# Ryukhaan/speech-to-video-mpp

Hardware: AMD Instinct MI355X
Metric: synthesized 256×256 frames/sec/GPU (LNet+ENet path); 1/2/4/8-GPU scaling (higher is better)
Workload: dtype f32; 1 GPU; ENet(+LNet) forward, B=16 synthetic 256x256 crops + [1,80,16] mel windows -> 384x384 (models/ENet.py:82-139); crop=256, global_batch=16, batch_per_gpu=16, parallelism=frame-shard x1 (no data-path collective), graph=True, lanes=1, world_size_seen=1

## Files before the change

include/s2v.h:

```cpp
#ifndef S2V_H_
#define S2V_H_

#include <stddef.h>
#include <stdint.h>

#ifdef __cplusplus
extern "C" {
#endif

typedef void *s2v_stream_t;

enum {
    S2V_OK = 0,
    S2V_E_INVALID = -1,
    S2V_E_LAUNCH = -2,
    S2V_E_WORKSPACE = -3
};

enum {
    S2V_ACT_NONE = 0,
    S2V_ACT_RELU = 1,
    S2V_ACT_LRELU = 2,
    S2V_ACT_SIGMOID = 3,
    S2V_ACT_TANH = 4,
    S2V_ACT_GELU_TANH = 5
};

enum {
    S2V_IN_DIRECT = 0,
    S2V_IN_NEAREST_UP2 = 1,
    S2V_IN_TRANSPOSED = 2
};

enum { S2V_PAD_ZERO = 0, S2V_PAD_REFLECT = 1 };

typedef struct s2v_conv_params {
    const float *x; int n, h, w, cin, xcs;
    int in_mode; int pad_mode;
    int pre_act; float pre_alpha;
    const float *in_scale; int in_scale_ns;
    int kh, kw, sh, sw, ph, pw, dh, dw;
    const float *wt; int kpad, npad; int cout;
    int b_kn; int ldb;
    float *y; int oh, ow, ycs;
    const float *scale, *shift;
    const float *nc_scale; int nc_scale_ns;
    const float *pix_add; float pix_w;
    const float *res; int res_cs, res_h, res_w, res_oy, res_ox; int res_after_act;
    int act; float alpha;
    int batch; long long x_bs, w_bs, y_bs, res_bs;
    float *ws; size_t ws_bytes;
    int force_tile; int force_splits;
    int out_step; int out_full_h, out_full_w;
    int prec;
    const void *wt_x3;
    int grid_cap;
    float wt_scale;
    int out_pool;
    int x_split;
    unsigned long long *stamps;
    const unsigned long long *stamp_ctr;
    int stamp_slot, stamp_stride, stamp_reps;
    float x_scale;
    int *nonfinite;
    int d2s_cout;
    const float *post_mul, *post_add; int post_cs, post_c0;
    const float *dup_src, *dup_bias; float dup_a; int dup_cs, dup_off;
} s2v_conv_params;

enum { S2V_PREC_F32 = 0, S2V_PREC_BF16X3 = 1, S2V_PREC_F16X3 = 2, S2V_PREC_F16 = 3 };

int s2v_conv2d(const s2v_conv_params *p, s2v_stream_t stream);
size_t s2v_conv2d_ws_bytes(const s2v_conv_params *p);
int s2v_conv2d_plan(const s2v_conv_params *p, int *out11);
#define S2V_CONV_GROUP_MAX 4
int s2v_conv2d_group(const s2v_conv_params *ps, int n, s2v_stream_t stream);
size_t s2v_conv2d_group_ws_bytes(const s2v_conv_params *ps, int n);
int s2v_conv2d_group_plan(const s2v_conv_params *ps, int n, int *out);
enum { S2V_TUNE_HALO_MIN_BLOCKS = 0, S2V_TUNE_GLDS_TILE = 1, S2V_TUNE_SMALLK_TILE = 2, S2V_TUNE_X3_RATE_512 = 3,
       S2V_TUNE_IN_FUSED = 4, S2V_TUNE_RESIZE_UP2 = 5, S2V_TUNE_COUNT = 6 };
int s2v_tune(int key, long long value, long long *old_value);

int s2v_amax(const float *x, long long pixels, int c, int xcs, float *out, s2v_stream_t stream);

int s2v_split_weights(const float *w, int rows, int kpad, int prec, float scale, void *out, s2v_stream_t stream);
int s2v_split_weights_x3(const float *w, int rows, int kpad, void *out, s2v_stream_t stream);
int s2v_split_act(const float *x, long long pixels, int c, int xcs, int prec, float *out, int ocs,
                  s2v_stream_t stream);

int s2v_layernorm2d(const float *x, int n, int h, int w, int c, int xcs,
                    const float *weight, const float *bias, float eps, int act, float alpha, int pool,
                    const float *res, int res_cs, float *y, int ycs, void *ws, size_t ws_bytes,
                    s2v_stream_t stream);
size_t s2v_layernorm2d_ws_bytes(int n, int h, int w, int c);

int s2v_instnorm_adain(const float *x, int n, int h, int w, int c, int xcs,
                       const float *gamma, const float *beta, int gb_ns, float eps, int act, float alpha,
                       const float *res, int res_cs, float *y, int ycs, void *ws, size_t ws_bytes,
                       s2v_stream_t stream);
int s2v_instnorm_adain_pad(const float *x, int n, int h, int w, int c, int xcs, const float *gamma,
                           const float *beta, int gb_ns, float eps, int act, float alpha, const float *res, int res_cs,
                           float *y, int ycs, float *yp, int ypcs, void *ws, size_t ws_bytes, s2v_stream_t stream);
size_t s2v_instnorm_ws_bytes(int n, int h, int w, int c);

int s2v_adain_params(const float *hid, int batch, int hid_ns, int nhidden, const float *w2t,
                     const float *bias, const int *seg, int total, float *out, int out_ns,
                     s2v_stream_t stream);

int s2v_modconv_demod(const float *s, int batch, int s_ns, int cin, const float *wsq, int cout,
                      float eps, float post, float *d, int d_ns, s2v_stream_t stream);

int s2v_modconv_demod_rows(const float *s, int batch, int s_ns, const int *rows, int nrows,
                           const float *wsq, float eps, float post, float *d, int d_ns,
                           s2v_stream_t stream);

int s2v_resize(const float *x, int n, int c, int ih, int iw, long long xsn, long long xsc, long long xsy,
               long long xsx, float *y, int oh, int ow, long long ysn, long long ysc, long long ysy,
               long long ysx, float scale_h, float scale_w, int mode, s2v_stream_t stream);

int s2v_torgb_up2(const float *x, int n, int h, int w, int c, int xcs, const float *wt, int kpad, const float *s,
                  int s_ns, const float *bias, const float *skip, int skcs, float *y, int ycs, s2v_stream_t stream);

int s2v_row_pack(const float *x, int n, int h, int w, int c, int xcs, int kw, int pw, float *y, int ycs,
                 s2v_stream_t stream);

int s2v_pad_reflect(const float *x, int n, int h, int w, int c, int xcs, int pt, int pb, int pl, int pr,
                    float *y, int ycs, s2v_stream_t stream);

int s2v_row_layernorm(const float *x, int rows, int dim, int xld, const float *weight, const float *bias,
                      float eps, float *y, int yld, s2v_stream_t stream);

int s2v_attention(const float *q, const float *k, const float *v, int batch, int heads, int tokens,
                  int dim_head, int ld_q, int ld_k, int ld_v, long long bs_q, long long bs_k, long long bs_v,
                  float scale, float *o, int ld_o, long long bs_o, s2v_stream_t stream);

int s2v_flow_warp(const float *flow, int n, int fh, int fw, int flow_cs, const float *src, int c, int h,
                  int w, long long ssn, long long ssc, long long ssy, long long ssx, float *y, int ycs,
                  s2v_stream_t stream);
int s2v_flow_warp_cat(const float *flow, int n, int fh, int fw, int flow_cs, const float *src, int c, int h,
                      int w, long long ssn, long long ssc, long long ssy, long long ssx, float *y, int ycs,
                      s2v_stream_t stream);

int s2v_melspectrogram(const float *wav, long long n_samples, const float *tables, int pad_reflect,
                       float *out, long long frames, s2v_stream_t stream);

int s2v_mel_chunks(const float *mel, long long frames, const int *starts, int nchunks, int step, float *out,
                   s2v_stream_t stream);

int s2v_fused_bias_act(const float *x, const float *b, const float *ref, float *y, long long size, int c,
                       long long step_b, int act, int grad, float alpha, float scale, s2v_stream_t stream);
int s2v_upfirdn2d(const float *x, int major, int in_h, int in_w, int minor, const float *k, int kh, int kw,
                  int up_x, int up_y, int down_x, int down_y, int pad_x0, int pad_x1, int pad_y0, int pad_y1,
                  float *y, int out_h, int out_w, s2v_stream_t stream);
enum { S2V_DT_F32 = 0, S2V_DT_F16 = 1, S2V_DT_F64 = 2 };
int s2v_fused_bias_act_dt(int dtype, const void *x, const void *b, const void *ref, void *y, long long size, int c,
                          long long step_b, int act, int grad, double alpha, double scale, s2v_stream_t stream);
int s2v_upfirdn2d_dt(int dtype, const void *x, int major, int in_h, int in_w, int minor, const void *k, int kh,
                     int kw, int up_x, int up_y, int down_x, int down_y, int pad_x0, int pad_x1, int pad_y0,
                     int pad_y1, void *y, int out_h, int out_w, s2v_stream_t stream);

size_t s2v_fft_tables_floats(int h, int w);
int s2v_rfft2(const float *x, int n, int h, int w, int c, int xcs, const float *tables, float *spec, int scs,
              s2v_stream_t stream);
int s2v_irfft2(const float *spec, int n, int h, int w, int c, int scs, const float *tables, const float *res,
               int rcs, float *y, int ycs, s2v_stream_t stream);

int s2v_f16_split_check(const float *x, long long n, int *mismatch, s2v_stream_t stream);

int s2v_ffc_channels(int h);
int s2v_ffc_spec_fwd(const float *x_g, int xcs, int n, int h, const void *w1, int w1_kpad, float wt_scale, float x_scale,
                     const float *scale, const float *shift, const float *tables, float *t1, float *spec, int *flag,
                     int prec, s2v_stream_t stream);
int s2v_ffc_spec_inv(const float *spec, int n, int h, const void *wfu, int wfu_kpad, float wt_scale, float x_scale,
                     const float *scale, const float *shift, const float *tables, const float *t1, float *u, int *flag,
                     int prec, s2v_stream_t stream);
int s2v_ffc_norm(const float *y, int ycs, int n, int h, const float *u, const void *w2, int w2_kpad, float wt_scale,
                 float x_scale, const float *gamma, const float *beta, int gb_ns, float eps, int act, float alpha,
                 const float *res, int res_cs, float *out, int out_cs, float *pad, int pad_cs, int *flag, int prec,
                 s2v_stream_t stream);

int s2v_modulate_weights(const float *wt, int npad, int kpad, int K, int cin, int cout, const float *s, int s_ns,
                         const float *d, int d_ns, int batch, float *out, s2v_stream_t stream);
int s2v_modulate_weights_split(const float *wt, int npad, int kpad, int K, int cin, int cout, const float *s,
                               int s_ns, const float *d, int d_ns, int batch, int prec, float scale, void *out,
                               s2v_stream_t stream);
int s2v_modulate_weights_x3(const float *wt, int npad, int kpad, int K, int cin, int cout, const float *s, int s_ns,
                            const float *d, int d_ns, int batch, void *out, s2v_stream_t stream);

int s2v_fir2d(const float *x, int n, int ih, int iw, int c, int xcs, const float *k, int kh, int kw, int up,
              int down, int pad_y0, int pad_x0, float *y, int oh, int ow, int ycs, float gain, const float *bias,
              int act, float alpha, float post, s2v_stream_t stream);

int s2v_gaussian_noise(float *y, long long n, unsigned long long seed, unsigned long long offset,
                       s2v_stream_t stream);
int s2v_gaussian_noise_ctr(float *y, long long n, unsigned long long seed, unsigned long long offset,
                           const unsigned long long *ctr, int shift, s2v_stream_t stream);
int s2v_counter_add(unsigned long long *ctr, unsigned long long inc, s2v_stream_t stream);

int s2v_lipsync_inputs(const float *src, const float *fake, int n, int h, int w, unsigned char *ref_u8,
                       float *face6, float *gt, s2v_stream_t stream);
int s2v_to_u8(const float *x, long long n, float lo, float hi, float scale, float offset, unsigned char *y,
              s2v_stream_t stream);
int s2v_eltwise(const float *x, int xcs, const float *mul, int mcs, const float *add, int acs, const float *bias,
                long long pixels, int c, float a, int act, float alpha, float post, float *y, int ycs,
                s2v_stream_t stream);

int s2v_fill(float *y, long long n, float value, s2v_stream_t stream);


int s2v_resize_linear(const void *x, int n, int h, int w, int c, long long xrs, long long xis, void *y, int oh,
                      int ow, long long yrs, long long yis, int mode, s2v_stream_t stream);
int s2v_resize_linear_fxfy(const void *x, int n, int h, int w, int c, long long xrs, long long xis, void *y, int oh,
                           int ow, long long yrs, long long yis, int mode, double fx, double fy, s2v_stream_t stream);

size_t s2v_laplacian_blend_ws_bytes(int n, int h, int w, int c, int levels);
int s2v_laplacian_blend(const unsigned char *a, const unsigned char *b, const float *m, int n, int h, int w, int c,
                        int levels, int clip, float *out, void *ws, size_t ws_bytes, s2v_stream_t stream);

int s2v_parse_mask(const float *x, int n, int h, int w, int c, long long xbs, long long ps, long long cs,
                   const unsigned char *cmap, unsigned char *out, int *cls, s2v_stream_t stream);

int s2v_img_u8_to_m11(const unsigned char *x, long long pixels, int flip, float *y, int ycs, s2v_stream_t stream);


int s2v_sr_u8_in(const unsigned char *x, int n, int h, int w, int flip, int pad_b, int pad_r, float *y, int ycs,
                 s2v_stream_t stream);
int s2v_sr_f32_out(const float *x, int n, int h, int w, int xh, int xw, int xcs, int flip, unsigned char *y,
                   s2v_stream_t stream);


int s2v_bgr_mean_nhwc4(const void *x, int xtype, long long pixels, float *y, s2v_stream_t stream);
int s2v_maxpool2d_nhwc(const float *x, int n, int h, int w, int c, int k, int s, int p, float *y, int oh, int ow,
                       s2v_stream_t stream);
int s2v_retina_decode(const float *const *heads, const int *hs, const int *ws, int cs, int im_h, int im_w,
                      float thresh, float *cand, int *count, int max_cand, s2v_stream_t stream);
int s2v_retina_split(const float *const *heads, const int *hs, const int *ws, int cs, int im_h, int im_w, int n,
                     float *loc, float *conf, float *landms, s2v_stream_t stream);
int s2v_u8_mean_nhwc4(const unsigned char *x, int n, long long pixels, const float *mean, int flip, float *y,
                      s2v_stream_t stream);
int s2v_l2norm_nhwc(const float *x, long long pixels, int c, long long x_cs, const float *weight, float eps, float *y,
                    long long y_cs, s2v_stream_t stream);
int s2v_s3fd_decode(const float *const *heads, const int *hs, const int *ws, int cs, int n, float thresh, float *cand,
                    int *count, int max_cand, s2v_stream_t stream);
int s2v_nms(const float *cand, const int *count, int n, int max_cand, int row_stride, float iou_thresh,
            float min_score, int top_k, int keep_max, float *out, int *kept, int *status, s2v_stream_t stream);
int s2v_nms_capacity(void);
int s2v_jpeg_encode(const uint8_t *frames, int n, int h, int w, long pitch_bytes, long frame_stride_bytes, int bgr,
                    const uint8_t *header, int header_bytes, const uint16_t *qtables, uint8_t *out, long capacity,
                    int *sizes, int *status, void *ws, long ws_bytes, s2v_stream_t stream);
long s2v_jpeg_ws_bytes(int n, int h, int w);
long s2v_jpeg_worst_bytes(int h, int w);
int s2v_jpeg_decode(const uint8_t *data, long data_bytes, const int *intervals, int n_intervals,
                    const int *frame_first, int max_per_frame, int n, int h, int w, int sampling,
                    const uint16_t *qtables, const uint8_t *huff_sets, int n_sets, const int *set_index, uint8_t *out,
                    long pitch_bytes, long frame_stride_bytes, int bgr, int *status, void *ws, long ws_bytes, int split,
                    s2v_stream_t stream);
long s2v_jpeg_decode_ws_bytes(int n, int h, int w, int sampling);
int s2v_warp_affine(const void *x, int n, int h, int w, int c, long long xrs, long long xis, int dtype,
                    const double *M, void *y, int oh, int ow, long long yrs, long long yis, s2v_stream_t stream);
int s2v_face_paste(const float *mask, const unsigned char *face, int S, const double *M, float *full_mask,
                   unsigned char *full_img, int H, int W, int y0, int x0, int wh, int ww, s2v_stream_t stream);
size_t s2v_gaussian_blur_ws_bytes(int h, int w, int dtype);
int s2v_gaussian_blur(const void *x, int xtype, int h, int w, int zero_border, const void *kern, int ksize, void *y,
                      int ytype, int dtype, void *ws, size_t ws_bytes, s2v_stream_t stream);
int s2v_filter3x3_u8(const unsigned char *x, int h, int w, int c, const float *kern, unsigned char *y,
                     s2v_stream_t stream);
int s2v_u8_to_gan(const unsigned char *x, int n, int h, int w, float *y, s2v_stream_t stream);
int s2v_gan_to_u8(const float *x, int n, int h, int w, unsigned char *y, s2v_stream_t stream);
int s2v_u8_div255_f64(const unsigned char *x, long long n, double *y, s2v_stream_t stream);
int s2v_u8_div255_f64_border(const unsigned char *x, int h, int w, int border, double *y, s2v_stream_t stream);
int s2v_face_blend(const unsigned char *base, const float *full_mask, const unsigned char *full_img,
                   const double *mask_sharp, unsigned char *out, long long pixels, s2v_stream_t stream);


int s2v_warp_affine_border(const void *x, int n, int h, int w, int c, long long xrs, long long xis, int dtype,
                           const double *M, void *y, int oh, int ow, long long yrs, long long yis,
                           const double *border, s2v_stream_t stream);
int s2v_tensor2img_u8(const float *x, int n, int h, int w, unsigned char *y, s2v_stream_t stream);
int s2v_restore_mask(const double *M, int S, int H, int W, int y0, int x0, int wh, int ww, float *erosion,
                     double *area, s2v_stream_t stream);
int s2v_restore_parts(void);
int s2v_erode_rect_f32(const float *x, int h, int w, int k, float *y, float *ws, s2v_stream_t stream);
int s2v_restore_paste(const unsigned char *face, int S, const double *M, const float *soft, const float *erosion,
                      int y0, int x0, int wh, int ww, const void *base, int base_f32, void *out, int out_f32, int H,
                      int W, s2v_stream_t stream);


int s2v_pil_resize_crop(const unsigned char *x, int n, int h0, int w0, long long xis, const int *params, int filter,
                        float *y, int oh, int ow, int ycs, s2v_stream_t stream);


int s2v_pil_transform_quad(const unsigned char *x, int n, int h, int w, int c, long long xrs, long long xis,
                           const double *table, unsigned char *y, int oh, int ow, long long yrs, long long yis,
                           s2v_stream_t stream);
int s2v_pil_perspective_paste(const unsigned char *crop, int n, int sh, int sw, int cc, long long crs,
                              long long cis, const double *coeffs, const unsigned char *target, int h, int w,
                              int tc, long long trs, long long tis, unsigned char *y, int yc, long long yrs,
                              long long yis, s2v_stream_t stream);

int s2v_spatial_mean_nhwc(const float *x, int n, int hw, int c, float *y, s2v_stream_t stream);


int s2v_bn_act_nhwc(const float *x, long long pixels, int c, long long x_cs, int x_off, const float *scale,
                    const float *shift, float *y, long long y_cs, int y_off, s2v_stream_t stream);
int s2v_fan_merge(const float *a, long long a_cs, const float *b, long long b_cs, int b_half, int n, int h, int w,
                  int c, float *s, long long s_cs, float *sa, long long sa_cs, const float *scale_a,
                  const float *shift_a, float *p, long long p_cs, float *pa, long long pa_cs, const float *scale_b,
                  const float *shift_b, s2v_stream_t stream);
int s2v_fan_crop(const unsigned char *frames, int n, int h, int w, const int *table, const int *host_table, int faces,
                 float *y, s2v_stream_t stream);
int s2v_fan_peaks(const float *hm, int n, int h, int w, int c, long long cs, float *preds, float *vals,
                  s2v_stream_t stream);


int s2v_gani_input(const unsigned char *x, int n, int h, int w, long long xrs, long long xis, const float *aus,
                   float *y, int oh, int ow, s2v_stream_t stream);
int s2v_gani_blend(const float *head, long long head_cs, const float *in, long long in_cs, int n, int h, int w,
                   float *color_mask, float *aus_mask, float *fake_img, s2v_stream_t stream);
int s2v_gani_compose(const float *pred, const unsigned char *orig, long long ors, long long ois, const float *fake,
                     int fh, int fw, int n, int ph, int pw, void *y, int out_u8, s2v_stream_t stream);

const char *s2v_last_error(void);
int s2v_device_cus(void);
const char *s2v_version(void);

#ifdef __cplusplus
}
#endif
#endif
```

speech-to-video-mpp_amd/_lib.py:

```python
from __future__ import annotations

import ctypes
import os
import threading

LIB_PATH = os.path.join(os.path.dirname(os.path.abspath(__file__)), "libs2v.so")

ACT_NONE, ACT_RELU, ACT_LRELU, ACT_SIGMOID, ACT_TANH, ACT_GELU_TANH = range(6)
IN_DIRECT, IN_NEAREST_UP2, IN_TRANSPOSED = range(3)
PAD_ZERO, PAD_REFLECT = range(2)
PREC_F32, PREC_BF16X3, PREC_F16X3, PREC_F16 = range(4)

_c_int, _c_float, _c_ll, _c_size, _vp = ctypes.c_int, ctypes.c_float, ctypes.c_longlong, ctypes.c_size_t, ctypes.c_void_p


class ConvParams(ctypes.Structure):
    _fields_ = [
        ("x", _vp), ("n", _c_int), ("h", _c_int), ("w", _c_int), ("cin", _c_int), ("xcs", _c_int),
        ("in_mode", _c_int), ("pad_mode", _c_int), ("pre_act", _c_int), ("pre_alpha", _c_float),
        ("in_scale", _vp), ("in_scale_ns", _c_int),
        ("kh", _c_int), ("kw", _c_int), ("sh", _c_int), ("sw", _c_int), ("ph", _c_int), ("pw", _c_int),
        ("dh", _c_int), ("dw", _c_int),
        ("wt", _vp), ("kpad", _c_int), ("npad", _c_int), ("cout", _c_int), ("b_kn", _c_int), ("ldb", _c_int),
        ("y", _vp), ("oh", _c_int), ("ow", _c_int), ("ycs", _c_int),
        ("scale", _vp), ("shift", _vp), ("nc_scale", _vp), ("nc_scale_ns", _c_int),
        ("pix_add", _vp), ("pix_w", _c_float),
        ("res", _vp), ("res_cs", _c_int), ("res_h", _c_int), ("res_w", _c_int), ("res_oy", _c_int),
        ("res_ox", _c_int), ("res_after_act", _c_int),
        ("act", _c_int), ("alpha", _c_float),
        ("batch", _c_int), ("x_bs", _c_ll), ("w_bs", _c_ll), ("y_bs", _c_ll), ("res_bs", _c_ll),
        ("ws", _vp), ("ws_bytes", _c_size),
        ("force_tile", _c_int), ("force_splits", _c_int),
        ("out_step", _c_int), ("out_full_h", _c_int), ("out_full_w", _c_int),
        ("prec", _c_int), ("wt_x3", _vp),
        ("grid_cap", _c_int),
        ("wt_scale", _c_float),
        ("out_pool", _c_int),
        ("x_split", _c_int),
        ("stamps", _vp), ("stamp_ctr", _vp), ("stamp_slot", _c_int), ("stamp_stride", _c_int),
        ("stamp_reps", _c_int),
        ("x_scale", _c_float), ("nonfinite", _vp),
        ("d2s_cout", _c_int),
        ("post_mul", _vp), ("post_add", _vp), ("post_cs", _c_int), ("post_c0", _c_int),
        ("dup_src", _vp), ("dup_bias", _vp), ("dup_a", _c_float), ("dup_cs", _c_int), ("dup_off", _c_int),
    ]


_SIGS = {
    "s2v_conv2d": (_c_int, [ctypes.POINTER(ConvParams), _vp]),
    "s2v_conv2d_ws_bytes": (_c_size, [ctypes.POINTER(ConvParams)]),
    "s2v_conv2d_plan": (_c_int, [ctypes.POINTER(ConvParams), ctypes.POINTER(_c_int)]),
    "s2v_conv2d_group": (_c_int, [ctypes.POINTER(ConvParams), _c_int, _vp]),
    "s2v_conv2d_group_ws_bytes": (_c_size, [ctypes.POINTER(ConvParams), _c_int]),
    "s2v_conv2d_group_plan": (_c_int, [ctypes.POINTER(ConvParams), _c_int, ctypes.POINTER(_c_int)]),
    "s2v_tune": (_c_int, [_c_int, _c_ll, ctypes.POINTER(_c_ll)]),
    "s2v_layernorm2d": (_c_int, [_vp, _c_int, _c_int, _c_int, _c_int, _c_int, _vp, _vp, _c_float, _c_int, _c_float,
                                 _c_int, _vp, _c_int, _vp, _c_int, _vp, _c_size, _vp]),
    "s2v_layernorm2d_ws_bytes": (_c_size, [_c_int, _c_int, _c_int, _c_int]),
    "s2v_instnorm_adain": (_c_int, [_vp, _c_int, _c_int, _c_int, _c_int, _c_int, _vp, _vp, _c_int, _c_float, _c_int,
                                    _c_float, _vp, _c_int, _vp, _c_int, _vp, _c_size, _vp]),
    "s2v_instnorm_adain_pad": (_c_int, [_vp, _c_int, _c_int, _c_int, _c_int, _c_int, _vp, _vp, _c_int, _c_float,
                                        _c_int, _c_float, _vp, _c_int, _vp, _c_int, _vp, _c_int, _vp, _c_size, _vp]),
    "s2v_instnorm_ws_bytes": (_c_size, [_c_int, _c_int, _c_int, _c_int]),
    "s2v_adain_params": (_c_int, [_vp, _c_int, _c_int, _c_int, _vp, _vp, _vp, _c_int, _vp, _c_int, _vp]),
    "s2v_modconv_demod": (_c_int, [_vp, _c_int, _c_int, _c_int, _vp, _c_int, _c_float, _c_float, _vp, _c_int, _vp]),
    "s2v_modconv_demod_rows": (_c_int, [_vp, _c_int, _c_int, _vp, _c_int, _vp, _c_float, _c_float, _vp, _c_int,
                                        _vp]),
    "s2v_torgb_up2": (_c_int, [_vp, _c_int, _c_int, _c_int, _c_int, _c_int, _vp, _c_int, _vp, _c_int, _vp, _vp,
                               _c_int, _vp, _c_int, _vp]),
    "s2v_resize": (_c_int, [_vp, _c_int, _c_int, _c_int, _c_int, _c_ll, _c_ll, _c_ll, _c_ll, _vp, _c_int, _c_int,
                            _c_ll, _c_ll, _c_ll, _c_ll, _c_float, _c_float, _c_int, _vp]),
    "s2v_row_pack": (_c_int, [_vp, _c_int, _c_int, _c_int, _c_int, _c_int, _c_int, _c_int, _vp, _c_int, _vp]),
    "s2v_pad_reflect": (_c_int, [_vp, _c_int, _c_int, _c_int, _c_int, _c_int, _c_int, _c_int, _c_int, _c_int, _vp,
                                 _c_int, _vp]),
    "s2v_row_layernorm": (_c_int, [_vp, _c_int, _c_int, _c_int, _vp, _vp, _c_float, _vp, _c_int, _vp]),
    "s2v_attention": (_c_int, [_vp, _vp, _vp, _c_int, _c_int, _c_int, _c_int, _c_int, _c_int, _c_int, _c_ll, _c_ll,
                               _c_ll, _c_float, _vp, _c_int, _c_ll, _vp]),
    "s2v_flow_warp": (_c_int, [_vp, _c_int, _c_int, _c_int, _c_int, _vp, _c_int, _c_int, _c_int, _c_ll, _c_ll,
                               _c_ll, _c_ll, _vp, _c_int, _vp]),
    "s2v_flow_warp_cat": (_c_int, [_vp, _c_int, _c_int, _c_int, _c_int, _vp, _c_int, _c_int, _c_int, _c_ll, _c_ll,
                                   _c_ll, _c_ll, _vp, _c_int, _vp]),
    "s2v_melspectrogram": (_c_int, [_vp, _c_ll, _vp, _c_int, _vp, _c_ll, _vp]),
    "s2v_mel_chunks": (_c_int, [_vp, _c_ll, _vp, _c_int, _c_int, _vp, _vp]),
    "s2v_fused_bias_act": (_c_int, [_vp, _vp, _vp, _vp, _c_ll, _c_int, _c_ll, _c_int, _c_int, _c_float, _c_float,
                                    _vp]),
    "s2v_upfirdn2d": (_c_int, [_vp, _c_int, _c_int, _c_int, _c_int, _vp, _c_int, _c_int, _c_int, _c_int, _c_int,
                               _c_int, _c_int, _c_int, _c_int, _c_int, _vp, _c_int, _c_int, _vp]),
    "s2v_fused_bias_act_dt": (_c_int, [_c_int, _vp, _vp, _vp, _vp, _c_ll, _c_int, _c_ll, _c_int, _c_int,
                                       ctypes.c_double, ctypes.c_double, _vp]),
    "s2v_upfirdn2d_dt": (_c_int, [_c_int, _vp, _c_int, _c_int, _c_int, _c_int, _vp, _c_int, _c_int, _c_int, _c_int,
                                  _c_int, _c_int, _c_int, _c_int, _c_int, _c_int, _vp, _c_int, _c_int, _vp]),
    "s2v_fir2d": (_c_int, [_vp, _c_int, _c_int, _c_int, _c_int, _c_int, _vp, _c_int, _c_int, _c_int, _c_int, _c_int,
                           _c_int, _vp, _c_int, _c_int, _c_int, _c_float, _vp, _c_int, _c_float, _c_float, _vp]),
    "s2v_fft_tables_floats": (_c_size, [_c_int, _c_int]),
    "s2v_rfft2": (_c_int, [_vp, _c_int, _c_int, _c_int, _c_int, _c_int, _vp, _vp, _c_int, _vp]),
    "s2v_irfft2": (_c_int, [_vp, _c_int, _c_int, _c_int, _c_int, _c_int, _vp, _vp, _c_int, _vp, _c_int, _vp]),
    "s2v_f16_split_check": (_c_int, [_vp, _c_ll, _vp, _vp]),
    "s2v_ffc_channels": (_c_int, [_c_int]),
    "s2v_ffc_spec_fwd": (_c_int, [_vp, _c_int, _c_int, _c_int, _vp, _c_int, _c_float, _c_float, _vp, _vp, _vp, _vp, _vp,
                                  _vp, _c_int, _vp]),
    "s2v_ffc_spec_inv": (_c_int, [_vp, _c_int, _c_int, _vp, _c_int, _c_float, _c_float, _vp, _vp, _vp, _vp, _vp, _vp,
                                  _c_int, _vp]),
    "s2v_ffc_norm": (_c_int, [_vp, _c_int, _c_int, _c_int, _vp, _vp, _c_int, _c_float, _c_float, _vp, _vp, _c_int,
                              _c_float, _c_int, _c_float, _vp, _c_int, _vp, _c_int, _vp, _c_int, _vp, _c_int, _vp]),
    "s2v_split_weights": (_c_int, [_vp, _c_int, _c_int, _c_int, _c_float, _vp, _vp]),
    "s2v_split_act": (_c_int, [_vp, _c_ll, _c_int, _c_int, _c_int, _vp, _c_int, _vp]),
    "s2v_amax": (_c_int, [_vp, _c_ll, _c_int, _c_int, _vp, _vp]),
    "s2v_split_weights_x3": (_c_int, [_vp, _c_int, _c_int, _vp, _vp]),
    "s2v_modulate_weights_split": (_c_int, [_vp, _c_int, _c_int, _c_int, _c_int, _c_int, _vp, _c_int, _vp, _c_int,
                                            _c_int, _c_int, _c_float, _vp, _vp]),
    "s2v_modulate_weights_x3": (_c_int, [_vp, _c_int, _c_int, _c_int, _c_int, _c_int, _vp, _c_int, _vp, _c_int,
                                         _c_int, _vp, _vp]),
    "s2v_modulate_weights": (_c_int, [_vp, _c_int, _c_int, _c_int, _c_int, _c_int, _vp, _c_int, _vp, _c_int, _c_int,
                                      _vp, _vp]),
    "s2v_gaussian_noise": (_c_int, [_vp, _c_ll, ctypes.c_uint64, ctypes.c_uint64, _vp]),
    "s2v_gaussian_noise_ctr": (_c_int, [_vp, _c_ll, ctypes.c_uint64, ctypes.c_uint64, _vp, _c_int, _vp]),
    "s2v_counter_add": (_c_int, [_vp, ctypes.c_uint64, _vp]),
    "s2v_lipsync_inputs": (_c_int, [_vp, _vp, _c_int, _c_int, _c_int, _vp, _vp, _vp, _vp]),
    "s2v_to_u8": (_c_int, [_vp, _c_ll, _c_float, _c_float, _c_float, _c_float, _vp, _vp]),
    "s2v_eltwise": (_c_int, [_vp, _c_int, _vp, _c_int, _vp, _c_int, _vp, _c_ll, _c_int, _c_float, _c_int, _c_float,
                             _c_float, _vp, _c_int, _vp]),
    "s2v_fill": (_c_int, [_vp, _c_ll, _c_float, _vp]),
    "s2v_resize_linear": (_c_int, [_vp, _c_int, _c_int, _c_int, _c_int, _c_ll, _c_ll, _vp, _c_int, _c_int, _c_ll,
                                   _c_ll, _c_int, _vp]),
    "s2v_resize_linear_fxfy": (_c_int, [_vp, _c_int, _c_int, _c_int, _c_int, _c_ll, _c_ll, _vp, _c_int, _c_int, _c_ll,
                                        _c_ll, _c_int, ctypes.c_double, ctypes.c_double, _vp]),
    "s2v_laplacian_blend_ws_bytes": (_c_size, [_c_int, _c_int, _c_int, _c_int, _c_int]),
    "s2v_laplacian_blend": (_c_int, [_vp, _vp, _vp, _c_int, _c_int, _c_int, _c_int, _c_int, _c_int, _vp, _vp, _c_size,
                                     _vp]),
    "s2v_parse_mask": (_c_int, [_vp, _c_int, _c_int, _c_int, _c_int, _c_ll, _c_ll, _c_ll, _vp, _vp, _vp, _vp]),
    "s2v_img_u8_to_m11": (_c_int, [_vp, _c_ll, _c_int, _vp, _c_int, _vp]),
    "s2v_sr_u8_in": (_c_int, [_vp, _c_int, _c_int, _c_int, _c_int, _c_int, _c_int, _vp, _c_int, _vp]),
    "s2v_sr_f32_out": (_c_int, [_vp, _c_int, _c_int, _c_int, _c_int, _c_int, _c_int, _c_int, _vp, _vp]),
    "s2v_bgr_mean_nhwc4": (_c_int, [_vp, _c_int, _c_ll, _vp, _vp]),
    "s2v_maxpool2d_nhwc": (_c_int, [_vp] + [_c_int] * 7 + [_vp, _c_int, _c_int, _vp]),
    "s2v_retina_decode": (_c_int, [_vp, _vp, _vp, _c_int, _c_int, _c_int, _c_float, _vp, _vp, _c_int, _vp]),
    "s2v_retina_split": (_c_int, [_vp, _vp, _vp, _c_int, _c_int, _c_int, _c_int, _vp, _vp, _vp, _vp]),
    "s2v_u8_mean_nhwc4": (_c_int, [_vp, _c_int, _c_ll, _vp, _c_int, _vp, _vp]),
    "s2v_l2norm_nhwc": (_c_int, [_vp, _c_ll, _c_int, _c_ll, _vp, _c_float, _vp, _c_ll, _vp]),
    "s2v_s3fd_decode": (_c_int, [_vp, _vp, _vp, _c_int, _c_int, _c_float, _vp, _vp, _c_int, _vp]),
    "s2v_nms": (_c_int, [_vp, _vp, _c_int, _c_int, _c_int, _c_float, _c_float, _c_int, _c_int, _vp, _vp, _vp, _vp]),
    "s2v_nms_capacity": (_c_int, []),
    "s2v_jpeg_encode": (_c_int, [_vp, _c_int, _c_int, _c_int, ctypes.c_long, ctypes.c_long, _c_int, _vp, _c_int, _vp,
                                 _vp, ctypes.c_long, _vp, _vp, _vp, ctypes.c_long, _vp]),
    "s2v_jpeg_ws_bytes": (ctypes.c_long, [_c_int, _c_int, _c_int]),
    "s2v_jpeg_worst_bytes": (ctypes.c_long, [_c_int, _c_int]),
    "s2v_jpeg_decode": (_c_int, [_vp, ctypes.c_long, _vp, _c_int, _vp, _c_int, _c_int, _c_int, _c_int, _c_int, _vp, _vp,
                                 _c_int, _vp, _vp, ctypes.c_long, ctypes.c_long, _c_int, _vp, _vp, ctypes.c_long,
                                 _c_int, _vp]),
    "s2v_jpeg_decode_ws_bytes": (ctypes.c_long, [_c_int, _c_int, _c_int, _c_int]),
    "s2v_bn_act_nhwc": (_c_int, [_vp, _c_ll, _c_int, _c_ll, _c_int, _vp, _vp, _vp, _c_ll, _c_int, _vp]),
    "s2v_fan_merge": (_c_int, [_vp, _c_ll, _vp, _c_ll, _c_int, _c_int, _c_int, _c_int, _c_int, _vp, _c_ll, _vp, _c_ll,
                               _vp, _vp, _vp, _c_ll, _vp, _c_ll, _vp, _vp, _vp]),
    "s2v_fan_crop": (_c_int, [_vp, _c_int, _c_int, _c_int, _vp, _vp, _c_int, _vp, _vp]),
    "s2v_fan_peaks": (_c_int, [_vp, _c_int, _c_int, _c_int, _c_int, _c_ll, _vp, _vp, _vp]),
    "s2v_warp_affine": (_c_int, [_vp, _c_int, _c_int, _c_int, _c_int, _c_ll, _c_ll, _c_int, _vp, _vp, _c_int, _c_int,
                                 _c_ll, _c_ll, _vp]),
    "s2v_face_paste": (_c_int, [_vp, _vp, _c_int, _vp, _vp, _vp] + [_c_int] * 6 + [_vp]),
    "s2v_gaussian_blur_ws_bytes": (_c_size, [_c_int, _c_int, _c_int]),
    "s2v_gaussian_blur": (_c_int, [_vp, _c_int, _c_int, _c_int, _c_int, _vp, _c_int, _vp, _c_int, _c_int, _vp, _c_size,
                                   _vp]),
    "s2v_filter3x3_u8": (_c_int, [_vp, _c_int, _c_int, _c_int, _vp, _vp, _vp]),
    "s2v_u8_to_gan": (_c_int, [_vp, _c_int, _c_int, _c_int, _vp, _vp]),
    "s2v_gan_to_u8": (_c_int, [_vp, _c_int, _c_int, _c_int, _vp, _vp]),
    "s2v_u8_div255_f64": (_c_int, [_vp, _c_ll, _vp, _vp]),
    "s2v_u8_div255_f64_border": (_c_int, [_vp, _c_int, _c_int, _c_int, _vp, _vp]),
    "s2v_face_blend": (_c_int, [_vp, _vp, _vp, _vp, _vp, _c_ll, _vp]),
    "s2v_warp_affine_border": (_c_int, [_vp, _c_int, _c_int, _c_int, _c_int, _c_ll, _c_ll, _c_int, _vp, _vp, _c_int,
                                        _c_int, _c_ll, _c_ll, _vp, _vp]),
    "s2v_tensor2img_u8": (_c_int, [_vp, _c_int, _c_int, _c_int, _vp, _vp]),
    "s2v_restore_mask": (_c_int, [_vp] + [_c_int] * 7 + [_vp, _vp, _vp]),
    "s2v_restore_parts": (_c_int, []),
    "s2v_erode_rect_f32": (_c_int, [_vp, _c_int, _c_int, _c_int, _vp, _vp, _vp]),
    "s2v_restore_paste": (_c_int, [_vp, _c_int, _vp, _vp, _vp] + [_c_int] * 4 + [_vp, _c_int, _vp, _c_int, _c_int,
                                                                             _c_int, _vp]),
    "s2v_pil_resize_crop": (_c_int, [_vp, _c_int, _c_int, _c_int, _c_ll, _vp, _c_int, _vp, _c_int, _c_int, _c_int,
                                     _vp]),
    "s2v_pil_transform_quad": (_c_int, [_vp, _c_int, _c_int, _c_int, _c_int, _c_ll, _c_ll, _vp, _vp, _c_int, _c_int,
                                        _c_ll, _c_ll, _vp]),
    "s2v_pil_perspective_paste": (_c_int, [_vp, _c_int, _c_int, _c_int, _c_int, _c_ll, _c_ll, _vp, _vp, _c_int,
                                           _c_int, _c_int, _c_ll, _c_ll, _vp, _c_int, _c_ll, _c_ll, _vp]),
    "s2v_spatial_mean_nhwc": (_c_int, [_vp, _c_int, _c_int, _c_int, _vp, _vp]),
    "s2v_gani_input": (_c_int, [_vp, _c_int, _c_int, _c_int, _c_ll, _c_ll, _vp, _vp, _c_int, _c_int, _vp]),
    "s2v_gani_blend": (_c_int, [_vp, _c_ll, _vp, _c_ll, _c_int, _c_int, _c_int, _vp, _vp, _vp, _vp]),
    "s2v_gani_compose": (_c_int, [_vp, _vp, _c_ll, _c_ll, _vp, _c_int, _c_int, _c_int, _c_int, _c_int, _vp, _c_int,
                                  _vp]),
    "s2v_last_error": (ctypes.c_char_p, []),
    "s2v_device_cus": (_c_int, []),
    "s2v_version": (ctypes.c_char_p, []),
}

EXPORTS = tuple(_SIGS)

_lock = threading.Lock()
_lib = None


class S2VError(RuntimeError):
    pass


def load():
    global _lib
    if _lib is not None:
        return _lib
    with _lock:
        if _lib is None:
            if not os.path.exists(LIB_PATH):
                raise S2VError(f"{LIB_PATH} is missing: build it with `make -C {os.path.dirname(LIB_PATH)}/csrc` "
                               "(or __graft_entry__.build()); the HIP path has no CPU fallback")
            lib = ctypes.CDLL(LIB_PATH)
            for name, (res, args) in _SIGS.items():
                fn = getattr(lib, name)
                fn.restype = res
                fn.argtypes = args
            _lib = lib
    return _lib


def check(rc: int, what: str):
    if rc != 0:
        msg = load().s2v_last_error().decode(errors="replace")
        raise S2VError(f"{what} failed ({rc}): {msg}")
```

speech-to-video-mpp_amd/csrc/conv_plan.cpp:

```cpp
#include "conv_plan.hpp"

#include <cmath>
#include <cstdint>
#include <cstdlib>
#include <vector>

namespace s2v {

static const struct { const char *env; long long def; } kKnobs[S2V_TUNE_COUNT] = {
    {"S2V_HALO_MIN_BLOCKS", 0}, {"S2V_GLDS_TILE", -1}, {"S2V_SMALLK_TILE", 1}, {"S2V_X3_RATE_512", 0},
    {"S2V_IN_FUSED", 576},
    {"S2V_RESIZE_UP2", 1}};
static_assert(S2V_TUNE_HALO_MIN_BLOCKS == 0 && S2V_TUNE_GLDS_TILE == 1 && S2V_TUNE_SMALLK_TILE == 2 &&
              S2V_TUNE_X3_RATE_512 == 3 && S2V_TUNE_IN_FUSED == 4 && S2V_TUNE_RESIZE_UP2 == 5, "kKnobs order");
static long long g_tune[S2V_TUNE_COUNT];
static bool g_tune_init = false;
long long tune_get(int key) {
    for (int i = 0; i < S2V_TUNE_COUNT && !g_tune_init; ++i) {
        const char *e = getenv(kKnobs[i].env);
        g_tune[i] = e ? atoll(e) : kKnobs[i].def;
    }
    g_tune_init = true;
    return g_tune[key];
}

long long tune_set(int key, long long value) {
    const long long prev = tune_get(key);
    g_tune[key] = value;
    return prev;
}

static bool head_x3_on() {
    static const int on = [] { const char *e = getenv("S2V_HEAD_X3"); return e ? atoi(e) : 1; }();
    return on != 0;
}
static bool k4_on() {
    static const int on = [] { const char *e = getenv("S2V_K4"); return e ? atoi(e) : 1; }();
    return on != 0;
}
static const std::vector<int> &group_tiles() {
    static const std::vector<int> cands = [] {
        std::vector<int> v;
        const char *e = getenv("S2V_GROUP_TILES");
        if (e && *e) {
            for (const char *q = e; *q;) {
                const int t = atoi(q);
                if (t == 0 || t == 1 || t == 3 || t == 4 || t == 6) v.push_back(t);
                while (*q && *q != ',') ++q;
                if (*q == ',') ++q;
            }
        }
        if (v.empty()) v = {4, 3, 1};
        return v;
    }();
    return cands;
}

static int plan_cus() { return device_cus() > 0 ? device_cus() : 256; }

static const TileCfg kTiles[] = {
    {128, 128, 2, 4, 1, 2}, {128, 64, 2, 4, 1, 2}, {64, 128, 2, 4, 1, 2}, {64, 64, 2, 4, 1, 2}, {256, 32, 4, 4, 1, 2},
    {128, 32, 4, 4, 1, 2}};
constexpr int kNumTiles = sizeof(kTiles) / sizeof(kTiles[0]);
struct X3Cfg {
    TileCfg t;
    float tflops;
    int bpc;
    int kind = 0;
};
static const X3Cfg kX3Tiles[] = {
    {{256, 256, 2, 8, 1, 1}, 400.f, 1}, {{128, 128, 2, 8, 1, 1}, 330.f, 2}, {{64, 128, 2, 8, 1, 1}, 260.f, 3},
    {{128, 64, 2, 4, 1, 1}, 290.f, 3},  {{64, 64, 2, 4, 1, 1}, 265.f, 4},   {{128, 32, 4, 4, 1, 1}, 235.f, 4},
    {{256, 128, 4, 8, 1, 1}, 335.f, 1}, {{256, 64, 8, 8, 1, 1}, 300.f, 2},  {{512, 128, 4, 8, 1, 1}, 360.f, 1},
    {{512, 64, 8, 8, 1, 1}, 335.f, 1},  {{256, 64, 4, 4, 1, 1}, 350.f, 2},  {{256, 32, 4, 4, 1, 1}, 0.f, 2},
    {{64, 64, 2, 4, 4, 1}, 0.f, 1},     {{128, 64, 2, 4, 2, 1}, 0.f, 1},   {{128, 32, 4, 4, 2, 1}, 0.f, 1},
    {{256, 64, 4, 4, 1, 1}, 0.f, 2, 1},
    {{256, 64, 4, 4, 1, 1}, 0.f, 2, 2},
    {{256, 64, 4, 4, 1, 1}, 0.f, 2, 3},
    {{512, 64, 8, 8, 1, 1}, 0.f, 1, 4},
    {{256, 128, 4, 8, 1, 1}, 0.f, 1, 5}};
constexpr int kNumX3 = sizeof(kX3Tiles) / sizeof(kX3Tiles[0]);

struct GldsCfg {
    int bm, bn, wm, nst;
};
static const GldsCfg kGlds[] = {{256, 256, 2, 2}, {256, 128, 4, 3}, {512, 128, 4, 2}};

static int batch_of(const s2v_conv_params *p) { return p->batch > 0 ? p->batch : 1; }

static long long tile_blocks(const Plan &pl, const TileCfg &t) {
    return (long long)cdiv(pl.M, t.bm) * cdiv(pl.cout, t.bn) * pl.batch;
}

int epi_vec4(const s2v_conv_params *p) {
    return p->cout % 4 == 0 && p->ycs % 4 == 0 && ((uintptr_t)p->y % 16) == 0 && p->y_bs % 4 == 0 &&
           (!p->res || (p->res_cs % 4 == 0 && ((uintptr_t)p->res % 16) == 0 && p->res_bs % 4 == 0)) &&
           (!p->scale || ((uintptr_t)p->scale % 16) == 0) && (!p->shift || ((uintptr_t)p->shift % 16) == 0) &&
           (!p->post_mul || (p->post_cs % 4 == 0 && p->post_c0 % 4 == 0 && ((uintptr_t)p->post_mul % 16) == 0 &&
                             ((uintptr_t)p->post_add % 16) == 0)) &&
           (!p->dup_src || (p->dup_cs % 4 == 0 && p->dup_off % 4 == 0 && ((uintptr_t)p->dup_src % 16) == 0 &&
                            (!p->dup_bias || ((uintptr_t)p->dup_bias % 16) == 0)));
}

static bool vec4_input(const s2v_conv_params *p) {
    return (p->cin % 4 == 0) && (p->xcs % 4 == 0) && (((uintptr_t)p->x % 16) == 0) && (p->x_bs % 4 == 0) &&
           (!p->in_scale || (p->in_scale_ns % 4 == 0 && ((uintptr_t)p->in_scale % 16) == 0));
}

static bool use_direct(const s2v_conv_params *p) { return p->cout <= 4 && !p->b_kn; }

static bool plain_head(const s2v_conv_params *p) {
    return p->cout <= 4 && p->kh == p->kw && p->in_mode == S2V_IN_DIRECT && p->sh == 1 && p->sw == 1 && p->dh == 1 &&
           p->dw == 1 && !p->in_scale && !p->pre_act && !p->w_bs && batch_of(p) == 1 && !p->b_kn && p->out_step <= 1 &&
           p->ph < p->kh && p->pw < p->kw && p->xcs % 4 == 0 && ((uintptr_t)p->x % 16) == 0 &&
           !(p->pad_mode == S2V_PAD_REFLECT && (p->ph >= p->h || p->pw >= p->w));
}

static int halo_ks(const s2v_conv_params *p) {
    if (!plain_head(p) || (p->kh != 3 && p->kh != 5 && p->kh != 7) || p->cin % 4) return 0;
    const long long blocks = (long long)p->n * cdiv(p->ow, 128) * cdiv(p->oh, 8);
    if (blocks < tune_get(S2V_TUNE_HALO_MIN_BLOCKS)) return 0;
    return p->kh;
}

static int halo_splits(const s2v_conv_params *p, int &per) {
    const long long blocks = (long long)p->n * cdiv(p->ow, 128) * cdiv(p->oh, 8);
    const int cus = plan_cus();
    const int quads = p->cin / 4;
    int s = blocks >= 3LL * cus ? 1 : (int)((3LL * cus + blocks - 1) / blocks);
    if (s > quads / 2) s = quads / 2;
    if (s < 1) s = 1;
    per = 4 * ((quads + s - 1) / s);
    return (p->cin + per - 1) / per;
}

static bool head_x3_ok(const s2v_conv_params *p) {
    if (!head_x3_on() || p->prec == S2V_PREC_F32 || p->x_split || p->force_tile || !p->wt_x3 || ((uintptr_t)p->wt_x3 % 16))
        return false;
    return plain_head(p) && (p->kh == 7 || p->kh == 5) && (p->cin == 32 || p->cin % 64 == 0) && p->cin <= 512 &&
           !p->out_pool && !p->d2s_cout;
}
static int head_rows(const s2v_conv_params *p) {
    const long long strips = cdiv(p->ow, 32 - p->kw + 1);
    int th = 16;
    const long long groups = p->cin > 64 ? p->cin / 64 : 1;
    while (th > 4 && (long long)p->n * strips * groups * cdiv(p->oh, th) < 2LL * device_cus()) th /= 2;
    return th;
}

static bool cpar_lw(int co, int K, long long w_bs, int batch, int M, int tpp) {
    return (size_t)co * K * sizeof(float) <= 16 * 1024 && (w_bs == 0 || batch == 1 || M % (256 / tpp) == 0);
}

static int cpar_lanes(int cin) { return cin >= 128 ? 8 : cin >= 64 ? 4 : cin >= 32 ? 2 : 4; }

static bool k4_ok(const s2v_conv_params *p) {
    if (!k4_on() || p->cin != 4 || p->kh != p->kw || (p->kh != 1 && p->kh != 3) || p->force_tile || p->b_kn || p->x_split)
        return false;
    if (p->in_mode != S2V_IN_DIRECT || p->pad_mode != S2V_PAD_ZERO || p->sh != 1 || p->sw != 1 || p->dh != 1 ||
        p->dw != 1 || p->ph != p->kh / 2 || p->pw != p->kw / 2)
        return false;
    if (p->cout % 32 || p->cout > 256 || p->in_scale || p->pre_act != S2V_ACT_NONE || p->nc_scale || p->res ||
        p->post_mul || p->dup_src || p->out_pool || p->out_step > 1 || p->d2s_cout > 0)
        return false;
    if (!p->wt || p->kpad < p->kh * p->kw * 4 || p->xcs % 4 || ((uintptr_t)p->x % 16) || p->x_bs % 4) return false;
    return (long long)p->n * p->oh * p->ow < (1LL << 31);
}

static bool smallk_cfg(const s2v_conv_params *p, int M, int K, int &tppx, int &qpt) {
    if (p->b_kn || p->force_tile || p->out_pool || p->cout < 8 || (p->cout & 3) || K > 64 || !vec4_input(p)) return false;
    if (p->prec != S2V_PREC_F32 && p->kh * p->kw > 1) return false;
    if (p->prec != S2V_PREC_F32 && K >= 32) return false;
    const int quads = p->cout / 4;
    if (quads & (quads - 1)) return false;
    tppx = quads < 64 ? quads : 64;
    qpt = quads / tppx;
    if (qpt > 2 || (size_t)K * p->cout * sizeof(float) > 64 * 1024) return false;
    return p->w_bs == 0 || batch_of(p) == 1 || M % (256 / tppx) == 0;
}

static int smallk_iters(const s2v_conv_params *p, int M, int tppx) {
    const bool per_entry = p->w_bs != 0 && batch_of(p) > 1;
    int it = 16;
    while (it > 1 && per_entry && M % (it * (256 / tppx)) != 0) it /= 2;
    return it;
}

static bool is_smallk(const s2v_conv_params *p) {
    const long long m = (long long)p->n * p->oh * p->ow, k = (long long)p->kh * p->kw * p->cin;
    int tppx, qpt;
    return m < (1LL << 31) && k <= 64 && smallk_cfg(p, (int)m, (int)k, tppx, qpt);
}
static bool tiled_x3(const s2v_conv_params *p) {
    return p->prec != S2V_PREC_F32 && !(use_direct(p) && !p->force_tile) && !is_smallk(p) && !k4_ok(p);
}

static int a_mode(const s2v_conv_params *p) {
    const bool vec = (p->cin % 4 == 0) && (p->xcs % 4 == 0) && (((uintptr_t)p->x % 16) == 0) && (p->x_bs % 4 == 0);
    if (!vec) return 2;
    const bool simple_pre = (p->pre_act == S2V_ACT_NONE || p->pre_act == S2V_ACT_RELU || p->pre_act == S2V_ACT_LRELU) &&
                            (!p->in_scale || (p->in_scale_ns % 4 == 0 && ((uintptr_t)p->in_scale % 16) == 0));
    if (p->cin % 32 == 0 && p->in_mode != S2V_IN_TRANSPOSED && simple_pre && !p->b_kn)
        return (p->pad_mode == S2V_PAD_ZERO && p->in_mode == S2V_IN_DIRECT) ? 0 : 3;
    if (p->cin % 32 == 0 && p->in_mode == S2V_IN_DIRECT && p->pad_mode == S2V_PAD_ZERO && simple_pre) return 0;
    return 1;
}

static long long x_extent_bytes(const s2v_conv_params *p) {
    return ((long long)p->n * p->h * p->w - 1) * p->xcs * 4 + (long long)p->cin * 4;
}
static long long w_extent_bytes(const s2v_conv_params *p) { return (long long)p->npad * p->kpad * 4; }

static bool x3_partial_1x1(const s2v_conv_params *p) {
    return p->kh == 1 && p->kw == 1 && p->cin % 8 == 0 && p->cin % 32 != 0 && p->in_mode == S2V_IN_DIRECT &&
           p->pad_mode == S2V_PAD_ZERO && !p->b_kn && !p->x_split && a_mode(p) == 1 && p->pre_act == S2V_ACT_NONE &&
           !p->in_scale;
}

static int x3_amode(const s2v_conv_params *p, const TileCfg &t) {
    const int am = x3_partial_1x1(p) ? 0 : a_mode(p);
    if (am != 0 || p->b_kn || p->kh * p->kw > 32 || t.bm % (16 * t.nw) != 0) return a_mode(p);
    if (x_extent_bytes(p) >= (1LL << 31) || w_extent_bytes(p) >= (1LL << 31)) return a_mode(p);
    return 4;
}

static bool direct_a_ok(const s2v_conv_params *p) {
    return tiled_x3(p) && !p->b_kn && !p->x_split && a_mode(p) == 0 && p->cin % 32 == 0 && !p->out_pool &&
           x_extent_bytes(p) < (1LL << 31) && w_extent_bytes(p) < (1LL << 31) && (long long)cdiv(p->cout, 64) * 64 <= p->npad;
}
static bool nar_ok(const s2v_conv_params *p) {
    return direct_a_ok(p) && p->kh * p->kw <= 32 && (!p->in_scale || (p->oh * p->ow) % 256 == 0);
}
static bool halo_ok(const s2v_conv_params *p) {
    return direct_a_ok(p) && p->kh == 3 && p->kw == 3 && p->sh == 1 && p->sw == 1 && p->dh == 1 && p->dw == 1 &&
           p->ph == 1 && p->pw == 1;
}

static double halo_fill(const s2v_conv_params *p, int th) {
    return (double)p->oh * p->ow / ((double)cdiv(p->oh, th) * th * cdiv(p->ow, 64) * 64);
}

static bool x3_kind_ok(const s2v_conv_params *p, int kind) {
    if (kind == 4) return halo_ok(p) && p->oh % 8 == 0;
    if (kind == 5) return halo_ok(p) && (long long)cdiv(p->cout, 128) * 128 <= p->npad;
    return kind == 0 || (kind == 3 ? halo_ok(p) : nar_ok(p));
}

static int persist_blocks(const s2v_conv_params *p, const Plan &pl) {
    if (p->grid_cap <= 0 || p->b_kn || pl.tile != 0 || pl.amode != 4 || p->post_mul || p->dup_src) return 0;
    const long long cap = p->grid_cap & ~7LL;
    return cap > 0 && tile_blocks(pl, pl.t) * pl.splits > cap ? (int)cap : 0;
}

static int fill_splits(const s2v_conv_params *p, const Plan &pl, long long blocks, long long below) {
    if (p->force_splits > 0) return p->force_splits;
    const int s = blocks < below ? (int)((2LL * plan_cus() + blocks - 1) / blocks) : 1;
    return s > pl.ktiles / 8 ? pl.ktiles / 8 : s;
}

static void finish_plan(Plan &pl, int splits) {
    if (pl.kslab > 1) {
        const int groups = pl.ktiles / pl.kslab;
        if (splits > groups) splits = groups;
        if (splits < 1) splits = 1;
        pl.tps = (groups + splits - 1) / splits * pl.kslab;
        pl.splits = (pl.ktiles + pl.tps - 1) / pl.tps;
        return;
    }
    if (splits > pl.ktiles) splits = pl.ktiles;
    if (splits < 1) splits = 1;
    pl.tps = (pl.ktiles + splits - 1) / splits;
    pl.splits = (pl.ktiles + pl.tps - 1) / pl.tps;
}

static void finish_x3(const s2v_conv_params *p, Plan &pl, int tile, int splits) {
    const X3Cfg &c = kX3Tiles[tile];
    pl.tile = tile;
    pl.t = c.t;
    pl.route = c.kind >= 3 ? Route::X3Halo : c.kind >= 1 ? Route::X3Nar : Route::X3Tile;
    if (c.kind >= 3) {
        pl.kslab = 9;
        pl.th = c.kind == 4 ? 8 : 4;
        pl.wn = c.kind == 5 ? 2 : 1;
    }
    finish_plan(pl, splits);
    pl.amode = c.kind >= 3 ? 8 : c.kind >= 1 ? 5 + c.kind : x3_amode(p, c.t);
    if (c.kind >= 1 || pl.amode == 4) {
        pl.x_bytes = (unsigned)x_extent_bytes(p);
        pl.w_bytes = (unsigned)w_extent_bytes(p);
    }
    if (pl.route == Route::X3Tile) pl.persist = persist_blocks(p, pl);
}

static void make_plan_x3(const s2v_conv_params *p, Plan &pl) {
    const int M = pl.M, batch = pl.batch;
    const int cus = plan_cus();
    if (p->force_tile > 0) {
        const int tile = p->force_tile - 1;
        return finish_x3(p, pl, tile, fill_splits(p, pl, tile_blocks(pl, kX3Tiles[tile].t), 2LL * cus));
    }
    if (halo_ok(p) && p->cout > 32 && p->cout <= 128 && halo_fill(p, 4) >= 0.85) {
        const long long blocks = (long long)p->n * cdiv(p->oh, 4) * cdiv(p->ow, 64) * cdiv(p->cout, 64) * batch;
        const int kind = p->cout > 64 && x3_kind_ok(p, 5) ? 5 : 3;
        const bool big_n128 = p->cout > 64 && (long long)p->n * p->oh * p->ow * batch >= (1LL << 20);
        if (blocks >= 2LL * cus && !big_n128) {
            for (int i = 0; i < kNumX3; ++i)
                if (kX3Tiles[i].kind == kind) return finish_x3(p, pl, i, 1);
        }
    }
    if (pl.ktiles <= 4 && !p->b_kn && tune_get(S2V_TUNE_SMALLK_TILE)) {
        int t = p->cout > 128 ? 0 : (p->cout > 64 ? 1 : 4);
        const TileCfg &c = kX3Tiles[t].t;
        if ((long long)cdiv(p->cout, c.bn) * c.bn <= p->npad && tile_blocks(pl, c) >= 4LL * cus) return finish_x3(p, pl, t, 1);
    }
    double best = 1e30;
    int bt = 8, bs = 1;
    const int am = a_mode(p);
    for (int i = 0; i < kNumX3; ++i) {
        const X3Cfg &c = kX3Tiles[i];
        if (c.tflops <= 0.f) continue;
        if (!x3_kind_ok(p, c.kind)) continue;
        if (p->b_kn && c.t.nw != 4) continue;
        if (c.t.bm >= 256 && c.t.bn >= 128 && am != 0 && am != 3) continue;
        if (c.t.bm >= 256 && c.t.bn <= 64 && am != 0) continue;
        if (!p->b_kn && (long long)cdiv(p->cout, c.t.bn) * c.t.bn > p->npad) continue;
        const long long tiles = tile_blocks(pl, c.t);
        const double slots = (double)cus * c.bpc;
        for (int s = 1; s <= 16; s *= 2) {
            if (s > 1 && (p->force_splits > 0 || s > pl.ktiles / 4)) break;
            if (p->force_splits > 0) s = p->force_splits;
            const int tps = (pl.ktiles + s - 1) / s;
            const long long r512 = (c.t.bm == 512) ? tune_get(S2V_TUNE_X3_RATE_512) : 0;
            const double rate = r512 > 0 ? (double)r512 : c.tflops;
            const double t_block = 2.0 * c.t.bm * c.t.bn * 32.0 * tps / (rate * 1e12 / slots);
            double t = std::ceil((double)(tiles * s) / slots) * t_block;
            if (s > 1) t += 4e-6 + (double)batch * M * p->cout * 4.0 * (s + 1) / 4e12;
            if (t < best * 0.97) {
                best = t;
                bt = i;
                bs = s;
            }
            if (p->force_splits > 0) break;
        }
    }
    finish_x3(p, pl, bt, bs);
}

static int glds_cfg(const s2v_conv_params *p) {
    const int forced = (int)tune_get(S2V_TUNE_GLDS_TILE);
    if (forced >= 0 && forced < (int)(sizeof(kGlds) / sizeof(kGlds[0]))) {
        const GldsCfg &c = kGlds[forced];
        if ((long long)cdiv(p->cout, c.bn) * c.bn <= p->npad) return forced;
    }
    if (p->cout > 128 && (long long)cdiv(p->cout, 256) * 256 <= p->npad) return 0;
    const long long m = (long long)p->n * p->oh * p->ow * batch_of(p);
    return m >= 512LL * 1024 ? 2 : 1;
}

static void make_plan_glds(const s2v_conv_params *p, Plan &pl) {
    pl.route = Route::Glds;
    pl.tile = glds_cfg(p);
    const GldsCfg &c = kGlds[pl.tile];
    pl.t = TileCfg{c.bm, c.bn, c.wm, 8, c.nst, 0};
    pl.amode = 5;
    finish_plan(pl, fill_splits(p, pl, tile_blocks(pl, pl.t), plan_cus()));
}

static void make_plan_igemm(const s2v_conv_params *p, Plan &pl) {
    const long long target = 2LL * plan_cus();
    int cands[kNumTiles];
    int nc = 0;
    if (p->force_tile > 0) {
        cands[nc++] = p->force_tile - 1;
    } else if (p->cout <= 32) {
        cands[nc++] = 5;
    } else if (p->cout <= 64) {
        cands[nc++] = 1; cands[nc++] = 3;
    } else {
        cands[nc++] = 0; cands[nc++] = 1; cands[nc++] = 2; cands[nc++] = 3;
    }
    pl.tile = cands[nc - 1];
    for (int i = 0; i < nc; ++i)
        if (tile_blocks(pl, kTiles[cands[i]]) >= target) {
            pl.tile = cands[i];
            break;
        }
    pl.route = Route::Igemm;
    pl.t = kTiles[pl.tile];
    pl.amode = a_mode(p);
    finish_plan(pl, fill_splits(p, pl, tile_blocks(pl, pl.t), target));
}

static Plan new_plan(const s2v_conv_params *p, int M, int K) {
    Plan pl{};
    pl.M = M; pl.K = K; pl.batch = batch_of(p);
    pl.cout = p->cout; pl.prec = p->prec; pl.bkn = p->b_kn != 0;
    pl.kslab = 1; pl.ktiles = (K + 31) / 32; pl.splits = 1; pl.tps = pl.ktiles;
    return pl;
}

static Plan make_plan(const s2v_conv_params *p_in, int M, int K) {
    s2v_conv_params q = *p_in;
    if (q.prec == S2V_PREC_F16) q.prec = S2V_PREC_F16X3;
    if (q.out_pool) q.force_splits = 1;
    const s2v_conv_params *p = &q;
    Plan pl = new_plan(p, M, K);
    int tppx, qpt;
    if (p->x_split) {
        make_plan_glds(p, pl);
    } else if (head_x3_ok(p)) {
        pl.route = Route::HeadX3;
        pl.splits = p->cin > 64 ? p->cin / 64 : 1;
        pl.fsize = p->kh;
        pl.ncs = p->cin == 32 ? 1 : 2;
        pl.rows = head_rows(p);
    } else if (use_direct(p) && !p->force_tile) {
        if ((pl.fsize = halo_ks(p)) != 0) {
            pl.route = Route::HaloSmall;
            pl.splits = halo_splits(p, pl.tps);
        } else if (vec4_input(p)) {
            pl.route = Route::SmallCpar;
            pl.lanes = cpar_lanes(p->cin);
            pl.lds_w = cpar_lw(p->cout, K, p->w_bs, pl.batch, M, pl.lanes);
        } else {
            pl.route = Route::DirectSmall;
        }
    } else if (k4_ok(p)) {
        pl.route = Route::K4;
        pl.kt = p->kh * p->kw;
    } else if (smallk_cfg(p, M, K, tppx, qpt)) {
        pl.kt = p->cin == 4 && p->kh == p->kw && (p->kh == 1 || p->kh == 3) ? p->kh * p->kw : 0;
        pl.route = pl.kt ? Route::SmallK4 : Route::SmallK;
        pl.tppx = tppx;
        pl.qpt = qpt;
        pl.iters = smallk_iters(p, M, tppx);
    } else if (tiled_x3(p)) {
        make_plan_x3(p, pl);
    } else {
        make_plan_igemm(p, pl);
    }
    if (pl.splits > 1) pl.ws_bytes = (size_t)pl.batch * pl.splits * (size_t)M * p->cout * sizeof(float);
    if (p_in->prec == S2V_PREC_F16 && (pl.route == Route::X3Tile || pl.route == Route::X3Halo)) pl.prec = S2V_PREC_F16;
    return pl;
}

static bool pow2_or_zero(float v) {
    int e;
    return v == 0.f || (v > 0.f && std::frexp(v, &e) == 0.5f);
}

static int validate(const s2v_conv_params *p, int &M, int &K) {
    S2V_REQUIRE(p && p->x && p->y, "conv2d: null pointer");
    S2V_REQUIRE(pow2_or_zero(p->x_scale), "conv2d: x_scale must be 0 or a positive power of two, got %g", p->x_scale);
    S2V_REQUIRE(!p->x_split || p->x_scale == 0.f || p->x_scale == 1.f,
                "conv2d: split-layout inputs carry no x_scale (split them already scaled)");
    S2V_REQUIRE(!p->stamps || (p->stamp_ctr && p->stamp_reps > 0 && p->stamp_slot >= 0 &&
                               p->stamp_slot < p->stamp_stride),
                "conv2d: launch stamps need stamp_ctr, stamp_reps > 0 and 0 <= stamp_slot < stamp_stride");
    S2V_REQUIRE(p->prec == S2V_PREC_F32 || p->prec == S2V_PREC_BF16X3 || p->prec == S2V_PREC_F16X3 ||
                    p->prec == S2V_PREC_F16,
                "conv2d: bad prec %d", p->prec);
    S2V_REQUIRE(pow2_or_zero(p->wt_scale), "conv2d: wt_scale must be 0 or a positive power of two, got %g", p->wt_scale);
    const bool x3 = tiled_x3(p);
// ... 200 lines not shown
```

speech-to-video-mpp_amd/csrc/torch_launch.cpp:

```cpp
#include <ATen/ATen.h>
#include <ATen/hip/HIPContext.h>
#include <c10/core/DeviceGuard.h>
#include <torch/library.h>

#include <vector>

#include "../../include/s2v.h"

namespace {

using at::Tensor;
using OptT = c10::optional<Tensor>;

void *stream() { return (void *)at::hip::getCurrentHIPStream().stream(); }

void check(int rc, const char *what) { TORCH_CHECK(rc == 0, what, " failed (", rc, "): ", s2v_last_error()); }

bool has(const OptT &t) { return t && t->defined(); }

void same_dev(const Tensor &t, const at::Device &dev, const char *what) {
    TORCH_CHECK(t.is_cuda(), what, ": expected a HIP device tensor (the s2v ops have no CPU kernel)");
    TORCH_CHECK(t.device() == dev, what, ": on ", t.device(), ", the op's inputs are on ", dev);
}

// ... 354 lines not shown
    float wscale = 1.f;
    if (x3) {
        wscale = ((prec == S2V_PREC_F16X3 || prec == S2V_PREC_F16) && has(d)) ? 2048.f : 1.f;
        p.wt = nullptr; p.wt_x3 = wbuf.data_ptr(); p.wt_scale = wscale;
    }
    set_stamps(p, stamps, stamp_ctr, stamp_pos, dev);
    set_range(p, x_scale, nonfinite, dev);
    const size_t need = s2v_conv2d_ws_bytes(&p);
    const Ws w = workspace(ws, dev);
    if (dry || w.bytes < need) return plan_list(p, (int64_t)need);
    p.ws = (float *)w.p; p.ws_bytes = w.bytes;
    auto out = plan_list(p, 0);
    const float *dp = has(d) ? d->data_ptr<float>() : nullptr;
    TORCH_CHECK(premod == 0.0 || (x3 ? premod == (double)wscale : premod < 0.0),
                "modconv: the pre-modulated weights (premod ", premod, ") are not the layout this conv reads (",
                x3 ? "split, pre-scale " : "fp32", x3 ? wscale : 0.f, ")");
    if (premod == 0.0 && x3)
        check(s2v_modulate_weights_split(wt.data_ptr<float>(), npad, kpad, K, p.cin, (int)cout, s.data_ptr<float>(),
                                         s_ns, dp, d_ns, B, split_layout(prec), wscale, wbuf.data_ptr(), stream()),
              "s2v_modulate_weights_split");
    else if (premod == 0.0)
        check(s2v_modulate_weights(wt.data_ptr<float>(), npad, kpad, K, p.cin, (int)cout, s.data_ptr<float>(), s_ns, dp,
                                   d_ns, B, wbuf.data_ptr<float>(), stream()),
              "s2v_modulate_weights");
    check(s2v_conv2d(&p, stream()), "s2v_conv2d");
    return out;
}

void modulate_weights_(const Tensor &wt, const Tensor &s, const OptT &d, const Tensor &wbuf, int64_t cout, int64_t cin,
                       int64_t taps, int64_t prec, double wscale) {
    const c10::DeviceGuard guard(wt.device());
    const at::Device dev = wt.device();
    f32(wt, dev, "modulate wt");
    TORCH_CHECK(wt.dim() == 2 && wt.is_contiguous() && wt.size(0) >= cout, "modulate wt: packed [npad, kpad]");
    const int npad = (int)wt.size(0), kpad = (int)wt.size(1), K = (int)(taps * cin);
    TORCH_CHECK(kpad >= K && cin > 0 && cout > 0, "modulate: kpad < taps * cin");
    f32(wbuf, dev, "modulate wbuf");
    TORCH_CHECK(wbuf.dim() == 3 && wbuf.is_contiguous() && wbuf.size(1) == npad && wbuf.size(2) == kpad,
                "modulate wbuf: [B, npad, kpad]");
    const int B = (int)wbuf.size(0);
    const int s_ns = (int)rows_view(s, dev, B, cin, "modulate s");
    int d_ns = 0;
    if (has(d)) d_ns = (int)rows_view(*d, dev, B, cout, "modulate d");
    const float *dp = has(d) ? d->data_ptr<float>() : nullptr;
    if (prec != S2V_PREC_F32)
        check(s2v_modulate_weights_split(wt.data_ptr<float>(), npad, kpad, K, (int)cin, (int)cout, s.data_ptr<float>(),
                                         s_ns, dp, d_ns, B, (int)prec, (float)wscale, wbuf.data_ptr(), stream()),
              "s2v_modulate_weights_split");
    else
        check(s2v_modulate_weights(wt.data_ptr<float>(), npad, kpad, K, (int)cin, (int)cout, s.data_ptr<float>(), s_ns,
                                   dp, d_ns, B, wbuf.data_ptr<float>(), stream()),
              "s2v_modulate_weights");
}

std::vector<int64_t> gemm_kn_(const Tensor &a, const Tensor &b, const Tensor &out, int64_t batch, int64_t a_bs,
                              int64_t b_bs, int64_t out_bs, const OptT &res, int64_t res_bs, int64_t act, double alpha,
                              int64_t prec, const OptT &ws, int64_t force_tile, int64_t force_splits, bool dry) {
    const c10::DeviceGuard guard(a.device());
    const at::Device dev = a.device();
    f32(a, dev, "gemm a"); f32(b, dev, "gemm b"); f32(out, dev, "gemm out");
    TORCH_CHECK(a.is_contiguous() && b.is_contiguous() && out.is_contiguous(), "gemm: contiguous operands");
    const int64_t M = a.size(-2), K = a.size(-1), N = b.size(-1);
    TORCH_CHECK(b.size(-2) == K && out.size(-2) == M && out.size(-1) == N, "gemm: [M, K] @ [K, N] -> [M, N]");
    TORCH_CHECK(batch >= 1 && (batch - 1) * a_bs + M * K <= a.numel() && (batch - 1) * b_bs + K * N <= b.numel() &&
                    (batch - 1) * out_bs + M * N <= out.numel(),
                "gemm: batch strides leave the operands");
    s2v_conv_params p{};
    p.x = a.data_ptr<float>(); p.n = 1; p.h = 1; p.w = (int)M; p.cin = (int)K; p.xcs = (int)K;
    p.kh = p.kw = p.sh = p.sw = p.dh = p.dw = 1;
    p.wt = b.data_ptr<float>(); p.cout = (int)N; p.b_kn = 1; p.ldb = (int)N;
    p.prec = (int)prec;
    p.y = out.data_ptr<float>(); p.oh = 1; p.ow = (int)M; p.ycs = (int)N;
    if (has(res)) {
        f32(*res, dev, "gemm res");
        TORCH_CHECK(res->is_contiguous() && (batch - 1) * res_bs + M * N <= res->numel(), "gemm res");
        p.res = res->data_ptr<float>(); p.res_cs = (int)N; p.res_h = 1; p.res_w = (int)M; p.res_bs = res_bs;
    }
    p.act = (int)act; p.alpha = (float)alpha;
    p.batch = (int)batch; p.x_bs = a_bs; p.w_bs = b_bs; p.y_bs = out_bs;
    p.force_tile = (int)force_tile; p.force_splits = (int)force_splits;
    const size_t need = s2v_conv2d_ws_bytes(&p);
    const Ws w = workspace(ws, dev);
    if (dry || w.bytes < need) return plan_list(p, (int64_t)need);
    p.ws = (float *)w.p; p.ws_bytes = w.bytes;
    auto o = plan_list(p, 0);
    check(s2v_conv2d(&p, stream()), "s2v_conv2d(gemm)");
    return o;
}

void amax_(const Tensor &x, const Tensor &out) {
    const c10::DeviceGuard guard(x.device());
    const NV xv = nhwc(x, x.device(), "amax x");
    f32(out, x.device(), "amax out");
    TORCH_CHECK(out.numel() >= 1 && out.is_contiguous(), "amax out: float32 [1]");
    check(s2v_fill(out.data_ptr<float>(), 1, 0.f, stream()), "s2v_fill");
    check(s2v_amax(xv.p, (long long)xv.n * xv.h * xv.w, xv.c, xv.cs, out.data_ptr<float>(), stream()), "s2v_amax");
}

void split_weights_(const Tensor &w, const Tensor &out, int64_t prec, double scale) {
    const c10::DeviceGuard guard(w.device());
    f32(w, w.device(), "split_weights w");
    f32(out, w.device(), "split_weights out");
    TORCH_CHECK(w.dim() == 2 && w.is_contiguous() && out.sizes() == w.sizes() && out.is_contiguous() &&
                    w.size(1) % 32 == 0,
                "split_weights: packed [rows, kpad], kpad % 32 == 0, out of the same shape");
    check(s2v_split_weights(w.data_ptr<float>(), (int)w.size(0), (int)w.size(1), (int)prec, (float)scale,
                            out.data_ptr(), stream()),
          "s2v_split_weights");
}

void split_act_(const Tensor &x, const Tensor &out, int64_t prec) {
    const c10::DeviceGuard guard(x.device());
    const NV xv = nhwc(x, x.device(), "split_act x"), ov = nhwc(out, x.device(), "split_act out");
    TORCH_CHECK(xv.n == ov.n && xv.h == ov.h && xv.w == ov.w && xv.c == ov.c, "split_act: out must match x");
    check(s2v_split_act(xv.p, (long long)xv.n * xv.h * xv.w, xv.c, xv.cs, (int)prec, ov.p, ov.cs, stream()),
          "s2v_split_act");
}

int64_t layernorm2d_(const Tensor &x, const Tensor &weight, const Tensor &bias, double eps, int64_t act,
                     double alpha, bool pool, const OptT &res, const Tensor &y, const OptT &ws) {
    const c10::DeviceGuard guard(x.device());
    const at::Device dev = x.device();
    const NV xv = nhwc(x, dev, "layernorm2d x"), yv = nhwc(y, dev, "layernorm2d y");
    const int f = pool ? 2 : 1;
    TORCH_CHECK(yv.n == xv.n && yv.h * f == xv.h && yv.w * f == xv.w && yv.c == xv.c, "layernorm2d: y shape");
    const float *wp = vec(weight, dev, xv.c, "layernorm2d weight"), *bp = vec(bias, dev, xv.c, "layernorm2d bias");
    const float *rp = nullptr;
    int rcs = 0;
    if (has(res)) {
        const NV rv = nhwc(*res, dev, "layernorm2d res");
        TORCH_CHECK(rv.n == yv.n && rv.h == yv.h && rv.w == yv.w && rv.c == yv.c, "layernorm2d: res shape");
        rp = rv.p; rcs = rv.cs;
    }
    const size_t need = s2v_layernorm2d_ws_bytes(xv.n, xv.h, xv.w, xv.c);
    const Ws w = workspace(ws, dev);
    if (w.bytes < need) return (int64_t)need;
    check(s2v_layernorm2d(xv.p, xv.n, xv.h, xv.w, xv.c, xv.cs, wp, bp, (float)eps, (int)act, (float)alpha, pool, rp,
                          rcs, yv.p, yv.cs, w.p, w.bytes, stream()),
          "s2v_layernorm2d");
    return 0;
}

int64_t instnorm_(const Tensor &x, const OptT &gamma, const OptT &beta, double eps, int64_t act, double alpha,
                  const OptT &res, const Tensor &y, const OptT &pad_out, const OptT &ws) {
    const c10::DeviceGuard guard(x.device());
    const at::Device dev = x.device();
    const NV xv = nhwc(x, dev, "instnorm x"), yv = nhwc(y, dev, "instnorm y");
    TORCH_CHECK(yv.n == xv.n && yv.h == xv.h && yv.w == xv.w && yv.c == xv.c, "instnorm: y shape");
    TORCH_CHECK(has(gamma) == has(beta), "instnorm: gamma and beta together");
    const float *gp = nullptr, *bp = nullptr;
    int ns = 0;
    if (has(gamma)) {
        ns = (int)rows_view(*gamma, dev, xv.n, xv.c, "instnorm gamma");
        TORCH_CHECK(rows_view(*beta, dev, xv.n, xv.c, "instnorm beta") == ns, "instnorm: gamma / beta row strides");
        gp = gamma->data_ptr<float>(); bp = beta->data_ptr<float>();
    }
    const float *rp = nullptr;
    int rcs = 0;
    if (has(res)) {
        const NV rv = nhwc(*res, dev, "instnorm res");
        TORCH_CHECK(rv.n == xv.n && rv.h == xv.h && rv.w == xv.w && rv.c == xv.c, "instnorm: res shape");
        rp = rv.p; rcs = rv.cs;
    }
    const size_t need = s2v_instnorm_ws_bytes(xv.n, xv.h, xv.w, xv.c);
    const Ws w = workspace(ws, dev);
    if (w.bytes < need) return (int64_t)need;
    if (has(pad_out)) {
        const NV pv = nhwc(*pad_out, dev, "instnorm pad_out");
        TORCH_CHECK(pv.n == xv.n && pv.h == xv.h + 2 && pv.w == xv.w + 2 && pv.c == xv.c,
                    "instnorm pad_out: [N, H + 2, W + 2, C]");
        check(s2v_instnorm_adain_pad(xv.p, xv.n, xv.h, xv.w, xv.c, xv.cs, gp, bp, ns, (float)eps, (int)act,
                                     (float)alpha, rp, rcs, yv.p, yv.cs, pv.p, pv.cs, w.p, w.bytes, stream()),
              "s2v_instnorm_adain_pad");
    } else {
        check(s2v_instnorm_adain(xv.p, xv.n, xv.h, xv.w, xv.c, xv.cs, gp, bp, ns, (float)eps, (int)act, (float)alpha, rp,
                                 rcs, yv.p, yv.cs, w.p, w.bytes, stream()),
              "s2v_instnorm_adain");
    }
    return 0;
}

void adain_params_(const Tensor &hid, int64_t nhidden, const Tensor &w2t, const Tensor &bias, const Tensor &seg,
                   const Tensor &out) {
    const c10::DeviceGuard guard(hid.device());
    const at::Device dev = hid.device();
    const int64_t batch = out.size(0), total = out.size(1);
    const int64_t hns = rows_view(hid, dev, batch, 1, "adain hid");
    const int64_t ons = rows_view(out, dev, batch, total, "adain out");
    f32(w2t, dev, "adain w2t");
    TORCH_CHECK(w2t.is_contiguous() && w2t.dim() == 2 && w2t.size(0) == nhidden && w2t.size(1) == total,
                "adain w2t: [nhidden, total]");
    vec(bias, dev, total, "adain bias");
    same_dev(seg, dev, "adain seg");
    TORCH_CHECK(seg.scalar_type() == at::kInt && seg.is_contiguous() && seg.numel() >= total, "adain seg: int32 [total]");
    check(s2v_adain_params(hid.data_ptr<float>(), (int)batch, (int)hns, (int)nhidden, w2t.data_ptr<float>(),
                           bias.data_ptr<float>(), seg.data_ptr<int>(), (int)total, out.data_ptr<float>(), (int)ons,
                           stream()),
          "s2v_adain_params");
}

void modconv_demod_(const Tensor &s, const Tensor &wsq, const Tensor &d, double eps, double post) {
    const c10::DeviceGuard guard(s.device());
    const at::Device dev = s.device();
    const int64_t batch = d.size(0), cout = wsq.size(0), cin = wsq.size(1);
    const int64_t sns = rows_view(s, dev, batch, cin, "demod s"), dns = rows_view(d, dev, batch, cout, "demod d");
    vec(wsq, dev, cout * cin, "demod wsq");
    check(s2v_modconv_demod(s.data_ptr<float>(), (int)batch, (int)sns, (int)cin, wsq.data_ptr<float>(), (int)cout,
                            (float)eps, (float)post, d.data_ptr<float>(), (int)dns, stream()),
          "s2v_modconv_demod");
}

void modconv_demod_rows_(const Tensor &s, const Tensor &rows, const Tensor &wsq, const Tensor &d, double eps,
                         double post, int64_t s_reach) {
    const c10::DeviceGuard guard(s.device());
    const at::Device dev = s.device();
    const int64_t batch = d.size(0), nrows = rows.size(0);
    same_dev(rows, dev, "demod rows");
    TORCH_CHECK(rows.scalar_type() == at::kInt && rows.is_contiguous() && rows.dim() == 2 && rows.size(1) == 4,
                "demod rows: int32 [nrows, 4]");
    const int64_t sns = rows_view(s, dev, batch, std::max<int64_t>(s_reach, 2), "demod s");
    vec(wsq, dev, wsq.numel(), "demod wsq");
    const int64_t dns = rows_view(d, dev, batch, nrows, "demod d");
    check(s2v_modconv_demod_rows(s.data_ptr<float>(), (int)batch, (int)sns, rows.data_ptr<int>(), (int)nrows,
                                 wsq.data_ptr<float>(), (float)eps, (float)post, d.data_ptr<float>(), (int)dns,
                                 stream()),
          "s2v_modconv_demod_rows");
}

void row_layernorm_(const Tensor &x, const Tensor &weight, const Tensor &bias, double eps, const Tensor &y) {
    const c10::DeviceGuard guard(x.device());
    const at::Device dev = x.device();
    const int64_t rows = x.size(0), dim = x.size(1);
    const int64_t xld = rows_view(x, dev, rows, dim, "row_layernorm x");
    const int64_t yld = rows_view(y, dev, rows, dim, "row_layernorm y");
    check(s2v_row_layernorm(x.data_ptr<float>(), (int)rows, (int)dim, (int)xld, vec(weight, dev, dim, "ln weight"),
                            vec(bias, dev, dim, "ln bias"), (float)eps, y.data_ptr<float>(), (int)yld, stream()),
          "s2v_row_layernorm");
}

void attention_(const Tensor &q, const Tensor &k, const Tensor &v, const Tensor &out, int64_t batch, int64_t heads,
                int64_t tokens, int64_t dim_head, double scale) {
    const c10::DeviceGuard guard(q.device());
    const at::Device dev = q.device();
    const int64_t rows = batch * tokens, cols = heads * dim_head;
    const int64_t lq = rows_view(q, dev, rows, cols, "attention q"), lk = rows_view(k, dev, rows, cols, "attention k");
    const int64_t lv = rows_view(v, dev, rows, cols, "attention v"), lo = rows_view(out, dev, rows, cols, "attention out");
    check(s2v_attention(q.data_ptr<float>(), k.data_ptr<float>(), v.data_ptr<float>(), (int)batch, (int)heads,
                        (int)tokens, (int)dim_head, (int)lq, (int)lk, (int)lv, tokens * lq, tokens * lk, tokens * lv,
                        (float)scale, out.data_ptr<float>(), (int)lo, tokens * lo, stream()),
          "s2v_attention");
}

const float *strided(const Tensor &base, int64_t off, at::IntArrayRef size, at::IntArrayRef st, const at::Device &dev,
                     const char *what) {
    f32(base, dev, what);
    TORCH_CHECK(size.size() == 4 && st.size() == 4, what, ": 4 sizes and 4 strides");
    int64_t lo = off, hi = off;
    for (int i = 0; i < 4; ++i) {
        TORCH_CHECK(size[i] > 0, what, ": empty view");
        const int64_t span = (size[i] - 1) * st[i];
        if (span < 0) lo += span; else hi += span;
    }
    const int64_t avail = base.storage().nbytes() / 4 - base.storage_offset();
    TORCH_CHECK(lo >= 0 && hi < avail, what, ": view [", lo, ", ", hi, "] leaves its tensor (", avail, " elements)");
    return base.data_ptr<float>() + off;
}

void resize_(const Tensor &x, int64_t x_off, at::IntArrayRef x_size, at::IntArrayRef x_stride, const Tensor &y,
             int64_t y_off, at::IntArrayRef y_size, at::IntArrayRef y_stride, double scale_h, double scale_w,
             int64_t mode) {
    const c10::DeviceGuard guard(x.device());
    const at::Device dev = x.device();
    const float *xp = strided(x, x_off, x_size, x_stride, dev, "resize x");
    float *yp = const_cast<float *>(strided(y, y_off, y_size, y_stride, dev, "resize y"));
    TORCH_CHECK(x_size[0] == y_size[0] && x_size[1] == y_size[1], "resize: n / c of x and y differ");
    check(s2v_resize(xp, (int)x_size[0], (int)x_size[1], (int)x_size[2], (int)x_size[3], x_stride[0], x_stride[1],
                     x_stride[2], x_stride[3], yp, (int)y_size[2], (int)y_size[3], y_stride[0], y_stride[1],
                     y_stride[2], y_stride[3], (float)scale_h, (float)scale_w, (int)mode, stream()),
          "s2v_resize");
}

void row_pack_(const Tensor &x, const Tensor &y, int64_t kw, int64_t pw) {
    const c10::DeviceGuard guard(x.device());
    const at::Device dev = x.device();
    const NV xv = nhwc(x, dev, "row_pack x"), yv = nhwc(y, dev, "row_pack y");
    TORCH_CHECK(yv.n == xv.n && yv.h == xv.h && yv.w == xv.w && yv.c == yv.cs && yv.c >= kw * xv.c,
                "row_pack: y must be a dense [n, h, w, >= kw * c] tensor");
    check(s2v_row_pack(xv.p, xv.n, xv.h, xv.w, xv.c, xv.cs, (int)kw, (int)pw, yv.p, yv.cs, stream()), "s2v_row_pack");
}

void pad_reflect_(const Tensor &x, const Tensor &y, at::IntArrayRef pads) {
    const c10::DeviceGuard guard(x.device());
    const at::Device dev = x.device();
    TORCH_CHECK(pads.size() == 4, "pad_reflect: pads (top, bottom, left, right)");
    const NV xv = nhwc(x, dev, "pad_reflect x"), yv = nhwc(y, dev, "pad_reflect y");
    TORCH_CHECK(yv.n == xv.n && yv.c == xv.c && yv.h == xv.h + pads[0] + pads[1] && yv.w == xv.w + pads[2] + pads[3],
                "pad_reflect: y shape");
    check(s2v_pad_reflect(xv.p, xv.n, xv.h, xv.w, xv.c, xv.cs, (int)pads[0], (int)pads[1], (int)pads[2], (int)pads[3],
                          yv.p, yv.cs, stream()),
          "s2v_pad_reflect");
}

void torgb_up2_(const Tensor &x, const Tensor &wt, const Tensor &s, const OptT &bias, const Tensor &skip,
                const Tensor &y) {
    const c10::DeviceGuard guard(x.device());
    const at::Device dev = x.device();
    const NV xv = nhwc(x, dev, "torgb x"), kv = nhwc(skip, dev, "torgb skip"), yv = nhwc(y, dev, "torgb y");
    f32(wt, dev, "torgb wt");
    TORCH_CHECK(wt.dim() == 2 && wt.is_contiguous() && wt.size(0) >= 3 && wt.size(1) >= xv.c,
                "torgb wt: packed 1x1 rows [>= 3, kpad >= C]");
    const int s_ns = (int)rows_view(s, dev, xv.n, xv.c, "torgb s");
    const float *bp = vec(bias, dev, 3, "torgb bias");
    TORCH_CHECK(kv.n == xv.n && yv.n == xv.n && yv.h == xv.h && yv.w == xv.w && 2 * kv.h == xv.h && 2 * kv.w == xv.w &&
                    kv.c == 4 && yv.c == 4,
                "torgb: skip [N, H/2, W/2, 4] and y [N, H, W, 4] views expected");
    check(s2v_torgb_up2(xv.p, xv.n, xv.h, xv.w, xv.c, xv.cs, wt.data_ptr<float>(), (int)wt.size(1), s.data_ptr<float>(),
                        s_ns, bp, kv.p, kv.cs, yv.p, yv.cs, stream()),
          "s2v_torgb_up2");
}

void flow_warp_(const Tensor &flow, const Tensor &src, const Tensor &y) {
    const c10::DeviceGuard guard(flow.device());
    const at::Device dev = flow.device();
    const NV fv = nhwc(flow, dev, "flow_warp flow"), yv = nhwc(y, dev, "flow_warp y");
    f32(src, dev, "flow_warp src");
    TORCH_CHECK(src.dim() == 4 && src.size(0) == fv.n && fv.c >= 2, "flow_warp: src [N, C, H, W], flow >= 2 channels");
    TORCH_CHECK(yv.n == fv.n && yv.h == src.size(2) && yv.w == src.size(3) && yv.c == src.size(1), "flow_warp: y shape");
    check(s2v_flow_warp(fv.p, fv.n, fv.h, fv.w, fv.cs, src.data_ptr<float>(), (int)src.size(1), (int)src.size(2),
                        (int)src.size(3), src.stride(0), src.stride(1), src.stride(2), src.stride(3), yv.p, yv.cs,
                        stream()),
          "s2v_flow_warp");
}

void flow_warp_cat_(const Tensor &flow, const Tensor &src, const Tensor &y) {
    const c10::DeviceGuard guard(flow.device());
    const at::Device dev = flow.device();
    const NV fv = nhwc(flow, dev, "flow_warp_cat flow"), yv = nhwc(y, dev, "flow_warp_cat y");
    f32(src, dev, "flow_warp_cat src");
    TORCH_CHECK(src.dim() == 4 && src.size(0) == fv.n && fv.c >= 2, "flow_warp_cat: src [N, C, H, W], flow >= 2 channels");
    TORCH_CHECK(yv.n == fv.n && yv.h == src.size(2) && yv.w == src.size(3) && yv.c == 2 * src.size(1),
                "flow_warp_cat: y [N, H, W, 2C]");
    check(s2v_flow_warp_cat(fv.p, fv.n, fv.h, fv.w, fv.cs, src.data_ptr<float>(), (int)src.size(1), (int)src.size(2),
                            (int)src.size(3), src.stride(0), src.stride(1), src.stride(2), src.stride(3), yv.p, yv.cs,
                            stream()),
          "s2v_flow_warp_cat");
}

void fill_value_(const Tensor &y, double value) {
    const c10::DeviceGuard guard(y.device());
    f32(y, y.device(), "fill y");
    TORCH_CHECK(y.is_contiguous(), "fill: contiguous y");
    check(s2v_fill(y.data_ptr<float>(), y.numel(), (float)value, stream()), "s2v_fill");
}

void gaussian_noise_(const Tensor &y, int64_t seed, int64_t offset, const OptT &ctr, int64_t shift) {
    const c10::DeviceGuard guard(y.device());
    f32(y, y.device(), "noise y");
    TORCH_CHECK(y.is_contiguous(), "noise: contiguous y");
    if (has(ctr)) {
        same_dev(*ctr, y.device(), "noise ctr");
        TORCH_CHECK(ctr->scalar_type() == at::kLong && ctr->numel() >= 1, "noise ctr: int64 [1]");
        check(s2v_gaussian_noise_ctr(y.data_ptr<float>(), y.numel(), (unsigned long long)seed,
                                     (unsigned long long)offset, (const unsigned long long *)ctr->data_ptr(), (int)shift,
                                     stream()),
              "s2v_gaussian_noise_ctr");
    } else {
        check(s2v_gaussian_noise(y.data_ptr<float>(), y.numel(), (unsigned long long)seed, (unsigned long long)offset,
                                 stream()),
              "s2v_gaussian_noise");
    }
}

void counter_add_(const Tensor &ctr, int64_t inc) {
    const c10::DeviceGuard guard(ctr.device());
    same_dev(ctr, ctr.device(), "counter");
    TORCH_CHECK(ctr.scalar_type() == at::kLong && ctr.numel() >= 1, "counter: int64 [1]");
    check(s2v_counter_add((unsigned long long *)ctr.data_ptr(), (unsigned long long)inc, stream()), "s2v_counter_add");
}

void rfft2_(const Tensor &x, const Tensor &tables, const Tensor &spec) {
    const c10::DeviceGuard guard(x.device());
    const at::Device dev = x.device();
    const NV xv = nhwc(x, dev, "rfft2 x");
    vec(tables, dev, (int64_t)s2v_fft_tables_floats(xv.h, xv.w), "rfft2 tables");
    f32(spec, dev, "rfft2 spec");
    TORCH_CHECK(spec.dim() == 3 && spec.is_contiguous() && spec.size(0) == xv.n &&
                    spec.size(1) == (int64_t)xv.h * (xv.w / 2 + 1) && spec.size(2) >= 2 * xv.c,
                "rfft2 spec: [N, h * (w/2 + 1), >= 2C]");
    check(s2v_rfft2(xv.p, xv.n, xv.h, xv.w, xv.c, xv.cs, tables.data_ptr<float>(), spec.data_ptr<float>(),
                    (int)spec.size(2), stream()),
          "s2v_rfft2");
}

const void *split_rows(const Tensor &w, const at::Device &dev, int64_t rows, int64_t k, const char *what) {
    f32(w, dev, what);
    TORCH_CHECK(w.dim() == 2 && w.is_contiguous() && w.size(0) >= rows && w.size(1) >= k && w.size(1) % 32 == 0, what,
                ": split packed weights [npad >= ", rows, ", kpad >= ", k, "] expected, got ", w.sizes());
    return w.data_ptr();
}

int *range_flag(const OptT &flag, const at::Device &dev) {
    if (!has(flag)) return nullptr;
    same_dev(*flag, dev, "ffc flag");
    TORCH_CHECK(flag->scalar_type() == at::kInt && flag->numel() >= 1, "ffc flag: int32 [1]");
    return flag->data_ptr<int>();
}

void ffc_spec_fwd_(const Tensor &xg, const Tensor &w1, double wt_scale, double x_scale, const OptT &scale,
                   const OptT &shift, const Tensor &tables, const Tensor &t1, const Tensor &spec, const OptT &flag,
                   int64_t prec) {
    const c10::DeviceGuard guard(xg.device());
    const at::Device dev = xg.device();
    const NV xv = nhwc(xg, dev, "ffc x_g");
    const int c = s2v_ffc_channels(xv.h), cg = c - c / 4, cc = cg / 2;
    TORCH_CHECK(c > 0 && xv.w == xv.h && xv.c == cg, "ffc_spec_fwd: x_g [N, h, h, 3C/4] with h in {12, 24, 48}");
    const NV tv = nhwc(t1, dev, "ffc t1");
    TORCH_CHECK(tv.n == xv.n && tv.h == xv.h && tv.w == xv.w && tv.c == cc && tv.cs == cc, "ffc t1: dense [N, h, h, cc]");
    f32(spec, dev, "ffc spec");
    TORCH_CHECK(spec.dim() == 3 && spec.is_contiguous() && spec.size(0) == xv.n &&
                    spec.size(1) == (int64_t)xv.h * (xv.h / 2 + 1) && spec.size(2) == 2 * cc,
                "ffc spec: dense [N, F, 2cc]");
    vec(tables, dev, (int64_t)s2v_fft_tables_floats(xv.h, xv.h), "ffc tables");
    check(s2v_ffc_spec_fwd(xv.p, xv.cs, xv.n, xv.h, split_rows(w1, dev, cc, cg, "ffc w1"), (int)w1.size(1),
                           (float)wt_scale, (float)x_scale, vec(scale, dev, cc, "ffc scale1"), vec(shift, dev, cc, "ffc shift1"),
                           tables.data_ptr<float>(), tv.p, spec.data_ptr<float>(), range_flag(flag, dev), (int)prec,
                           stream()),
          "s2v_ffc_spec_fwd");
}

void ffc_spec_inv_(const Tensor &spec, const Tensor &wfu, double wt_scale, double x_scale, const OptT &scale,
                   const OptT &shift, const Tensor &tables, const Tensor &t1, const Tensor &u, const OptT &flag,
                   int64_t prec) {
    const c10::DeviceGuard guard(spec.device());
    const at::Device dev = spec.device();
    const NV tv = nhwc(t1, dev, "ffc t1"), uv = nhwc(u, dev, "ffc u");
    const int c = s2v_ffc_channels(tv.h), cg = c - c / 4, cc = cg / 2;
    TORCH_CHECK(c > 0 && tv.w == tv.h && tv.c == cc && tv.cs == cc, "ffc t1: dense [N, h, h, cc]");
    TORCH_CHECK(uv.n == tv.n && uv.h == tv.h && uv.w == tv.w && uv.c == cc && uv.cs == cc, "ffc u: dense [N, h, h, cc]");
    f32(spec, dev, "ffc spec");
    TORCH_CHECK(spec.dim() == 3 && spec.is_contiguous() && spec.size(0) == tv.n &&
                    spec.size(1) == (int64_t)tv.h * (tv.h / 2 + 1) && spec.size(2) == 2 * cc,
                "ffc spec: dense [N, F, 2cc]");
    vec(tables, dev, (int64_t)s2v_fft_tables_floats(tv.h, tv.h), "ffc tables");
    check(s2v_ffc_spec_inv(spec.data_ptr<float>(), tv.n, tv.h, split_rows(wfu, dev, 2 * cc, cg, "ffc wfu"),
                           (int)wfu.size(1), (float)wt_scale, (float)x_scale, vec(scale, dev, 2 * cc, "ffc scale_fu"),
                           vec(shift, dev, 2 * cc, "ffc shift_fu"), tables.data_ptr<float>(), tv.p, uv.p,
                           range_flag(flag, dev), (int)prec, stream()),
          "s2v_ffc_spec_inv");
}

void ffc_norm_(const Tensor &y, const Tensor &u, const Tensor &w2, double wt_scale, double x_scale, const OptT &gamma,
               const OptT &beta, double eps, int64_t act, double alpha, const OptT &res, const Tensor &out,
               const OptT &pad_out, const OptT &flag, int64_t prec) {
    const c10::DeviceGuard guard(y.device());
    const at::Device dev = y.device();
    const NV yv = nhwc(y, dev, "ffc_norm y"), uv = nhwc(u, dev, "ffc_norm u"), ov = nhwc(out, dev, "ffc_norm out");
    const int c = s2v_ffc_channels(yv.h), cg = c - c / 4, cc = cg / 2;
    TORCH_CHECK(c > 0 && yv.w == yv.h && yv.c == c, "ffc_norm: y [N, h, h, C] with h in {12, 24, 48}");
    TORCH_CHECK(uv.n == yv.n && uv.h == yv.h && uv.w == yv.w && uv.c == cc && uv.cs == cc, "ffc_norm u: dense [N, h, h, cc]");
    TORCH_CHECK(ov.n == yv.n && ov.h == yv.h && ov.w == yv.w && ov.c == c, "ffc_norm: out shape");
    TORCH_CHECK(has(gamma) == has(beta), "ffc_norm: gamma and beta together");
    const float *gp = nullptr, *bp = nullptr;
    int ns = 0;
    if (has(gamma)) {
        ns = (int)rows_view(*gamma, dev, yv.n, c, "ffc_norm gamma");
        TORCH_CHECK(rows_view(*beta, dev, yv.n, c, "ffc_norm beta") == ns, "ffc_norm: gamma / beta row strides");
        gp = gamma->data_ptr<float>(); bp = beta->data_ptr<float>();
    }
    const float *rp = nullptr;
    int rcs = 0;
    if (has(res)) {
        const NV rv = nhwc(*res, dev, "ffc_norm res");
        TORCH_CHECK(rv.n == yv.n && rv.h == yv.h && rv.w == yv.w && rv.c == c, "ffc_norm: res shape");
        rp = rv.p; rcs = rv.cs;
    }
    float *pp = nullptr;
    int pcs = 0;
    if (has(pad_out)) {
        const NV pv = nhwc(*pad_out, dev, "ffc_norm pad_out");
        TORCH_CHECK(pv.n == yv.n && pv.h == yv.h + 2 && pv.w == yv.w + 2 && pv.c == c, "ffc_norm pad_out: [N, h+2, h+2, C]");
        pp = pv.p; pcs = pv.cs;
    }
    check(s2v_ffc_norm(yv.p, yv.cs, yv.n, yv.h, uv.p, split_rows(w2, dev, cg, cc, "ffc w2"), (int)w2.size(1),
                       (float)wt_scale, (float)x_scale, gp, bp, ns, (float)eps, (int)act, (float)alpha, rp, rcs, ov.p,
                       ov.cs, pp, pcs, range_flag(flag, dev), (int)prec, stream()),
          "s2v_ffc_norm");
}

void irfft2_(const Tensor &spec, const Tensor &tables, const OptT &res, const Tensor &y) {
    const c10::DeviceGuard guard(spec.device());
    const at::Device dev = spec.device();
    const NV yv = nhwc(y, dev, "irfft2 y");
    vec(tables, dev, (int64_t)s2v_fft_tables_floats(yv.h, yv.w), "irfft2 tables");
    f32(spec, dev, "irfft2 spec");
    TORCH_CHECK(spec.dim() == 3 && spec.is_contiguous() && spec.size(0) == yv.n &&
                    spec.size(1) == (int64_t)yv.h * (yv.w / 2 + 1) && spec.size(2) >= 2 * yv.c,
                "irfft2 spec: [N, h * (w/2 + 1), >= 2C]");
    const float *rp = nullptr;
    int rcs = 0;
    if (has(res)) {
        const NV rv = nhwc(*res, dev, "irfft2 res");
        TORCH_CHECK(rv.n == yv.n && rv.h == yv.h && rv.w == yv.w && rv.c == yv.c, "irfft2: res shape");
        rp = rv.p; rcs = rv.cs;
    }
    check(s2v_irfft2(spec.data_ptr<float>(), yv.n, yv.h, yv.w, yv.c, (int)spec.size(2), tables.data_ptr<float>(), rp,
                     rcs, yv.p, yv.cs, stream()),
          "s2v_irfft2");
}

void eltwise_(const Tensor &x, const OptT &mul, const OptT &add, const OptT &bias, double a, int64_t act,
              double alpha, double post, const Tensor &y) {
    const c10::DeviceGuard guard(x.device());
    const at::Device dev = x.device();
    const NV xv = nhwc(x, dev, "eltwise x"), yv = nhwc(y, dev, "eltwise y");
    TORCH_CHECK(yv.n == xv.n && yv.h == xv.h && yv.w == xv.w && yv.c == xv.c, "eltwise: y shape");
    const float *mp = nullptr, *ap = nullptr;
    int mcs = 0, acs = 0;
    if (has(mul)) {
        const NV v = nhwc(*mul, dev, "eltwise mul");
        TORCH_CHECK(v.n == xv.n && v.h == xv.h && v.w == xv.w && v.c == xv.c, "eltwise: mul shape");
        mp = v.p; mcs = v.cs;
    }
    if (has(add)) {
        const NV v = nhwc(*add, dev, "eltwise add");
        TORCH_CHECK(v.n == xv.n && v.h == xv.h && v.w == xv.w && v.c == xv.c, "eltwise: add shape");
        ap = v.p; acs = v.cs;
    }
    check(s2v_eltwise(xv.p, xv.cs, mp, mcs, ap, acs, vec(bias, dev, xv.c, "eltwise bias"),
                      (long long)xv.n * xv.h * xv.w, xv.c, (float)a, (int)act, (float)alpha, (float)post, yv.p, yv.cs,
                      stream()),
          "s2v_eltwise");
}

void fir2d_(const Tensor &x, const Tensor &kernel, const Tensor &y, int64_t up, int64_t down, int64_t pad_y0,
            int64_t pad_x0, double gain, const OptT &bias, int64_t act, double alpha, double post) {
    const c10::DeviceGuard guard(x.device());
    const at::Device dev = x.device();
    const NV xv = nhwc(x, dev, "fir2d x"), yv = nhwc(y, dev, "fir2d y");
    TORCH_CHECK(xv.n == yv.n && xv.c == yv.c, "fir2d: batch / channel mismatch");
    f32(kernel, dev, "fir2d kernel");
    TORCH_CHECK(kernel.dim() == 2 && kernel.is_contiguous(), "fir2d kernel: [kh, kw]");
    check(s2v_fir2d(xv.p, xv.n, xv.h, xv.w, xv.c, xv.cs, kernel.data_ptr<float>(), (int)kernel.size(0),
                    (int)kernel.size(1), (int)up, (int)down, (int)pad_y0, (int)pad_x0, yv.p, yv.h, yv.w, yv.cs,
                    (float)gain, vec(bias, dev, xv.c, "fir2d bias"), (int)act, (float)alpha, (float)post, stream()),
          "s2v_fir2d");
}

void lipsync_inputs_(const Tensor &src, const OptT &fake, const Tensor &ref_u8, const Tensor &face6,
                     const Tensor &gt) {
    const c10::DeviceGuard guard(src.device());
    const at::Device dev = src.device();
    f32(src, dev, "lipsync src"); f32(face6, dev, "lipsync face6");
    f32(gt, dev, "lipsync gt");
    same_dev(ref_u8, dev, "lipsync ref_u8");
    TORCH_CHECK(src.dim() == 4 && src.size(1) == 3 && src.is_contiguous(), "lipsync: src [N, 3, H, W] contiguous");
    const int64_t n = src.size(0), h = src.size(2), w = src.size(3);
    if (has(fake)) {
        f32(*fake, dev, "lipsync fake");
        TORCH_CHECK(fake->is_contiguous() && fake->sizes() == src.sizes(), "lipsync: fake like src");
    }
    TORCH_CHECK(ref_u8.scalar_type() == at::kByte && ref_u8.is_contiguous() && ref_u8.sizes() == src.sizes(),
                "lipsync: ref_u8 uint8 like src");
    TORCH_CHECK(face6.is_contiguous() && face6.dim() == 4 && face6.size(0) == n && face6.size(1) == 6 &&
                    face6.size(2) == h && face6.size(3) == w,
                "lipsync: face6 [N, 6, H, W]");
    TORCH_CHECK(gt.is_contiguous() && gt.sizes() == src.sizes(), "lipsync: gt like src");
    check(s2v_lipsync_inputs(src.data_ptr<float>(), has(fake) ? fake->data_ptr<float>() : nullptr, (int)n, (int)h, (int)w,
                             ref_u8.data_ptr<uint8_t>(), face6.data_ptr<float>(), gt.data_ptr<float>(), stream()),
          "s2v_lipsync_inputs");
}

void to_u8_(const Tensor &x, const Tensor &y, double lo, double hi, double scale, double offset) {
    const c10::DeviceGuard guard(x.device());
    f32(x, x.device(), "to_u8 x");
    same_dev(y, x.device(), "to_u8 y");
    TORCH_CHECK(x.is_contiguous() && y.is_contiguous() && y.scalar_type() == at::kByte && y.numel() == x.numel(),
                "to_u8: contiguous x and uint8 y of the same size");
    check(s2v_to_u8(x.data_ptr<float>(), x.numel(), (float)lo, (float)hi, (float)scale, (float)offset,
                    y.data_ptr<uint8_t>(), stream()),
          "s2v_to_u8");
}

void mel_chunks_(const Tensor &mel, const Tensor &starts, int64_t step, const Tensor &out) {
    const c10::DeviceGuard guard(mel.device());
    const at::Device dev = mel.device();
    f32(mel, dev, "mel_chunks mel");
    f32(out, dev, "mel_chunks out");
    same_dev(starts, dev, "mel_chunks starts");
    TORCH_CHECK(mel.dim() == 2 && mel.size(0) == 80 && mel.is_contiguous(), "mel_chunks: mel [80, frames]");
    TORCH_CHECK(starts.scalar_type() == at::kInt && starts.is_contiguous(), "mel_chunks: int32 starts");
    const int64_t nch = starts.numel();
    TORCH_CHECK(out.is_contiguous() && out.numel() == nch * 80 * step, "mel_chunks: out [n, 80, step]");
    check(s2v_mel_chunks(mel.data_ptr<float>(), mel.size(1), starts.data_ptr<int>(), (int)nch, (int)step,
                         out.data_ptr<float>(), stream()),
          "s2v_mel_chunks");
}

void melspectrogram_(const Tensor &wav, const Tensor &tables, bool pad_reflect, const Tensor &out) {
    const c10::DeviceGuard guard(wav.device());
    const at::Device dev = wav.device();
    f32(wav, dev, "mel wav");
    f32(out, dev, "mel out");
    TORCH_CHECK(wav.dim() == 1 && wav.is_contiguous(), "mel: wav [S]");
    const int64_t frames = 1 + wav.size(0) / 200;
    TORCH_CHECK(out.is_contiguous() && out.dim() == 2 && out.size(0) == 80 && out.size(1) == frames,
                "mel: out [80, 1 + S / 200]");
    vec(tables, dev, 80 * 401 + 3 * 800, "mel tables");
    check(s2v_melspectrogram(wav.data_ptr<float>(), wav.size(0), tables.data_ptr<float>(), pad_reflect,
                             out.data_ptr<float>(), frames, stream()),
          "s2v_melspectrogram");
}

}

TORCH_LIBRARY_FRAGMENT(s2v, m) {
    m.def("conv2d_(Tensor x, Tensor(a!) y, Tensor wt, Tensor? wt_split, float wt_scale, int cout, int[2] kernel, "
          "int[2] stride, int[2] padding, int[2] dilation, int in_mode, int pad_mode, int prec, Tensor? scale, "
          "Tensor? shift, Tensor? in_scale, Tensor? nc_scale, int pre_act, float pre_alpha, Tensor? pix_add, "
          "float pix_w, Tensor? res, int[2] res_offset, bool res_after_act, int act, float alpha, int out_step, "
          "bool out_pool, bool x_split, Tensor? ws, int grid_cap, int force_tile, int force_splits, "
          "Tensor(s!)? stamps, Tensor? stamp_ctr, int[3] stamp_pos, float x_scale, Tensor(f!)? nonfinite, "
          "bool dry, Tensor? post_mul=None, Tensor? post_add=None, int post_c0=0, Tensor? dup_src=None, "
          "Tensor? dup_bias=None, float dup_a=0., int dup_off=0) -> int[]");
    m.def("modulated_conv2d_(Tensor x, Tensor(a!) y, Tensor wt, Tensor s, Tensor? d, Tensor(b!) wbuf, int cout, "
          "int[2] kernel, int[2] padding, int in_mode, int prec, bool x_split, Tensor? scale, Tensor? shift, "
          "Tensor? pix_add, "
          "float pix_w, Tensor? res, "
          "bool res_after_act, int act, float alpha, Tensor? ws, int force_splits, Tensor(s!)? stamps, Tensor? stamp_ctr, "
          "int[3] stamp_pos, float x_scale, Tensor(f!)? nonfinite, bool dry, int d2s=0, int force_tile=0, "
          "float premod=0.) -> int[]");
    m.def("modulate_weights_(Tensor wt, Tensor s, Tensor? d, Tensor(a!) wbuf, int cout, int cin, int taps, int prec, "
          "float wscale) -> ()");
    m.def("amax_(Tensor x, Tensor(a!) out) -> ()");
    m.def("group_begin_() -> ()", &group_begin_);
    m.def("group_abort_() -> ()", &group_abort_);
    m.def("group_end_(Tensor? ws, bool dry) -> int[]", &group_end_);
    m.def("gemm_kn_(Tensor a, Tensor b, Tensor(a!) out, int batch, int a_bs, int b_bs, int out_bs, Tensor? res, "
          "int res_bs, int act, float alpha, int prec, Tensor? ws, int force_tile, int force_splits, bool dry) -> int[]");
    m.def("split_weights_(Tensor w, Tensor(a!) out, int prec, float scale) -> ()");
    m.def("split_act_(Tensor x, Tensor(a!) out, int prec) -> ()");
    m.def("layernorm2d_(Tensor x, Tensor weight, Tensor bias, float eps, int act, float alpha, bool pool, "
          "Tensor? res, Tensor(a!) y, Tensor? ws) -> int");
    m.def("instnorm_(Tensor x, Tensor? gamma, Tensor? beta, float eps, int act, float alpha, Tensor? res, "
          "Tensor(a!) y, Tensor(b!)? pad_out, Tensor? ws) -> int");
    m.def("adain_params_(Tensor hid, int nhidden, Tensor w2t, Tensor bias, Tensor seg, Tensor(a!) out) -> ()");
    m.def("modconv_demod_(Tensor s, Tensor wsq, Tensor(a!) d, float eps, float post) -> ()");
    m.def("modconv_demod_rows_(Tensor s, Tensor rows, Tensor wsq, Tensor(a!) d, float eps, float post, "
          "int s_reach) -> ()");
    m.def("row_layernorm_(Tensor x, Tensor weight, Tensor bias, float eps, Tensor(a!) y) -> ()");
    m.def("attention_(Tensor q, Tensor k, Tensor v, Tensor(a!) out, int batch, int heads, int tokens, int dim_head, "
          "float scale) -> ()");
    m.def("resize_(Tensor x, int x_off, int[4] x_size, int[4] x_stride, Tensor(a!) y, int y_off, int[4] y_size, "
          "int[4] y_stride, float scale_h, float scale_w, int mode) -> ()");
    m.def("pad_reflect_(Tensor x, Tensor(a!) y, int[4] pads) -> ()");
    m.def("row_pack_(Tensor x, Tensor(a!) y, int kw, int pw) -> ()");
    m.def("torgb_up2_(Tensor x, Tensor wt, Tensor s, Tensor? bias, Tensor skip, Tensor(a!) y) -> ()");
    m.def("flow_warp_(Tensor flow, Tensor src, Tensor(a!) y) -> ()");
    m.def("flow_warp_cat_(Tensor flow, Tensor src, Tensor(a!) y) -> ()");
    m.def("fill_value_(Tensor(a!) y, float value) -> ()");
    m.def("gaussian_noise_(Tensor(a!) y, int seed, int offset, Tensor? ctr, int shift) -> ()");
    m.def("counter_add_(Tensor(a!) ctr, int inc) -> ()");
    m.def("rfft2_(Tensor x, Tensor tables, Tensor(a!) spec) -> ()");
    m.def("irfft2_(Tensor spec, Tensor tables, Tensor? res, Tensor(a!) y) -> ()");
    m.def("ffc_spec_fwd_(Tensor x_g, Tensor w1, float wt_scale, float x_scale, Tensor? scale, Tensor? shift, "
          "Tensor tables, Tensor(a!) t1, Tensor(b!) spec, Tensor? flag, int prec) -> ()");
    m.def("ffc_spec_inv_(Tensor spec, Tensor wfu, float wt_scale, float x_scale, Tensor? scale, Tensor? shift, "
          "Tensor tables, Tensor t1, Tensor(a!) u, Tensor? flag, int prec) -> ()");
    m.def("ffc_norm_(Tensor(c!) y, Tensor u, Tensor w2, float wt_scale, float x_scale, Tensor? gamma, Tensor? beta, "
          "float eps, int act, float alpha, Tensor? res, Tensor(a!) out, Tensor(b!)? pad_out, Tensor? flag, int prec) -> ()");
    m.def("eltwise_(Tensor x, Tensor? mul, Tensor? add, Tensor? bias, float a, int act, float alpha, float post, "
          "Tensor(a!) y) -> ()");
    m.def("fir2d_(Tensor x, Tensor kernel, Tensor(a!) y, int up, int down, int pad_y0, int pad_x0, float gain, "
          "Tensor? bias, int act, float alpha, float post) -> ()");
    m.def("lipsync_inputs_(Tensor src, Tensor? fake, Tensor(a!) ref_u8, Tensor(b!) face6, Tensor(c!) gt) -> ()");
    m.def("to_u8_(Tensor x, Tensor(a!) y, float lo, float hi, float scale, float offset) -> ()");
    m.def("mel_chunks_(Tensor mel, Tensor starts, int step, Tensor(a!) out) -> ()");
    m.def("melspectrogram_(Tensor wav, Tensor tables, bool pad_reflect, Tensor(a!) out) -> ()");
}

TORCH_LIBRARY_IMPL(s2v, CUDA, m) {
    m.impl("conv2d_", &conv2d_);
    m.impl("modulated_conv2d_", &modulated_conv2d_);
    m.impl("modulate_weights_", &modulate_weights_);
    m.impl("gemm_kn_", &gemm_kn_);
    m.impl("split_weights_", &split_weights_);
    m.impl("amax_", &amax_);
    m.impl("split_act_", &split_act_);
    m.impl("layernorm2d_", &layernorm2d_);
    m.impl("instnorm_", &instnorm_);
    m.impl("adain_params_", &adain_params_);
    m.impl("modconv_demod_", &modconv_demod_);
    m.impl("modconv_demod_rows_", &modconv_demod_rows_);
    m.impl("row_layernorm_", &row_layernorm_);
    m.impl("attention_", &attention_);
    m.impl("resize_", &resize_);
    m.impl("pad_reflect_", &pad_reflect_);
    m.impl("row_pack_", &row_pack_);
    m.impl("torgb_up2_", &torgb_up2_);
    m.impl("flow_warp_", &flow_warp_);
    m.impl("flow_warp_cat_", &flow_warp_cat_);
    m.impl("fill_value_", &fill_value_);
    m.impl("gaussian_noise_", &gaussian_noise_);
    m.impl("counter_add_", &counter_add_);
    m.impl("rfft2_", &rfft2_);
    m.impl("irfft2_", &irfft2_);
    m.impl("ffc_spec_fwd_", &ffc_spec_fwd_);
    m.impl("ffc_spec_inv_", &ffc_spec_inv_);
    m.impl("ffc_norm_", &ffc_norm_);
    m.impl("eltwise_", &eltwise_);
    m.impl("fir2d_", &fir2d_);
    m.impl("lipsync_inputs_", &lipsync_inputs_);
    m.impl("to_u8_", &to_u8_);
    m.impl("mel_chunks_", &mel_chunks_);
    m.impl("melspectrogram_", &melspectrogram_);
}
```

speech-to-video-mpp_amd/csrc/torgb.hip:

```cpp
#include "common.hpp"

namespace s2v {

__device__ __forceinline__ void up2_index(int dst, int in, int &i0, int &i1, float &l0, float &l1) {
    float src = 0.5f * ((float)dst + 0.5f) - 0.5f;
    if (src < 0.f) src = 0.f;
    i0 = (int)src;
    i1 = i0 + ((i0 < in - 1) ? 1 : 0);
    l1 = src - (float)i0;
    l0 = 1.f - l1;
}

template <int TPP, int PPT>
__global__ __launch_bounds__(256) void torgb_up2_kernel(const float *__restrict__ x, int C, int H, int W, int xcs,
                                                        const float *__restrict__ wt, int kpad,
                                                        const float *__restrict__ s, int s_ns,
                                                        const float *__restrict__ bias,
                                                        const float *__restrict__ skip, int skcs,
                                                        float *__restrict__ y, int ycs) {
    extern __shared__ __attribute__((aligned(16))) float wm[];
    constexpr int SLOTS = 256 / TPP, PB = SLOTS * PPT;
    const int hw = H * W;
    const unsigned blk = xcd_block(blockIdx.x, gridDim.x);
    const long long q0 = (long long)blk * PB;
    const int b = (int)(q0 / hw);
    for (int e = threadIdx.x; e < 3 * C; e += 256) {
        const int o = e / C, c = e - o * C;
        wm[e] = wt[(long long)o * kpad + c] * s[(long long)b * s_ns + c];
    }
    __syncthreads();
    const int sub = threadIdx.x % TPP, slot = threadIdx.x / TPP;
    const float *xb = x + (long long)b * hw * xcs;
    const int p0 = (int)(q0 - (long long)b * hw) + slot;
    float acc[PPT][3];
#pragma unroll
    for (int i = 0; i < PPT; ++i) acc[i][0] = acc[i][1] = acc[i][2] = 0.f;
    for (int c = sub * 4; c < C; c += 4 * TPP) {
        const float4 w0 = *(const float4 *)&wm[c], w1 = *(const float4 *)&wm[C + c], w2 = *(const float4 *)&wm[2 * C + c];
        float4 v[PPT];
#pragma unroll
        for (int i = 0; i < PPT; ++i) v[i] = *(const float4 *)(xb + (long long)(p0 + i * SLOTS) * xcs + c);
#pragma unroll
        for (int i = 0; i < PPT; ++i) {
            acc[i][0] = fmaf(v[i].x, w0.x, fmaf(v[i].y, w0.y, fmaf(v[i].z, w0.z, fmaf(v[i].w, w0.w, acc[i][0]))));
            acc[i][1] = fmaf(v[i].x, w1.x, fmaf(v[i].y, w1.y, fmaf(v[i].z, w1.z, fmaf(v[i].w, w1.w, acc[i][1]))));
            acc[i][2] = fmaf(v[i].x, w2.x, fmaf(v[i].y, w2.y, fmaf(v[i].z, w2.z, fmaf(v[i].w, w2.w, acc[i][2]))));
        }
    }
#pragma unroll
    for (int i = 0; i < PPT; ++i)
#pragma unroll
        for (int o = 0; o < 3; ++o)
#pragma unroll
            for (int off = TPP / 2; off > 0; off >>= 1) acc[i][o] += __shfl_xor(acc[i][o], off, 64);
#pragma unroll
    for (int i = 0; i < PPT; ++i) {
        if (sub != i % TPP) continue;
        const int p = p0 + i * SLOTS;
        const int oy = p / W, ox = p - (p / W) * W;
        const int sh = H / 2, sw = W / 2;
        int y0, y1, x0, x1;
        float ly0, ly1, lx0, lx1;
        up2_index(oy, sh, y0, y1, ly0, ly1);
        up2_index(ox, sw, x0, x1, lx0, lx1);
        const float *sb = skip + (long long)b * sh * sw * skcs;
        const float4 ta = *(const float4 *)(sb + ((long long)y0 * sw + x0) * skcs);
        const float4 tb = *(const float4 *)(sb + ((long long)y0 * sw + x1) * skcs);
        const float4 tc = *(const float4 *)(sb + ((long long)y1 * sw + x0) * skcs);
        const float4 td = *(const float4 *)(sb + ((long long)y1 * sw + x1) * skcs);
        float4 u;
        u.x = ly0 * (lx0 * ta.x + lx1 * tb.x) + ly1 * (lx0 * tc.x + lx1 * td.x);
        u.y = ly0 * (lx0 * ta.y + lx1 * tb.y) + ly1 * (lx0 * tc.y + lx1 * td.y);
        u.z = ly0 * (lx0 * ta.z + lx1 * tb.z) + ly1 * (lx0 * tc.z + lx1 * td.z);
        u.w = ly0 * (lx0 * ta.w + lx1 * tb.w) + ly1 * (lx0 * tc.w + lx1 * td.w);
        float4 r;
        r.x = (acc[i][0] + (bias ? bias[0] : 0.f)) + u.x;
        r.y = (acc[i][1] + (bias ? bias[1] : 0.f)) + u.y;
        r.z = (acc[i][2] + (bias ? bias[2] : 0.f)) + u.z;
        r.w = u.w;
        *(float4 *)(y + ((long long)b * hw + p) * ycs) = r;
    }
}

template <int PPT>
static void launch_torgb(unsigned grid, size_t smem, const float *x, int c, int h, int w, int xcs, const float *wt,
                         int kpad, const float *s, int s_ns, const float *bias, const float *skip, int skcs, float *y,
                         int ycs, hipStream_t st) {
    torgb_up2_kernel<8, PPT><<<grid, 256, smem, st>>>(x, c, h, w, xcs, wt, kpad, s, s_ns, bias, skip, skcs, y, ycs);
}

}

using namespace s2v;

extern "C" int s2v_torgb_up2(const float *x, int n, int h, int w, int c, int xcs, const float *wt, int kpad,
                             const float *s, int s_ns, const float *bias, const float *skip, int skcs, float *y,
                             int ycs, s2v_stream_t stream) {
    S2V_REQUIRE(x && wt && s && skip && y && n > 0 && h > 1 && w > 1 && c > 0, "torgb_up2: bad args");
    S2V_REQUIRE(h % 2 == 0 && w % 2 == 0, "torgb_up2: output %dx%d must be twice the skip size", h, w);
    S2V_REQUIRE(c % 32 == 0 && xcs % 4 == 0 && xcs >= c && kpad >= c && s_ns >= c && skcs % 4 == 0 && skcs >= 4 &&
                    ycs % 4 == 0 && ycs >= 4,
                "torgb_up2: C %% 32 == 0, 4-channel skip / output, float4 pitches required");
    S2V_REQUIRE(((uintptr_t)x % 16) == 0 && ((uintptr_t)skip % 16) == 0 && ((uintptr_t)y % 16) == 0,
                "torgb_up2: 16-byte aligned x / skip / y");
    const long long hw = (long long)h * w, total = (long long)n * hw;
    int ppt = 16 / (c / 32);
    if (ppt < 1) ppt = 1;
    if (ppt > 4) ppt = 4;
    while (ppt > 1 && hw % (32LL * ppt) != 0) ppt >>= 1;
    S2V_REQUIRE(hw % (32LL * ppt) == 0, "torgb_up2: h * w must be a multiple of 32 (blocks stay in one sample)");
    const unsigned grid = (unsigned)(total / (32LL * ppt));
    const size_t smem = (size_t)3 * c * sizeof(float);
    hipStream_t st = (hipStream_t)stream;
    switch (ppt) {
        case 4: launch_torgb<4>(grid, smem, x, c, h, w, xcs, wt, kpad, s, s_ns, bias, skip, skcs, y, ycs, st); break;
        case 2: launch_torgb<2>(grid, smem, x, c, h, w, xcs, wt, kpad, s, s_ns, bias, skip, skcs, y, ycs, st); break;
        default: launch_torgb<1>(grid, smem, x, c, h, w, xcs, wt, kpad, s, s_ns, bias, skip, skcs, y, ycs, st); break;
    }
    return check_launch("torgb_up2");
}
```

speech-to-video-mpp_amd/engine/enet.py:

```python
from __future__ import annotations

import math
import os

import torch

from .. import ops
from ..ops import NHWC, ConvW
from .lnet import LNetEngine

LRELU = 0.2
OVERLAP = os.environ.get("S2V_ENET_OVERLAP", "1") == "1"
FUSED_TORGB = os.environ.get("S2V_ENET_FUSED_TORGB", "1") == "1"
POLY_UP = os.environ.get("S2V_ENET_POLY_UP", "1") == "1"
POLY_UP4 = os.environ.get("S2V_ENET_POLY_UP4", "0") == "1"
STYLE_GRID = os.environ.get("S2V_ENET_STYLE_GRID", "half")
ROWPACK0 = os.environ.get("S2V_ENET_ROWPACK0", "0") == "1"
FORK_AT = int(os.environ.get("S2V_ENET_FORK_AT", "0"))
PAUSE = tuple(int(v) for v in os.environ.get("S2V_ENET_PAUSE", "").split(":")) if os.environ.get("S2V_ENET_PAUSE") else None
PREMOD = os.environ.get("S2V_ENET_PREMOD", "1") == "1"
STACK_STRIPS = os.environ.get("S2V_ENET_STACK_STRIPS", "1") == "1"
RESUME_GRID = os.environ.get("S2V_ENET_RESUME_GRID", "")


def style_grid(device) -> int:
    if STYLE_GRID == "half":
        return ops.half_chip_blocks(device)
    return int(STYLE_GRID)

_FOLD = (((0.75, 0.25, 0.0), (0.25, 0.75, 0.75), (0.0, 0.0, 0.25)),
         ((0.25, 0.0, 0.0), (0.75, 0.75, 0.25), (0.0, 0.25, 0.75)))


def fold_up2_conv3(w: torch.Tensor) -> torch.Tensor:
    f = torch.tensor(_FOLD, dtype=torch.float64)
    wd = w.double()
    return torch.cat([torch.einsum("ap,bq,oipq->oiab", f[ry], f[rx], wd) for ry in (0, 1) for rx in (0, 1)]).float()


class StyleLayer:

    def __init__(self, sd, p, device, demodulate, upsample, is_rgb):
        m = p + "modulated_conv."
        w = sd[m + "weight"].float()[0]
        self.k = w.shape[-1]
        if w.shape[1] == 3:
            w = ops.pad_cin(w, 4)
        self.cin, self.cout = w.shape[1], w.shape[0]
        self.demodulate, self.upsample, self.is_rgb = demodulate, upsample, is_rgb
        bias = sd[p + "bias"].float().reshape(-1)
        self.conv = ConvW(w, bias, device, padding=self.k // 2)
        self.wsq = w.pow(2).sum((2, 3)).contiguous().to(device)
        self.mod_w = sd[m + "modulation.weight"].float()
        self.mod_b = sd[m + "modulation.bias"].float()
        if self.mod_w.shape[0] < self.cin:
            self.mod_w = torch.cat([self.mod_w, torch.zeros(self.cin - self.mod_w.shape[0], self.mod_w.shape[1])])
            self.mod_b = torch.cat([self.mod_b, torch.zeros(self.cin - self.mod_b.shape[0])])
        self.noise_w = None if is_rgb else float(sd[p + "weight"].float().reshape(-1)[0])
        self.device = device
        self.conv4 = self.wsq4 = None
        if upsample and self.k == 3 and (self.cin % 32 == 0 or (POLY_UP4 and self.cin == 4)):
            self.conv4 = ConvW(fold_up2_conv3(w), bias.repeat(4), device, padding=1)
            self.wsq4 = self.wsq.repeat(4, 1).contiguous()
        self.rp = None
        if ROWPACK0 and self.conv4 is None and not is_rgb and self.k == 3 and self.cin * self.k <= 32:
            self.conv.make_rowpack(device)
            self.rp = self.conv.rowpack.cin
            self.conv.rowpack.shift = self.conv.shift


class ENetEngine:
    def __init__(self, sd, device):
        dev = torch.device(device)
        self.device = dev
        self.lnet = LNetEngine(sd, dev, prefix="low_res.")
        self.first = ConvW(ops.pad_cin(sd["conv_body_first.weight"].float(), 4), sd["conv_body_first.bias"], dev)
        self.down = []
        for i in range(6):
            p = f"conv_body_down.{i}."
            sw = sd[p + "skip.weight"].float()
            skip2 = (sw / 4.0).expand(-1, -1, 2, 2).contiguous()
            self.down.append((ConvW(sd[p + "conv1.weight"], sd[p + "conv1.bias"], dev, padding=1),
                              ConvW(sd[p + "conv2.weight"], sd[p + "conv2.bias"], dev, padding=1),
                              ConvW(skip2, None, dev, stride=2)))
        self.final_conv = ConvW(sd["final_conv.weight"], sd["final_conv.bias"], dev, padding=1)
        wl = sd["final_linear.weight"].float()
        c4 = sd["final_conv.weight"].shape[0]
        wl = wl.reshape(wl.shape[0], c4, 4, 4).permute(0, 2, 3, 1).reshape(wl.shape[0], -1)
        self.final_linear = ConvW(wl, sd["final_linear.bias"], dev)
        self.layers = []
        for i in range(2):
            self.layers.append(StyleLayer(sd, f"style_convs.{2 * i}.", dev, True, True, False))
            self.layers.append(StyleLayer(sd, f"style_convs.{2 * i + 1}.", dev, True, False, False))
            self.layers.append(StyleLayer(sd, f"to_rgbs.{i}.", dev, False, False, True))
        offs, o, ws, bs = [], 0, [], []
        for l in self.layers:
            offs.append(o)
            mw, mb = l.mod_w, l.mod_b
            if l.rp is not None:
                z = l.rp - l.k * l.cin
                mw = torch.cat([mw] * l.k + [torch.zeros(z, mw.shape[1])])
                mb = torch.cat([mb] * l.k + [torch.zeros(z)])
            pad = (-mw.shape[0]) % 4
            ws += [mw, torch.zeros(pad, l.mod_w.shape[1])]
            bs += [mb, torch.zeros(pad)]
            o += mw.shape[0] + pad
        self.mod = ConvW(torch.cat(ws, 0), torch.cat(bs, 0), dev)
        self.mod_offs = offs
        self._demod = {}
        self.noise_seed = 0x5EED
        self.last_noises = [None] * 4

    def _side(self, ctx):
        side = ctx.streams(("enet", id(self)), 1)
        return None if side is None else side[0]

    def _demod_table(self, poly):
        if poly not in self._demod:
            ls = [(self.mod_offs[j], self.layers[j].wsq4 if poly and self.layers[j].conv4 is not None
                   else self.layers[j].wsq) for j in (0, 1, 3, 4)]
            t = ops.DemodRows(ls, self.device)
            t.width = [w.shape[0] for _, w in ls]
            self._demod[poly] = t
        return self._demod[poly]

    def _demods(self, ctx, s2):
        t = self._demod_table(POLY_UP)
        dall = ops.empty((s2.shape[0], t.nrows), self.device)
        ops.modconv_demod_rows(ctx, s2, t, dall, eps=1e-8, post=math.sqrt(2.0))
        return t, dall

    def _premodulate(self, ctx, s2, dtab, dall, b) -> dict:
        wb = {}
        for st in range(2):
            for li in range(2):
                L, idx = self.layers[3 * st + li], 2 * st + li
                off = self.mod_offs[3 * st + li]
                r0, wd = dtab.r0[idx], dtab.width[idx]
                sv = s2[:, off: off + L.cin]
                if L.cin <= 4:
                    continue
                if POLY_UP and L.conv4 is not None:
                    d4 = dall[:, r0: r0 + wd]
                    wb[idx] = {"conv4": ops.modulate_weights(ctx, L.conv4, sv, d4, b),
                               "conv": ops.modulate_weights(ctx, L.conv, sv, d4[:, : L.cout], b)}
                elif L.rp is None:
                    wb[idx] = {"conv": ops.modulate_weights(ctx, L.conv, sv, dall[:, r0: r0 + L.cout], b)}
        return wb

    def _poly_styleconv(self, ctx, L, cur: NHWC, s, d4, idx, noises, ctr, wb=None):
        dev, b = self.device, cur.n
        h2, w2 = 2 * cur.h, 2 * cur.w
        d = d4[:, : L.cout]
        noise = None
        if L.noise_w:
            if noises is not None and noises[idx] is not None:
                noise = noises[idx].reshape(b, h2, w2).contiguous()
            else:
                noise = torch.empty((b, h2, w2), device=dev)
                ops.gaussian_noise(ctx, noise, self.noise_seed, idx << 36, ctr=ctr, shift=40)
                self.last_noises[idx] = noise
        y = NHWC.empty(b, h2, w2, L.cout, dev)
        kw = dict(act=ops.ACT_LRELU, alpha=LRELU, pix_w=L.noise_w or 0.0)
        wb = wb or {}
        ops.modulated_conv2d(ctx, cur, L.conv4, y, s, d4, pix_add=noise, d2s=True, premod=wb.get("conv4"), **kw)
        c = cur.c
        if STACK_STRIPS:
            for axis, n_src, n_out in ((1, cur.h, h2), (2, cur.w, w2)):
                xs = NHWC(torch.cat([cur.t.narrow(axis, 0, 2), cur.t.narrow(axis, n_src - 2, 2)], axis))
                up = NHWC.empty(b, 2 * xs.h, 2 * xs.w, c, dev)
                ops.resize_nhwc(ctx, xs, up, scale_factor=2)
                ys = NHWC.empty(b, up.h, up.w, L.cout, dev)
                nz = None if noise is None else torch.cat([noise.narrow(axis, 0, 4), noise.narrow(axis, n_out - 4, 4)],
                                                          axis)
                ops.modulated_conv2d(ctx, up, L.conv, ys, s, d, pix_add=nz, premod=wb.get("conv"), **kw)
                y.t.narrow(axis, 0, 2).copy_(ys.t.narrow(axis, 0, 2))
                y.t.narrow(axis, n_out - 2, 2).copy_(ys.t.narrow(axis, 6, 2))
            return y
        strips = ((cur.t[:, 0:2], lambda t: t[:, 0:4], lambda t: t[:, 0:2], lambda t: t[:, 0:2]),
                  (cur.t[:, cur.h - 2:], lambda t: t[:, h2 - 4:], lambda t: t[:, 2:4], lambda t: t[:, h2 - 2:]),
                  (cur.t[:, :, 0:2], lambda t: t[:, :, 0:4], lambda t: t[:, :, 0:2], lambda t: t[:, :, 0:2]),
                  (cur.t[:, :, cur.w - 2:], lambda t: t[:, :, w2 - 4:], lambda t: t[:, :, 2:4],
                   lambda t: t[:, :, w2 - 2:]))
        for xs_t, nsel, ssel, ysel in strips:
            xs = NHWC(xs_t.contiguous())
            up = NHWC.empty(b, 2 * xs.h, 2 * xs.w, c, dev)
            ops.resize_nhwc(ctx, xs, up, scale_factor=2)
            ys = NHWC.empty(b, up.h, up.w, L.cout, dev)
            nz = None if noise is None else nsel(noise).contiguous()
            ops.modulated_conv2d(ctx, up, L.conv, ys, s, d, pix_add=nz, premod=wb.get("conv"), **kw)
            ysel(y.t).copy_(ssel(ys.t))
        return y

    def style_code(self, ctx, ref: torch.Tensor):
        st = self.style_begin(ctx, ref)
        self.style_down(ctx, st, len(self.down))
        return self.style_end(ctx, st)

    def style_begin(self, ctx, ref: torch.Tensor) -> dict:
        dev, b = self.device, ref.shape[0]
        x = NHWC.empty(b, 256, 256, 4, dev)
        ops.fill(ctx, x.t)
        ops.nchw_to_nhwc(ctx, ref, x.slice(0, 3))
        f = NHWC.empty(b, 256, 256, self.first.cout, dev)
        ops.conv2d(ctx, x, self.first, f, act=ops.ACT_LRELU, alpha=LRELU)
        return {"f": f, "i": 0}

    def style_down(self, ctx, st: dict, upto: int):
        f, b, dev = st["f"], st["f"].n, self.device
        while st["i"] < min(upto, len(self.down)):
            c1, c2, sk = self.down[st["i"]]
            h, w = f.h, f.w
            td = NHWC.empty(b, h // 2, w // 2, c1.cout, dev)
            ops.conv2d(ctx, f, c1, td, act=ops.ACT_LRELU, alpha=LRELU, pool=True)
            out = NHWC.empty(b, h // 2, w // 2, c2.cout, dev)
            ops.conv2d(ctx, f, sk, out)
            ops.conv2d(ctx, td, c2, out, act=ops.ACT_LRELU, alpha=LRELU, res=out, res_after=True)
            f = out
            st["i"] += 1
        st["f"] = f

    def style_end(self, ctx, st: dict):
        f, b, dev = st["f"], st["f"].n, self.device
        g = NHWC.empty(b, f.h, f.w, self.final_conv.cout, dev)
        ops.conv2d(ctx, f, self.final_conv, g, act=ops.ACT_LRELU, alpha=LRELU)
        style = NHWC.empty(b, 1, 1, self.final_linear.cout, dev)
        ops.conv2d(ctx, NHWC(g.t.view(b, 1, 1, -1)), self.final_linear, style)
        return style

    def forward(self, ctx, audio, face, gt, out: torch.Tensor, low: torch.Tensor, noises=None, aux=None):
        dev = self.device
        b = audio.shape[0]
        svec = NHWC.empty(b, 1, 1, self.mod.cout, dev)
        side = self._side(ctx) if OVERLAP else None
        enc = {}

        def finish(sctx):
            enc["style"] = self.style_end(sctx, enc.pop("st"))
            ops.conv2d(sctx, enc["style"], self.mod, svec)
            enc["d"] = self._demods(sctx, svec.t.view(b, -1))
            if PREMOD:
                enc["wb"] = self._premodulate(sctx, svec.t.view(b, -1), enc["d"][0], enc["d"][1], b)

        def fork():
            sst, sctx = side
            sst.wait_stream(torch.cuda.current_stream(dev))
            with ops.x3_grid_cap(sctx, style_grid(dev)), ops.side_stream(sst, ctx.keep):
                enc["st"] = self.style_begin(sctx, face[:, 3:])
                self.style_down(sctx, enc["st"], PAUSE[0] if PAUSE else len(self.down))
                if not PAUSE:
                    finish(sctx)

        def resume():
            sst, sctx = side
            sst.wait_stream(torch.cuda.current_stream(dev))
            grid = int(RESUME_GRID) if RESUME_GRID else style_grid(dev)
            with ops.x3_grid_cap(sctx, grid), ops.side_stream(sst, ctx.keep):
                self.style_down(sctx, enc["st"], len(self.down))
                finish(sctx)

        on_level = None
        if side is not None:
            if FORK_AT:
                on_level = lambda h: fork() if h == FORK_AT and not enc else None
            else:
                fork()
                if PAUSE and PAUSE[1]:
                    on_level = lambda h: resume() if h == PAUSE[1] and "st" in enc else None
        else:
            enc["style"] = self.style_code(ctx, face[:, 3:])
            ops.conv2d(ctx, enc["style"], self.mod, svec)
            enc["d"] = self._demods(ctx, svec.t.view(b, -1))
        x6 = NHWC.empty(b, 96, 96, 6, dev)
        ops.nchw_to_nhwc(ctx, face[:, :3], x6.slice(0, 3))
        ops.nchw_to_nhwc(ctx, gt, x6.slice(3, 3))
        lo = NHWC.empty(b, 96, 96, 4, dev)
        self.lnet.forward(ctx, audio, x6, lo, pad_rgb=True, on_level=on_level)
        if side is not None and not enc:
            fork()
        if side is not None and "st" in enc:
            resume()
        ops.nhwc_to_nchw(ctx, lo.slice(0, 3), low)
        if side is not None:
            torch.cuda.current_stream(dev).wait_stream(side[0])
        style, (dtab, dall) = enc["style"], enc["d"]
        s2 = svec.t.view(b, -1)
        if aux is not None:
            aux["style"] = style.t.view(b, -1)
        cur = NHWC.empty(b, 100, 100, 4, dev)
        ops.pad_reflect(ctx, lo, cur, (2, 2, 2, 2))
        skip = cur
        ctr = None
        self.last_noises = [None] * 4
        if noises is None and any(L.noise_w for L in self.layers):
            ctr = ctx.noise(id(self)).bump(ctx)
        for st in range(2):
            for li in range(2):
                L = self.layers[3 * st + li]
                off = self.mod_offs[3 * st + li]
                r0, wd = dtab.r0[2 * st + li], dtab.width[2 * st + li]
                if POLY_UP and L.conv4 is not None:
                    cur = self._poly_styleconv(ctx, L, cur, s2[:, off: off + L.cin], dall[:, r0: r0 + wd],
                                               2 * st + li, noises, ctr, wb=enc.get("wb", {}).get(2 * st + li))
                    continue
                x = cur
                if L.upsample:
                    x = NHWC.empty(b, 2 * cur.h, 2 * cur.w, cur.c, dev)
                    ops.resize_nhwc(ctx, cur, x, scale_factor=2)
                conv, cin = L.conv, L.cin
                if L.rp is not None:
                    xp = NHWC.empty(b, x.h, x.w, L.rp, dev)
                    ops.row_pack(ctx, x, xp, L.k, L.k // 2)
                    x, conv, cin = xp, L.conv.rowpack, L.rp
                d = dall[:, r0: r0 + L.cout]
                y = NHWC.empty(b, x.h, x.w, L.cout, dev)
                noise = None
                if L.noise_w:
                    if noises is not None and noises[2 * st + li] is not None:
                        noise = noises[2 * st + li].contiguous()
                    else:
                        noise = torch.empty((b, x.h, x.w), device=dev)
                        ops.gaussian_noise(ctx, noise, self.noise_seed, (2 * st + li) << 36, ctr=ctr, shift=40)
                        self.last_noises[2 * st + li] = noise
                pm = enc.get("wb", {}).get(2 * st + li, {}).get("conv") if L.rp is None else None
                ops.modulated_conv2d(ctx, x, conv, y, s2[:, off: off + cin], d, act=ops.ACT_LRELU, alpha=LRELU,
                                     pix_add=noise, pix_w=L.noise_w or 0.0, premod=pm)
                cur = y
            R = self.layers[3 * st + 2]
            off = self.mod_offs[3 * st + 2]
            rgb = NHWC.empty(b, cur.h, cur.w, 4, dev)
            if FUSED_TORGB and R.cin % 32 == 0 and (cur.h * cur.w) % 32 == 0:
                ops.torgb_up2(ctx, cur, R.conv, s2[:, off: off + R.cin], skip, rgb)
            else:
                ops.resize_nhwc(ctx, skip, rgb, scale_factor=2)
                ops.modulated_conv2d(ctx, cur, R.conv, rgb.slice(0, 3), s2[:, off: off + R.cin], res=rgb.slice(0, 3))
            skip = rgb
        ops.nhwc_to_nchw(ctx, skip.slice(0, 3), out, crop=(8, 8))
        return out, low
```

speech-to-video-mpp_amd/ops.py:

```python
from __future__ import annotations

import contextlib
import ctypes
import math
import os
import threading
import weakref

import torch

from . import _lib, torch_ops
from ._lib import (ACT_GELU_TANH, ACT_LRELU, ACT_NONE, ACT_RELU, ACT_SIGMOID, ACT_TANH,
                   IN_DIRECT, IN_NEAREST_UP2, IN_TRANSPOSED, PAD_REFLECT, PAD_ZERO, PREC_BF16X3, PREC_F16, PREC_F16X3, PREC_F32,
                   check)

F32 = 4

_PRECISIONS = {"f16x3": PREC_F16X3, "bf16x3": PREC_BF16X3, "f32": PREC_F32, "f16": PREC_F16}
SPLIT_PRECISIONS = ("f16x3", "bf16x3")
PRECISION = os.environ.get("S2V_PRECISION", "f16x3")
if PRECISION not in _PRECISIONS:
    raise ValueError(f"S2V_PRECISION must be one of {sorted(_PRECISIONS)}, got {PRECISION!r}")


# ... 347 lines not shown
            for rx in range(2):
                sub = torch.einsum("ap,bq,oipq->oiab", f[ry], f[rx], w).float()
                cw = ConvW(sub, None, device, padding=(1 - ry, 1 - rx))
                cw.scale, cw.shift = self.scale, self.shift
                plans.append(((ry, rx), cw, (ry, rx)))
        self.poly = plans
        return self

    def make_rowpack(self, device):
        assert self.in_mode == IN_DIRECT and (self.sh, self.sw, self.dh, self.dw) == (1, 1, 1, 1)
        assert self.pad_mode == PAD_ZERO and self.cin * self.kw <= 64 and 2 * self.pw + 1 == self.kw
        w = self.wt[: self.cout, : self.K].cpu().reshape(self.cout, self.kh, self.kw, self.cin)
        cp = (self.kw * self.cin + 31) // 32 * 32
        wp = torch.zeros(self.cout, cp, self.kh, 1)
        wp[:, : self.kw * self.cin, :, 0] = w.permute(0, 2, 3, 1).reshape(self.cout, self.kw * self.cin, self.kh)
        cw = ConvW(wp, None, device, padding=(self.ph, 0))
        cw.scale, cw.shift = self.scale, self.shift
        self.rowpack = cw
        return self

    rowpack = None

    def out_hw(self, h, w):
        if self.in_mode == IN_TRANSPOSED:
            return ((h - 1) * self.sh - 2 * self.ph + self.dh * (self.kh - 1) + self.oph + 1,
                    (w - 1) * self.sw - 2 * self.pw + self.dw * (self.kw - 1) + self.opw + 1)
        if self.in_mode == IN_NEAREST_UP2:
            h, w = 2 * h, 2 * w
        return ((h + 2 * self.ph - self.dh * (self.kh - 1) - 1) // self.sh + 1,
                (w + 2 * self.pw - self.dw * (self.kw - 1) - 1) // self.sw + 1)


def _ptr(t):
    return None if t is None else t.data_ptr()


def conv2d(ctx: Ctx, x: NHWC, cw: ConvW, y: NHWC, *, act=ACT_NONE, alpha=0.0, res: NHWC | None = None,
           res_after=False, res_offset=(0, 0), nc_scale=None, in_scale=None, pre_act=ACT_NONE, pre_alpha=0.0,
           pix_add=None, pix_w=0.0, scale=None, shift=None, force_tile=0, force_splits=0, pool=False, post=None,
           dup=None):
    assert (post is None and dup is None) or (cw.rowpack is None and getattr(cw, "poly", None) is None), \
        "conv: post / dup epilogues on plain (not row-packed, not polyphase) convs only"
    if cw.rowpack is not None:
        assert x.c == cw.cin, f"conv: input has {x.c} channels, weights expect {cw.cin}"
        assert in_scale is None, "row-packed conv: no input scale"
        xp = NHWC.empty(x.n, x.h, x.w, cw.rowpack.cin, x.t.device)
        row_pack(ctx, x, xp, cw.kw, cw.pw)
        return conv2d(ctx, xp, cw.rowpack, y, act=act, alpha=alpha, res=res, res_after=res_after, res_offset=res_offset,
                      nc_scale=nc_scale, in_scale=None, pre_act=pre_act, pre_alpha=pre_alpha, pix_add=pix_add,
                      pix_w=pix_w, scale=scale, shift=shift, force_tile=force_tile, force_splits=force_splits, pool=pool)
    if getattr(cw, "poly", None) is not None:
        assert pix_add is None, "polyphase transposed conv: no pix_add epilogue"
        assert res is None or (res.t.data_ptr() == y.t.data_ptr() and res.coff == y.coff and not res_after), \
            "polyphase transposed conv: only an in-place residual (res is the output view)"
        oh, ow = cw.out_hw(x.h, x.w)
        assert (y.n, y.h, y.w, y.c) == (x.n, oh, ow, cw.cout), "conv_transpose: output view mismatch"
        grouped = cw.in_mode == IN_NEAREST_UP2 and x.n * x.h * x.w <= UP2_GROUP_PIXELS and not force_tile
        with conv_group(ctx, enabled=grouped):
            for (ry, rx), sub, _ in cw.poly:
                if (oh - ry + 1) // 2 <= 0 or (ow - rx + 1) // 2 <= 0:
                    continue
                yc = y.t[:, ry::2, rx::2, y.coff: y.coff + y.c]
                _conv(ctx, x, sub, yc, 2, act, alpha, yc if res is not None else None, False, (0, 0), nc_scale,
                      in_scale, pre_act, pre_alpha, None, 0.0, scale, shift, force_tile, force_splits)
        return y
    oh, ow = cw.out_hw(x.h, x.w)
    assert x.c == cw.cin, f"conv: input has {x.c} channels, weights expect {cw.cin}"
    f = 2 if pool else 1
    assert (y.n, y.h * f, y.w * f, y.c) == (x.n, oh, ow, cw.cout), \
        f"conv: output view {(y.n, y.h, y.w, y.c)} != {(x.n, oh // f, ow // f, cw.cout)}"
    extra = {}
    if post is not None:
        pm, pa, c0 = post
        assert (pm.n, pm.h, pm.w, pm.c) == (y.n, y.h, y.w, cw.cout - c0) and (pa.n, pa.h, pa.w, pa.c) == (pm.n, pm.h,
                                                                                                         pm.w, pm.c)
        extra.update(post_mul=pm.v, post_add=pa.v, post_c0=int(c0))
    if dup is not None:
        ds, db, da, off = dup
        assert (ds.n, ds.h, ds.w, ds.c) == (y.n, y.h, y.w, cw.cout)
        assert y.coff == 0 and off >= cw.cout and off + cw.cout <= y.cs, "dup: second output inside y's pixel pitch"
        extra.update(dup_src=ds.v, dup_bias=db, dup_a=float(da), dup_off=int(off))
    _conv(ctx, x, cw, y.v, 1, act, alpha, None if res is None else res.v, res_after, res_offset, nc_scale, in_scale,
          pre_act, pre_alpha, pix_add, pix_w, scale, shift, force_tile, force_splits, pool=pool, extra=extra)
    return y


def _conv_flops(x, cw, yv, pool):
    oh, ow = (yv.shape[1], yv.shape[2])
    if pool:
        oh, ow = 2 * oh, 2 * ow
    pix = x.n * x.h * x.w if cw.in_mode == IN_TRANSPOSED else x.n * oh * ow
    return 2.0 * pix * cw.kh * cw.kw * cw.cin * cw.cout


def conv_key(x, cw, yv, out_step, pool, prec) -> str:
    return (f"x{x.n}x{x.h}x{x.w}x{x.c}c{x.cs}|k{cw.kh}x{cw.kw}s{cw.sh}x{cw.sw}p{cw.ph}x{cw.pw}d{cw.dh}x{cw.dw}"
            f"m{cw.in_mode}{cw.pad_mode}|y{yv.shape[1]}x{yv.shape[2]}x{cw.cout}c{yv.stride(2)}|o{out_step}{int(pool)}"
            f"|p{prec}")


def _conv(ctx, x, cw, yv, out_step, act, alpha, resv, res_after, res_offset, nc_scale, in_scale, pre_act, pre_alpha,
          pix_add, pix_w, scale, shift, force_tile, force_splits, pool=False, extra=None):
    prec = prec_code()
    x_split = int(getattr(x, "split", 0))
    if x_split and x_split != layout_code(prec):
        raise _lib.S2VError(f"conv: the input holds the split layout of precision code {x_split}, but the conv runs "
                            f"in {PRECISION!r} (code {prec}); split it again with split_act after set_precision")
    wsplit = cw.wt_x3(ctx, prec) if prec != PREC_F32 else None
    wscale = cw.split_scale(prec)
    xscale, flag = _range(ctx, cw, x, prec, in_scale)
    cap = int(getattr(ctx, "grid_cap", 0))
    sc = cw.scale if scale is None else scale
    sh = cw.shift if shift is None else shift
    key = None
    if (PERFDB or TUNE is not None) and prec != PREC_F32 and not (force_tile or force_splits or x_split or cap or
                                                                   _grouping()):
        key = conv_key(x, cw, yv, out_step, pool, layout_code(prec))
        if TUNE is None and perfdb_applies(x.t.device):
            force_tile, force_splits = PERFDB.get(key, (0, 0))

    def launch(ws, dry=False, st=_NOSTAMP, ft=None, fs=None):
        return S2V.conv2d_(x.v, yv, cw.wt, wsplit, wscale, cw.cout, [cw.kh, cw.kw], [cw.sh, cw.sw], [cw.ph, cw.pw],
                           [cw.dh, cw.dw], cw.in_mode, cw.pad_mode, prec, sc, sh, in_scale, nc_scale, pre_act, pre_alpha,
                           pix_add, pix_w, resv, list(res_offset), res_after, act, alpha, out_step, pool, x_split != 0,
                           ws, cap, force_tile if ft is None else ft, force_splits if fs is None else fs, st[0], st[1],
                           st[2], xscale, flag, dry, **(extra or {}))
    if TUNE is not None and key is not None:
        TUNE(ctx, key, lambda ft, fs: _with_ws(ctx, lambda ws: launch(ws, False, _NOSTAMP, ft, fs)[0]),
             lambda ft, fs: launch(ctx.ws.tensor(), True, _NOSTAMP, ft, fs)[1:], yv, resv)
    _run_conv(ctx, launch, x, cw, yv, pool, in_scale, nc_scale, pix_add, resv)


@contextlib.contextmanager
def conv_group(ctx: Ctx, enabled: bool = True):
    if not enabled or CONV_HOOK is not None:
        yield
        return
    S2V.group_begin_()
    _TLS.grouping = True
    try:
        yield
    except BaseException:
        S2V.group_abort_()
        raise
    finally:
        _TLS.grouping = False
    global LAST_GROUP
    res = []

    def end(ws):
        r = S2V.group_end_(ws, False)
        res[:] = r
        return r[0]
    try:
        _with_ws(ctx, end)
    except BaseException:
        S2V.group_abort_()
        raise
    LAST_GROUP = res[1] if len(res) > 1 else 0


def check_all_ranges(what="s2v"):
    for c in list(Ctx.ALL):
        c.check_range(what)


def guard_active() -> bool:
    return RANGE_GUARD and PRECISION in ("f16x3", "f16")


class _Calibration:
    SLOTS = 4096

    def __init__(self, device):
        self.device = device
        self.bufs = [torch.zeros(self.SLOTS, device=device)]
        self.n = 0
        self.items = []

    def slot(self):
        if self.n == len(self.bufs) * self.SLOTS:
            self.bufs.append(torch.zeros(self.SLOTS, device=self.device))
        i = self.n
        self.n += 1
        return i, self.bufs[i // self.SLOTS][i % self.SLOTS: i % self.SLOTS + 1]


def _root(ctx):
    while getattr(ctx, "parent", None) is not None:
        ctx = ctx.parent
    return ctx


def _amax_into(t: torch.Tensor, out: torch.Tensor):
    if t.dim() == 2:
        n, c = t.shape
        t = t.as_strided((1, 1, n, c), (n * t.stride(0), n * t.stride(0), t.stride(0), 1))
    S2V.amax_(t, out)


CALIB_PASSES = 4


def begin_calibration(ctx):
    _root(ctx).calib = _Calibration(ctx.device)


def end_forward(ctx, calibrating: bool) -> str:
    root = _root(ctx)
    cal = getattr(root, "calib", None) if calibrating else None
    root.calib = None
    flag = root._flag
    vals = [b.cpu() for b in cal.bufs] if cal is not None else []
    bad = bool(int(flag.item())) if flag is not None else False
    if flag is not None and bad:
        flag.zero_()
    scaled = False
    if cal is not None:
        per = {}
        for cw, prec, xs, ss in cal.items:
            m = float(vals[xs // _Calibration.SLOTS][xs % _Calibration.SLOTS])
            if ss >= 0:
                m *= float(vals[ss // _Calibration.SLOTS][ss % _Calibration.SLOTS])
            key = (id(cw), prec)
            per[key] = (cw, prec, max(per[key][2], m) if key in per else m)
        recal = False
        for cw, prec, m in per.values():
            if not math.isfinite(m):
                recal = True
                continue
            sc = x_scale_for(m)
            cw.__dict__.setdefault("_xscale", {})[prec] = sc
            cw.x_amax = m
            scaled = scaled or sc != 1.0
        if recal:
            return "recalibrate"
    if scaled:
        return "scaled"
    return "overflow" if bad else ""


def _range(ctx, cw, x, prec, in_scale=None):
    if layout_code(prec) != PREC_F16X3 or not RANGE_GUARD or int(getattr(x, "split", 0)):
        return 1.0, None
    scales = cw.__dict__.setdefault("_xscale", {})
    s = scales.get(prec)
    if s is None:
        if x.t.is_cuda and torch.cuda.is_current_stream_capturing():
            raise _lib.S2VError("activation ranges must be calibrated by an eager run before graph capture")
        cal = getattr(_root(ctx), "calib", None)
        if cal is not None:
            xs, out = cal.slot()
            _amax_into(x.v, out)
            ss = -1
            if in_scale is not None:
                ss, out2 = cal.slot()
                _amax_into(in_scale, out2)
            cal.items.append((cw, prec, xs, ss))
            return 1.0, ctx.range_flag()
        m = torch.zeros(2, device=x.t.device)
        _amax_into(x.v, m[0:1])
        if in_scale is not None:
            _amax_into(in_scale, m[1:2])
        mv = m.cpu()
        amax = float(mv[0]) * (float(mv[1]) if in_scale is not None else 1.0)
        s = x_scale_for(amax)
        scales[prec] = s
        cw.x_amax = amax
    return s, ctx.range_flag()


def _run_conv(ctx, launch, x, cw, yv, pool, in_scale=None, nc_scale=None, pix_add=None, resv=None):
    st = _NOSTAMP

    def go():
        _with_ws(ctx, lambda ws: launch(ws, False, st)[0])
    if CONV_HOOK is None and STAMP is None:
        go()
        return
    plan = launch(ctx.ws.tensor(), True)[1:]
    oh, ow = yv.shape[1] * (2 if pool else 1), yv.shape[2] * (2 if pool else 1)
    info = ConvLaunch(plan, n=x.n, h=x.h, w=x.w, cin=x.c, oh=oh, ow=ow, cout=cw.cout, kh=cw.kh, kw=cw.kw,
                      in_scale=in_scale is not None, nc_scale=nc_scale is not None, pix_add=pix_add is not None,
                      res=resv is not None, res_is_y=resv is not None and resv.data_ptr() == yv.data_ptr())
    flops = _conv_flops(x, cw, yv, pool)
    if STAMP is not None and not _grouping():
        st = STAMP(info, flops) or _NOSTAMP
    if CONV_HOOK is None:
        go()
    else:
        CONV_HOOK(ctx, info, flops, go)


def modulate_weights(ctx: Ctx, cw: ConvW, s: torch.Tensor, d: torch.Tensor | None, batch: int):
    prec = prec_code()
    wbuf = empty((batch, cw.npad, cw.kpad), cw.wt.device)
    wscale = 2048.0 if (layout_code(prec) == PREC_F16X3 and d is not None) else 1.0
    S2V.modulate_weights_(cw.wt, s, d, wbuf, cw.cout, cw.cin, cw.kh * cw.kw, layout_code(prec), wscale)
    return wbuf, (wscale if prec != PREC_F32 else -1.0)


def modulated_conv2d(ctx: Ctx, x: NHWC, cw: ConvW, y: NHWC, s: torch.Tensor, d: torch.Tensor | None = None, *,
                     act=ACT_NONE, alpha=0.0, res: NHWC | None = None, res_after=False, pix_add=None, pix_w=0.0,
                     shift=None, force_splits=0, d2s=False, premod=None):
    oh, ow = cw.out_hw(x.h, x.w)
    assert cw.in_mode != IN_TRANSPOSED and cw.poly is None and (cw.sh, cw.sw, cw.dh, cw.dw) == (1, 1, 1, 1), \
        "modulated_conv2d: direct stride-1 convs only"
    if d2s:
        assert x.c == cw.cin and cw.cout % 4 == 0 and res is None and (y.n, y.h, y.w, y.c) == (x.n, 2 * oh, 2 * ow,
                                                                                             cw.cout // 4)
    else:
        assert x.c == cw.cin and (y.n, y.h, y.w, y.c) == (x.n, oh, ow, cw.cout)
    if premod is not None:
        wbuf, pm = premod
        assert tuple(wbuf.shape) == (x.n, cw.npad, cw.kpad), "modulated_conv2d: premod weights of another shape"
    else:
        wbuf, pm = torch.empty((x.n, cw.npad, cw.kpad), device=cw.wt.device), 0.0
    yv, resv = y.v, None if res is None else res.v
    prec = prec_code()
    x_split = int(getattr(x, "split", 0))
    if x_split and x_split != layout_code(prec):
        raise _lib.S2VError(f"modulated conv: the input holds the split layout of precision code {x_split}, but the "
                            f"conv runs in {PRECISION!r} (code {prec})")
    sh = cw.shift if shift is None else shift
    xscale, flag = _range(ctx, cw, x, prec)
    key, force_tile = None, 0
    if (PERFDB or TUNE is not None) and prec != PREC_F32 and not (force_splits or x_split):
        key = conv_key(x, cw, yv, 1, False, layout_code(prec)) + f"|mod{int(d is not None)}{int(d2s)}"
        if TUNE is None and perfdb_applies(x.t.device):
            force_tile, force_splits = PERFDB.get(key, (0, 0))

    def launch(ws, dry=False, st=_NOSTAMP, ft=None, fs=None):
        return S2V.modulated_conv2d_(x.v, yv, cw.wt, s, d, wbuf, cw.cout, [cw.kh, cw.kw], [cw.ph, cw.pw], cw.in_mode,
                                     prec,
                                     x_split != 0, cw.scale, sh, pix_add, pix_w, resv, res_after, act, alpha, ws,
                                     force_splits if fs is None else fs, st[0], st[1], st[2], xscale, flag, dry, int(d2s),
                                     force_tile if ft is None else ft, pm)
    if TUNE is not None and key is not None:
        TUNE(ctx, key, lambda ft, fs: _with_ws(ctx, lambda ws: launch(ws, False, _NOSTAMP, ft, fs)[0]),
             lambda ft, fs: launch(ctx.ws.tensor(), True, _NOSTAMP, ft, fs)[1:], yv, resv)
    _run_conv(ctx, launch, x, cw, yv[:, ::2, ::2, :] if d2s else yv, False, pix_add=pix_add, resv=resv)
    return y


def gemm_kn(ctx: Ctx, a: torch.Tensor, b: torch.Tensor, out: torch.Tensor, *, batch: int, a_bs: int, b_bs: int,
            out_bs: int, res: torch.Tensor | None = None, res_bs: int = 0, act=ACT_NONE, alpha=0.0,
            force_tile=0, force_splits=0):
    prec = prec_code()
    _with_ws(ctx, lambda ws: S2V.gemm_kn_(a, b, out, batch, a_bs, b_bs, out_bs, res, res_bs, act, alpha, prec, ws,
                                          force_tile, force_splits, False)[0])
    return out


def _plan(ctx: Ctx, p):
    out = (ctypes.c_int * 11)()
    check(ctx.lib.s2v_conv2d_plan(ctypes.byref(p), out), "s2v_conv2d_plan")
    return list(out)


def plan_symbol(plan) -> str:
    bm, bn, wm, avec, bkn, splits, x3, nw, ks, pf = plan[:10]
    persist = plan[10] if len(plan) > 10 else 0
    if avec == 5:
        return f"void s2v::conv_glds_x3<{bm}, {bn}, {wm}, {ks}, {x3 - 1}>(s2v::ConvArgs)"
    if avec in (6, 7):
        return f"void s2v::conv_x3_nar<{x3 - 1}, {avec - 6}>(s2v::ConvArgs)"
    if avec == 8:
        return f"void s2v::conv_x3_halo<{x3 - 1}, {bm // 64}, {bn // 64}>(s2v::ConvArgs)"
    if bm == 0:
        if wm < 0:
            if bkn >= 2000:
                return f"void s2v::conv_smallk4<{-wm}, {bkn - 2000}>(s2v::ConvArgs, int, int, int, int)"
            return f"void s2v::conv_smallk<{-wm}, {avec}>(s2v::ConvArgs, int, int, int, int)"
        if bkn >= 4000:
            return f"void s2v::conv_k4_mfma<{bkn - 4000}, false>(s2v::ConvArgs, int)"
        if bkn >= 3000:
            return f"void s2v::conv_head_x3<{x3 - 1}, {bn}, {bkn - 3000}, {wm}>(s2v::ConvArgs, int, int)"
        if bkn >= 1000:
            return f"void s2v::conv_halo_small<{bn}, {bkn - 1000}>(s2v::ConvArgs, int, int)"
        if wm:
            return f"void s2v::conv_small_cpar<{bn}, {wm}, {'true' if avec else 'false'}>(s2v::ConvArgs, int)"
        return f"void s2v::conv_direct_small<{bn}>(s2v::ConvArgs, int)"
    if x3:
        name = "conv_igemm_x3_persist" if persist else "conv_igemm_x3"
        return f"void s2v::{name}<{bm}, {bn}, {wm}, {nw}, {ks}, {pf}, {avec}, {bkn}, {x3 - 1}>(s2v::ConvArgs)"
    return f"void s2v::conv_igemm<{bm}, {bn}, {wm}, {avec}, {bkn}>(s2v::ConvArgs)"


def conv_symbol(ctx: Ctx, p) -> str:
    return plan_symbol(p.plan if isinstance(p, ConvLaunch) else _plan(ctx, p))


def split_act(ctx: Ctx, x: NHWC, out: NHWC | None = None) -> NHWC:
    prec = layout_code(prec_code())
    assert prec != PREC_F32, "split_act needs a split precision (f16x3 / bf16x3 / f16)"
    if out is None:
        out = NHWC.empty(x.n, x.h, x.w, x.c, x.t.device)
    assert (out.n, out.h, out.w, out.c) == (x.n, x.h, x.w, x.c) and out.coff == 0
    S2V.split_act_(x.v, out.v, prec)
    out.split = prec
    return out


(TUNE_HALO_MIN_BLOCKS, TUNE_GLDS_TILE, TUNE_SMALLK_TILE, TUNE_X3_RATE_512, TUNE_IN_FUSED,
 TUNE_RESIZE_UP2) = (0, 1, 2, 3, 4, 5)


def tune(ctx: Ctx, key: int, value: int) -> int:
    old = ctypes.c_longlong(0)
    check(ctx.lib.s2v_tune(key, value, ctypes.byref(old)), "s2v_tune")
    return old.value


@contextlib.contextmanager
def tuned(ctx: Ctx, key: int, value: int):
    if not value:
        yield
        return
    old = tune(ctx, key, value)
    try:
        yield
    finally:
        tune(ctx, key, old)


@contextlib.contextmanager
def x3_grid_cap(ctx: Ctx, blocks: int):
    prev = getattr(ctx, "grid_cap", 0)
    ctx.grid_cap = max(0, int(blocks)) // 8 * 8
    try:
        yield
    finally:
        ctx.grid_cap = prev


def half_chip_blocks(device) -> int:
    cus = torch.cuda.get_device_properties(torch.device(device)).multi_processor_count
    return max(8, cus // 2 // 8 * 8)


def conv_splits(ctx: Ctx, p) -> int:
    return (p.plan if isinstance(p, ConvLaunch) else _plan(ctx, p))[5]


def layernorm2d(ctx: Ctx, x: NHWC, weight, bias, y: NHWC, *, act=ACT_LRELU, alpha=0.1, pool=False,
                res: NHWC | None = None, eps=1e-5):
    rv = None if res is None else res.v
    _with_ws(ctx, lambda ws: S2V.layernorm2d_(x.v, weight, bias, eps, act, alpha, pool, rv, y.v, ws))
    return y


def instnorm(ctx: Ctx, x: NHWC, y: NHWC, gamma=None, beta=None, *, act=ACT_NONE, alpha=0.0,
             res: NHWC | None = None, eps=1e-5, pad_out: NHWC | None = None):
    if pad_out is not None:
        assert (pad_out.n, pad_out.h, pad_out.w, pad_out.c) == (x.n, x.h + 2, x.w + 2, x.c)
    rv, pv = None if res is None else res.v, None if pad_out is None else pad_out.v
    _with_ws(ctx, lambda ws: S2V.instnorm_(x.v, gamma, beta, eps, act, alpha, rv, y.v, pv, ws))
    return y


def adain_params(ctx: Ctx, hid: torch.Tensor, nhidden: int, w2t: torch.Tensor, bias: torch.Tensor, seg: torch.Tensor,
                 out: torch.Tensor):
    S2V.adain_params_(hid, nhidden, w2t, bias, seg, out)
    return out


def modconv_demod(ctx: Ctx, s: torch.Tensor, wsq: torch.Tensor, out: torch.Tensor, *, eps=1e-8, post=1.0):
    S2V.modconv_demod_(s, wsq, out, eps, post)
    return out


class DemodRows:

    def __init__(self, layers, device):
        rows, ws, r0, w_off, reach = [], [], [], 0, 0
        for s_off, wsq in layers:
            cout, cin = wsq.shape
            r0.append(len(rows))
            rows += [(s_off, cin, w_off + o * cin, 0) for o in range(cout)]
            ws.append(wsq.reshape(-1).float().cpu())
            w_off += cout * cin
            reach = max(reach, s_off + cin)
        assert w_off < 2 ** 31, "demod table: squared weights past int32 offsets"
        self.rows = torch.tensor(rows, dtype=torch.int32).to(device)
        self.wsq = torch.cat(ws).contiguous().to(device)
        self.r0, self.nrows, self.s_reach = r0, len(rows), reach


def modconv_demod_rows(ctx: Ctx, s: torch.Tensor, table: DemodRows, out: torch.Tensor, *, eps=1e-8, post=1.0):
    S2V.modconv_demod_rows_(s, table.rows, table.wsq, out, eps, post, table.s_reach)
    return out


def torch_bilinear_scale(in_size: int, out_size: int, scale_factor=None) -> float:
    if scale_factor is not None and scale_factor > 0:
        return float(torch.tensor(1.0 / scale_factor, dtype=torch.float32))
    return float(torch.tensor(in_size, dtype=torch.float32) / out_size)


def resize(ctx: Ctx, x: torch.Tensor, x_off: int, x_shape, x_strides, y: torch.Tensor, y_off: int, y_hw, y_strides, *,
           scale_factor=None, mode=0):
    n, c, ih, iw = x_shape
    oh, ow = y_hw
    sh = torch_bilinear_scale(ih, oh, scale_factor) if mode == 0 else (
        float(torch.tensor(1.0 / scale_factor, dtype=torch.float32)) if scale_factor else ih / oh)
    sw = torch_bilinear_scale(iw, ow, scale_factor) if mode == 0 else (
        float(torch.tensor(1.0 / scale_factor, dtype=torch.float32)) if scale_factor else iw / ow)
    S2V.resize_(x, x_off, [n, c, ih, iw], list(x_strides), y, y_off, [n, c, oh, ow], list(y_strides), sh, sw, mode)


def nhwc_strides(v: NHWC):
    return (v.h * v.w * v.cs, 1, v.w * v.cs, v.cs)


def resize_nhwc(ctx: Ctx, x: NHWC, y: NHWC, scale_factor=None, mode=0):
    resize(ctx, x.t, x.coff, (x.n, x.c, x.h, x.w), nhwc_strides(x), y.t, y.coff, (y.h, y.w), nhwc_strides(y),
           scale_factor=scale_factor, mode=mode)
    return y


def nchw_to_nhwc(ctx: Ctx, x: torch.Tensor, y: NHWC, size=None):
    _require_cuda(x, "nchw_to_nhwc")
    resize(ctx, x, 0, tuple(x.shape), x.stride(), y.t, y.coff, (y.h, y.w), nhwc_strides(y))
    return y


def nhwc_to_nchw(ctx: Ctx, x: NHWC, out: torch.Tensor, crop=(0, 0)):
    n, c, oh, ow = out.shape
    off = x.coff + (crop[0] * x.w + crop[1]) * x.cs
    resize(ctx, x.t, off, (n, c, oh, ow), nhwc_strides(x), out, 0, (oh, ow), out.stride())
    return out


def torgb_up2(ctx: Ctx, x: NHWC, cw: "ConvW", s: torch.Tensor, skip: NHWC, y: NHWC):
    assert cw.kh == cw.kw == 1 and cw.cout == 3 and x.c == cw.cin, "torgb_up2: a 1x1 conv to 3 channels"
    assert (y.n, y.h, y.w, y.c) == (x.n, x.h, x.w, 4) and (skip.n, 2 * skip.h, 2 * skip.w, skip.c) == (x.n, x.h, x.w, 4)
    S2V.torgb_up2_(x.v, cw.wt, s, cw.shift, skip.v, y.v)
    return y


def row_pack(ctx: Ctx, x: NHWC, y: NHWC, kw: int, pw: int):
    S2V.row_pack_(x.v, y.v, kw, pw)
    return y


def pad_reflect(ctx: Ctx, x: NHWC, y: NHWC, pads):
    S2V.pad_reflect_(x.v, y.v, list(pads))
    return y


def row_layernorm(ctx: Ctx, x: torch.Tensor, weight, bias, y: torch.Tensor, eps=1e-5):
    S2V.row_layernorm_(x, weight, bias, eps, y)
    return y


def attention(ctx: Ctx, q: torch.Tensor, k: torch.Tensor, v: torch.Tensor, out: torch.Tensor, *, batch, heads,
              tokens, dim_head=64, scale=None):
    scale = dim_head ** -0.5 if scale is None else scale
    S2V.attention_(q, k, v, out, batch, heads, tokens, dim_head, scale)
    return out


def flow_warp(ctx: Ctx, flow: NHWC, src: torch.Tensor, y: NHWC):
    S2V.flow_warp_(flow.v, src, y.v)
    return y


def flow_warp_cat(ctx: Ctx, flow: NHWC, src: torch.Tensor, y: NHWC):
    S2V.flow_warp_cat_(flow.v, src, y.v)
    return y


def fill(ctx: Ctx, t: torch.Tensor, value: float = 0.0):
    S2V.fill_value_(t, value)
    return t


def pad_cin(w: torch.Tensor, cin: int) -> torch.Tensor:
    if w.shape[1] >= cin:
        return w
    z = torch.zeros((w.shape[0], cin - w.shape[1]) + tuple(w.shape[2:]), dtype=w.dtype)
    return torch.cat([w, z], 1)


def _i64(v: int) -> int:
    v &= 2 ** 64 - 1
    return v - 2 ** 64 if v >= 2 ** 63 else v


def gaussian_noise(ctx: Ctx, out: torch.Tensor, seed: int, offset: int = 0, ctr: torch.Tensor | None = None,
                   shift: int = 40):
    S2V.gaussian_noise_(out, _i64(seed), _i64(offset), ctr, shift)
    return out


class NoiseCounter:

    def __init__(self):
        self.t = None

    def bump(self, ctx: Ctx) -> torch.Tensor:
        if self.t is None:
            if ctx.device.type == "cuda" and torch.cuda.is_current_stream_capturing():
                raise _lib.S2VError("noise counter must be created by an eager run before graph capture")
            self.t = torch.zeros(1, dtype=torch.int64, device=ctx.device)
        S2V.counter_add_(self.t, 1)
        return self.t


_DFT_CACHE = {}


def fourier_matrices(h: int, w: int, device):
    key = (h, w, str(device))
    if key not in _DFT_CACHE:
        P, wf = h * w, w // 2 + 1
        F = h * wf
        eye = torch.eye(P, dtype=torch.float64).reshape(P, h, w)
        spec = torch.fft.rfftn(eye, dim=(-2, -1), norm="ortho").reshape(P, F)
        d2 = torch.stack([spec.real, spec.imag], -1).reshape(P, 2 * F).t()
        basis = torch.zeros(2 * F, F, dtype=torch.complex128)
        idx = torch.arange(F)
        basis[2 * idx, idx] = 1.0
        basis[2 * idx + 1, idx] = 1.0j
        iv = torch.fft.irfftn(basis.reshape(2 * F, h, wf), s=(h, w), dim=(-2, -1), norm="ortho")
        iv = iv.reshape(2 * F, P).t()
        _DFT_CACHE[key] = (d2.float().contiguous().to(device), iv.float().contiguous().to(device))
    return _DFT_CACHE[key]


def fir2d(ctx: Ctx, x: NHWC, kernel: torch.Tensor, y: NHWC, *, up=1, down=1, pad0=(0, 0), gain=1.0, bias=None,
          act=ACT_NONE, alpha=0.0, post=1.0):
    assert x.n == y.n and x.c == y.c, "fir2d: batch / channel mismatch"
    S2V.fir2d_(x.v, kernel, y.v, up, down, pad0[0], pad0[1], gain, bias, act, alpha, post)
    return y


def eltwise(ctx: Ctx, x: NHWC, y: NHWC, *, a=1.0, mul: NHWC | None = None, add: NHWC | None = None, bias=None,
            act=ACT_NONE, alpha=0.0, post=1.0):
    assert (x.n, x.h, x.w, x.c) == (y.n, y.h, y.w, y.c)
    for v in (mul, add):
        assert v is None or (v.n, v.h, v.w, v.c) == (x.n, x.h, x.w, x.c)
    S2V.eltwise_(x.v, None if mul is None else mul.v, None if add is None else add.v, bias, a, act, alpha, post, y.v)
    return y


_FFT_TABLES = {}


def fft_tables(h: int, w: int, device):
    key = (h, w, str(device))
    if key not in _FFT_TABLES:
        wf = w // 2 + 1
        rw = torch.fft.rfft(torch.eye(w, dtype=torch.float64), dim=1, norm="ortho")
        fw = torch.stack([rw.real, rw.imag], 1)
        fhc = torch.fft.fft(torch.eye(h, dtype=torch.complex128), dim=1, norm="ortho")
        fh = torch.stack([fhc.real, fhc.imag], 1)
        ihc = torch.fft.ifft(torch.eye(h, dtype=torch.complex128), dim=1, norm="ortho")
        ih = torch.stack([ihc.real, ihc.imag], 1)
        eye = torch.eye(wf, dtype=torch.float64)
        cre = torch.fft.irfft(torch.complex(eye, torch.zeros_like(eye)), n=w, dim=1, norm="ortho")
        cim = torch.fft.irfft(torch.complex(torch.zeros_like(eye), eye), n=w, dim=1, norm="ortho")
        iw = torch.stack([cre, cim], 1)
        t = torch.cat([fw.reshape(-1), fh.reshape(-1), ih.reshape(-1), iw.reshape(-1)]).float().contiguous()
        assert t.numel() == 2 * wf * w + 4 * h * h + 2 * w * wf
        _FFT_TABLES[key] = t.to(device)
    return _FFT_TABLES[key]


def ffc_fused_ok() -> bool:
    return PRECISION in ("f16x3", "bf16x3", "f16")


def ffc_spec_fwd(ctx: Ctx, xg: NHWC, cw: ConvW, tables: torch.Tensor, t1: NHWC, spec: torch.Tensor):
    prec = layout_code(prec_code())
    xs, flag = _range(ctx, cw, xg, prec)
    S2V.ffc_spec_fwd_(xg.v, cw.wt_x3(ctx, prec), cw.split_scale(prec), xs, cw.scale, cw.shift, tables, t1.v, spec,
                      flag, prec)
    return t1, spec


def ffc_spec_inv(ctx: Ctx, spec: torch.Tensor, cw: ConvW, tables: torch.Tensor, t1: NHWC, u: NHWC):
    prec = layout_code(prec_code())
    b, f, c2 = spec.shape
    xs, flag = _range(ctx, cw, NHWC(spec.view(b, f, 1, c2)), prec)
    S2V.ffc_spec_inv_(spec, cw.wt_x3(ctx, prec), cw.split_scale(prec), xs, cw.scale, cw.shift, tables, t1.v, u.v, flag,
                      prec)
    return u


def ffc_norm(ctx: Ctx, y: NHWC, u: NHWC, cw: ConvW, out: NHWC, gamma=None, beta=None, *, act=ACT_NONE, alpha=0.0,
             res: NHWC | None = None, eps=1e-5, pad_out: NHWC | None = None):
    prec = layout_code(prec_code())
    xs, flag = _range(ctx, cw, u, prec)
    S2V.ffc_norm_(y.v, u.v, cw.wt_x3(ctx, prec), cw.split_scale(prec), xs, gamma, beta, eps, act, alpha,
                  None if res is None else res.v, out.v, None if pad_out is None else pad_out.v, flag, prec)
    return out


def rfft2(ctx: Ctx, x: NHWC, tables: torch.Tensor, spec: torch.Tensor):
    S2V.rfft2_(x.v, tables, spec)
    return spec


def irfft2(ctx: Ctx, spec: torch.Tensor, tables: torch.Tensor, y: NHWC, res: NHWC | None = None):
    S2V.irfft2_(spec, tables, None if res is None else res.v, y.v)
    return y
```

Baseline: 683.8 frames/s.

## Compute only the receptive-field cone of the cropped output in the ENet tail

Adds a cropped-tail path for the final upsampling stages. Each conv and toRGB layer runs only on the window of pixels that feeds the final cropped output, using valid (zero) padding and windowed noise. The last toRGB kernel writes the cropped NCHW output directly, which removes the separate crop/layout conversion. This cuts convolution work on the high-resolution tail in exchange for extra windowing logic, and the windowed shapes skip the perf-database tuned tiles.

Result: faster. 709.2 frames/s, median of 6 (+3.7%).

```diff
diff --git a/include/s2v.h b/include/s2v.h
--- a/include/s2v.h
+++ b/include/s2v.h
@@ -120,6 +120,17 @@
 
 int s2v_torgb_up2(const float *x, int n, int h, int w, int c, int xcs, const float *wt, int kpad, const float *s,
                   int s_ns, const float *bias, const float *skip, int skcs, float *y, int ycs, s2v_stream_t stream);
+
+typedef struct s2v_torgb_win {
+    int fh, fw;
+    int oy, ox;
+    int sh, sw;
+    int sy, sx;
+    int nchw, cy, cx;
+} s2v_torgb_win;
+int s2v_torgb_up2_win(const float *x, int n, int h, int w, int c, int xcs, const float *wt, int kpad, const float *s,
+                      int s_ns, const float *bias, const float *skip, int skcs, float *y, int ycs,
+                      const s2v_torgb_win *win, s2v_stream_t stream);
 
 int s2v_row_pack(const float *x, int n, int h, int w, int c, int xcs, int kw, int pw, float *y, int ycs,
                  s2v_stream_t stream);
diff --git a/speech-to-video-mpp_amd/_lib.py b/speech-to-video-mpp_amd/_lib.py
--- a/speech-to-video-mpp_amd/_lib.py
+++ b/speech-to-video-mpp_amd/_lib.py
@@ -68,6 +68,8 @@
                                         _vp]),
     "s2v_torgb_up2": (_c_int, [_vp, _c_int, _c_int, _c_int, _c_int, _c_int, _vp, _c_int, _vp, _c_int, _vp, _vp,
                                _c_int, _vp, _c_int, _vp]),
+    "s2v_torgb_up2_win": (_c_int, [_vp, _c_int, _c_int, _c_int, _c_int, _c_int, _vp, _c_int, _vp, _c_int, _vp, _vp,
+                                   _c_int, _vp, _c_int, _vp, _vp]),
     "s2v_resize": (_c_int, [_vp, _c_int, _c_int, _c_int, _c_int, _c_ll, _c_ll, _c_ll, _c_ll, _vp, _c_int, _c_int,
                             _c_ll, _c_ll, _c_ll, _c_ll, _c_float, _c_float, _c_int, _vp]),
     "s2v_row_pack": (_c_int, [_vp, _c_int, _c_int, _c_int, _c_int, _c_int, _c_int, _c_int, _vp, _c_int, _vp]),
diff --git a/speech-to-video-mpp_amd/csrc/conv_plan.cpp b/speech-to-video-mpp_amd/csrc/conv_plan.cpp
--- a/speech-to-video-mpp_amd/csrc/conv_plan.cpp
+++ b/speech-to-video-mpp_amd/csrc/conv_plan.cpp
@@ -158,7 +158,7 @@
     if (!k4_on() || p->cin != 4 || p->kh != p->kw || (p->kh != 1 && p->kh != 3) || p->force_tile || p->b_kn || p->x_split)
         return false;
     if (p->in_mode != S2V_IN_DIRECT || p->pad_mode != S2V_PAD_ZERO || p->sh != 1 || p->sw != 1 || p->dh != 1 ||
-        p->dw != 1 || p->ph != p->kh / 2 || p->pw != p->kw / 2)
+        p->dw != 1 || !((p->ph == p->kh / 2 && p->pw == p->kw / 2) || (p->ph == 0 && p->pw == 0)))
         return false;
     if (p->cout % 32 || p->cout > 256 || p->in_scale || p->pre_act != S2V_ACT_NONE || p->nc_scale || p->res ||
         p->post_mul || p->dup_src || p->out_pool || p->out_step > 1 || p->d2s_cout > 0)
diff --git a/speech-to-video-mpp_amd/csrc/torch_launch.cpp b/speech-to-video-mpp_amd/csrc/torch_launch.cpp
--- a/speech-to-video-mpp_amd/csrc/torch_launch.cpp
+++ b/speech-to-video-mpp_amd/csrc/torch_launch.cpp
@@ -680,20 +680,45 @@
 }
 
 void torgb_up2_(const Tensor &x, const Tensor &wt, const Tensor &s, const OptT &bias, const Tensor &skip,
-                const Tensor &y) {
-    const c10::DeviceGuard guard(x.device());
-    const at::Device dev = x.device();
-    const NV xv = nhwc(x, dev, "torgb x"), kv = nhwc(skip, dev, "torgb skip"), yv = nhwc(y, dev, "torgb y");
+                const Tensor &y, at::IntArrayRef window, at::IntArrayRef crop) {
+    const c10::DeviceGuard guard(x.device());
+    const at::Device dev = x.device();
+    const NV xv = nhwc(x, dev, "torgb x"), kv = nhwc(skip, dev, "torgb skip");
     f32(wt, dev, "torgb wt");
     TORCH_CHECK(wt.dim() == 2 && wt.is_contiguous() && wt.size(0) >= 3 && wt.size(1) >= xv.c,
                 "torgb wt: packed 1x1 rows [>= 3, kpad >= C]");
     const int s_ns = (int)rows_view(s, dev, xv.n, xv.c, "torgb s");
     const float *bp = vec(bias, dev, 3, "torgb bias");
-    TORCH_CHECK(kv.n == xv.n && yv.n == xv.n && yv.h == xv.h && yv.w == xv.w && 2 * kv.h == xv.h && 2 * kv.w == xv.w &&
-                    kv.c == 4 && yv.c == 4,
-                "torgb: skip [N, H/2, W/2, 4] and y [N, H, W, 4] views expected");
-    check(s2v_torgb_up2(xv.p, xv.n, xv.h, xv.w, xv.c, xv.cs, wt.data_ptr<float>(), (int)wt.size(1), s.data_ptr<float>(),
-                        s_ns, bp, kv.p, kv.cs, yv.p, yv.cs, stream()),
+    TORCH_CHECK(window.empty() || window.size() == 6, "torgb window: (fh, fw, oy, ox, sy, sx) or empty");
+    TORCH_CHECK(crop.empty() || crop.size() == 2, "torgb crop: (cy, cx) or empty");
+    TORCH_CHECK(kv.n == xv.n && kv.c == 4, "torgb: skip [N, SH, SW, 4] view expected");
+    s2v_torgb_win win{};
+    win.sh = kv.h; win.sw = kv.w;
+    if (window.empty()) {
+        TORCH_CHECK(2 * kv.h == xv.h && 2 * kv.w == xv.w, "torgb: skip [N, H/2, W/2, 4] expected");
+        win.fh = xv.h; win.fw = xv.w;
+    } else {
+        for (int64_t v : window) TORCH_CHECK(v >= 0 && v < (1 << 30), "torgb window: bad value ", v);
+        win.fh = (int)window[0]; win.fw = (int)window[1]; win.oy = (int)window[2]; win.ox = (int)window[3];
+        win.sy = (int)window[4]; win.sx = (int)window[5];
+    }
+    float *yp = nullptr;
+    int ycs = 0;
+    if (crop.empty()) {
+        const NV yv = nhwc(y, dev, "torgb y");
+        TORCH_CHECK(yv.n == xv.n && yv.h == xv.h && yv.w == xv.w && yv.c == 4, "torgb: y [N, H, W, 4] view expected");
+        yp = yv.p; ycs = yv.cs;
+    } else {
+        f32(y, dev, "torgb y");
+        TORCH_CHECK(crop[0] >= 0 && crop[1] >= 0 && 2 * crop[0] < xv.h && 2 * crop[1] < xv.w, "torgb crop: bad (cy, cx)");
+        win.nchw = 1; win.cy = (int)crop[0]; win.cx = (int)crop[1];
+        TORCH_CHECK(y.dim() == 4 && y.is_contiguous() && y.size(0) == xv.n && y.size(1) == 3 &&
+                        y.size(2) == xv.h - 2 * win.cy && y.size(3) == xv.w - 2 * win.cx,
+                    "torgb: contiguous NCHW y [N, 3, H - 2 cy, W - 2 cx] expected, got ", y.sizes());
+        yp = y.data_ptr<float>();
+    }
+    check(s2v_torgb_up2_win(xv.p, xv.n, xv.h, xv.w, xv.c, xv.cs, wt.data_ptr<float>(), (int)wt.size(1),
+                            s.data_ptr<float>(), s_ns, bp, kv.p, kv.cs, yp, ycs, &win, stream()),
           "s2v_torgb_up2");
 }
 
@@ -1032,7 +1057,8 @@
           "int[4] y_stride, float scale_h, float scale_w, int mode) -> ()");
     m.def("pad_reflect_(Tensor x, Tensor(a!) y, int[4] pads) -> ()");
     m.def("row_pack_(Tensor x, Tensor(a!) y, int kw, int pw) -> ()");
-    m.def("torgb_up2_(Tensor x, Tensor wt, Tensor s, Tensor? bias, Tensor skip, Tensor(a!) y) -> ()");
+    m.def("torgb_up2_(Tensor x, Tensor wt, Tensor s, Tensor? bias, Tensor skip, Tensor(a!) y, int[] window, "
+          "int[] crop) -> ()");
     m.def("flow_warp_(Tensor flow, Tensor src, Tensor(a!) y) -> ()");
     m.def("flow_warp_cat_(Tensor flow, Tensor src, Tensor(a!) y) -> ()");
     m.def("fill_value_(Tensor(a!) y, float value) -> ()");
diff --git a/speech-to-video-mpp_amd/csrc/torgb.hip b/speech-to-video-mpp_amd/csrc/torgb.hip
--- a/speech-to-video-mpp_amd/csrc/torgb.hip
+++ b/speech-to-video-mpp_amd/csrc/torgb.hip
@@ -2,7 +2,7 @@
 
 namespace s2v {
 
-__device__ __forceinline__ void up2_index(int dst, int in, int &i0, int &i1, float &l0, float &l1) {
+__host__ __device__ __forceinline__ void up2_index(int dst, int in, int &i0, int &i1, float &l0, float &l1) {
     float src = 0.5f * ((float)dst + 0.5f) - 0.5f;
     if (src < 0.f) src = 0.f;
     i0 = (int)src;
@@ -11,19 +11,27 @@
     l0 = 1.f - l1;
 }
 
+
+struct TorgbGeo {
+    int fsh, fsw;
+    int oy, ox;
+    int sh, sw;
+    int sy, sx;
+    int nchw, cy, cx;
+};
+
 template <int TPP, int PPT>
 __global__ __launch_bounds__(256) void torgb_up2_kernel(const float *__restrict__ x, int C, int H, int W, int xcs,
                                                         const float *__restrict__ wt, int kpad,
                                                         const float *__restrict__ s, int s_ns,
                                                         const float *__restrict__ bias,
                                                         const float *__restrict__ skip, int skcs,
-                                                        float *__restrict__ y, int ycs) {
+                                                        float *__restrict__ y, int ycs, int chunks, TorgbGeo g) {
     extern __shared__ __attribute__((aligned(16))) float wm[];
     constexpr int SLOTS = 256 / TPP, PB = SLOTS * PPT;
     const int hw = H * W;
     const unsigned blk = xcd_block(blockIdx.x, gridDim.x);
-    const long long q0 = (long long)blk * PB;
-    const int b = (int)(q0 / hw);
+    const int b = (int)(blk / (unsigned)chunks);
     for (int e = threadIdx.x; e < 3 * C; e += 256) {
         const int o = e / C, c = e - o * C;
         wm[e] = wt[(long long)o * kpad + c] * s[(long long)b * s_ns + c];
@@ -31,15 +39,18 @@
     __syncthreads();
     const int sub = threadIdx.x % TPP, slot = threadIdx.x / TPP;
     const float *xb = x + (long long)b * hw * xcs;
-    const int p0 = (int)(q0 - (long long)b * hw) + slot;
+    const int p0 = (int)(blk - (unsigned)b * (unsigned)chunks) * PB + slot;
     float acc[PPT][3];
 #pragma unroll
     for (int i = 0; i < PPT; ++i) acc[i][0] = acc[i][1] = acc[i][2] = 0.f;
+    int pl[PPT];
+#pragma unroll
+    for (int i = 0; i < PPT; ++i) pl[i] = min(p0 + i * SLOTS, hw - 1);
     for (int c = sub * 4; c < C; c += 4 * TPP) {
         const float4 w0 = *(const float4 *)&wm[c], w1 = *(const float4 *)&wm[C + c], w2 = *(const float4 *)&wm[2 * C + c];
         float4 v[PPT];
 #pragma unroll
-        for (int i = 0; i < PPT; ++i) v[i] = *(const float4 *)(xb + (long long)(p0 + i * SLOTS) * xcs + c);
+        for (int i = 0; i < PPT; ++i) v[i] = *(const float4 *)(xb + (long long)pl[i] * xcs + c);
 #pragma unroll
         for (int i = 0; i < PPT; ++i) {
             acc[i][0] = fmaf(v[i].x, w0.x, fmaf(v[i].y, w0.y, fmaf(v[i].z, w0.z, fmaf(v[i].w, w0.w, acc[i][0]))));
@@ -57,13 +68,15 @@
     for (int i = 0; i < PPT; ++i) {
         if (sub != i % TPP) continue;
         const int p = p0 + i * SLOTS;
+        if (p >= hw) continue;
         const int oy = p / W, ox = p - (p / W) * W;
-        const int sh = H / 2, sw = W / 2;
         int y0, y1, x0, x1;
         float ly0, ly1, lx0, lx1;
-        up2_index(oy, sh, y0, y1, ly0, ly1);
-        up2_index(ox, sw, x0, x1, lx0, lx1);
-        const float *sb = skip + (long long)b * sh * sw * skcs;
+        up2_index(g.oy + oy, g.fsh, y0, y1, ly0, ly1);
+        up2_index(g.ox + ox, g.fsw, x0, x1, lx0, lx1);
+        y0 -= g.sy; y1 -= g.sy; x0 -= g.sx; x1 -= g.sx;
+        const int sw = g.sw;
+        const float *sb = skip + (long long)b * g.sh * sw * skcs;
         const float4 ta = *(const float4 *)(sb + ((long long)y0 * sw + x0) * skcs);
         const float4 tb = *(const float4 *)(sb + ((long long)y0 * sw + x1) * skcs);
         const float4 tc = *(const float4 *)(sb + ((long long)y1 * sw + x0) * skcs);
@@ -78,44 +91,95 @@
         r.y = (acc[i][1] + (bias ? bias[1] : 0.f)) + u.y;
         r.z = (acc[i][2] + (bias ? bias[2] : 0.f)) + u.z;
         r.w = u.w;
-        *(float4 *)(y + ((long long)b * hw + p) * ycs) = r;
+        if (!g.nchw) {
+            *(float4 *)(y + ((long long)b * hw + p) * ycs) = r;
+        } else {
+            const int ph = H - 2 * g.cy, pw = W - 2 * g.cx, qy = oy - g.cy, qx = ox - g.cx;
+            if ((unsigned)qy < (unsigned)ph && (unsigned)qx < (unsigned)pw) {
+                const long long plane = (long long)ph * pw;
+                float *yp = y + (long long)b * 3 * plane + (long long)qy * pw + qx;
+                yp[0] = r.x;
+                yp[plane] = r.y;
+                yp[2 * plane] = r.z;
+            }
+        }
     }
 }
 
 template <int PPT>
 static void launch_torgb(unsigned grid, size_t smem, const float *x, int c, int h, int w, int xcs, const float *wt,
                          int kpad, const float *s, int s_ns, const float *bias, const float *skip, int skcs, float *y,
-                         int ycs, hipStream_t st) {
-    torgb_up2_kernel<8, PPT><<<grid, 256, smem, st>>>(x, c, h, w, xcs, wt, kpad, s, s_ns, bias, skip, skcs, y, ycs);
+                         int ycs, int chunks, const TorgbGeo &g, hipStream_t st) {
+    torgb_up2_kernel<8, PPT><<<grid, 256, smem, st>>>(x, c, h, w, xcs, wt, kpad, s, s_ns, bias, skip, skcs, y, ycs,
+                                                      chunks, g);
+}
+
+static void up2_tap_range(int o, int len, int in, int &lo, int &hi) {
+    int i0, i1;
+    float l0, l1;
+    up2_index(o, in, i0, i1, l0, l1);
+    lo = i0;
+    up2_index(o + len - 1, in, i0, i1, l0, l1);
+    hi = i1;
 }
 
 }
 
 using namespace s2v;
 
+extern "C" int s2v_torgb_up2_win(const float *x, int n, int h, int w, int c, int xcs, const float *wt, int kpad,
+                                 const float *s, int s_ns, const float *bias, const float *skip, int skcs, float *y,
+                                 int ycs, const s2v_torgb_win *win, s2v_stream_t stream) {
+    S2V_REQUIRE(x && wt && s && skip && y && win && n > 0 && h > 1 && w > 1 && c > 0, "torgb_up2: bad args");
+    const int fh = win->fh > 0 ? win->fh : h, fw = win->fw > 0 ? win->fw : w;
+    S2V_REQUIRE(fh % 2 == 0 && fw % 2 == 0, "torgb_up2: output frame %dx%d must be twice the skip frame", fh, fw);
+    S2V_REQUIRE(win->oy >= 0 && win->ox >= 0 && win->oy + h <= fh && win->ox + w <= fw,
+                "torgb_up2: the %dx%d output window at (%d, %d) leaves the %dx%d frame", h, w, win->oy, win->ox, fh, fw);
+    S2V_REQUIRE(win->sh > 0 && win->sw > 0 && win->sy >= 0 && win->sx >= 0 && win->sy + win->sh <= fh / 2 &&
+                    win->sx + win->sw <= fw / 2,
+                "torgb_up2: the %dx%d skip window at (%d, %d) leaves the %dx%d skip frame", win->sh, win->sw, win->sy,
+                win->sx, fh / 2, fw / 2);
+    int ylo, yhi, xlo, xhi;
+    up2_tap_range(win->oy, h, fh / 2, ylo, yhi);
+    up2_tap_range(win->ox, w, fw / 2, xlo, xhi);
+    S2V_REQUIRE(ylo >= win->sy && yhi < win->sy + win->sh && xlo >= win->sx && xhi < win->sx + win->sw,
+                "torgb_up2: the output window at (%d, %d) reads skip rows %d..%d, columns %d..%d: outside the %dx%d "
+                "skip window at (%d, %d)", win->oy, win->ox, ylo, yhi, xlo, xhi, win->sh, win->sw, win->sy, win->sx);
+    S2V_REQUIRE(c % 32 == 0 && xcs % 4 == 0 && xcs >= c && kpad >= c && s_ns >= c && skcs % 4 == 0 && skcs >= 4,
+                "torgb_up2: C %% 32 == 0, 4-channel skip, float4 pitches required");
+    S2V_REQUIRE(((uintptr_t)x % 16) == 0 && ((uintptr_t)skip % 16) == 0, "torgb_up2: 16-byte aligned x / skip");
+    if (win->nchw)
+        S2V_REQUIRE(win->cy >= 0 && win->cx >= 0 && 2 * win->cy < h && 2 * win->cx < w,
+                    "torgb_up2: crop (%d, %d) leaves nothing of the %dx%d output", win->cy, win->cx, h, w);
+    else
+        S2V_REQUIRE(ycs % 4 == 0 && ycs >= 4 && ((uintptr_t)y % 16) == 0,
+                    "torgb_up2: 4-channel NHWC output, float4 pitch, 16-byte aligned y");
+    const long long hw = (long long)h * w;
+    S2V_REQUIRE(hw < (1LL << 31) && (long long)n * hw * xcs < (1LL << 62), "torgb_up2: problem too large");
+    int ppt = 16 / (c / 32);
+    if (ppt < 1) ppt = 1;
+    if (ppt > 4) ppt = 4;
+    if (hw % 32 == 0)
+        while (ppt > 1 && hw % (32LL * ppt) != 0) ppt >>= 1;
+    const long long chunks = (hw + 32LL * ppt - 1) / (32LL * ppt);
+    S2V_REQUIRE(chunks * n < (1LL << 31), "torgb_up2: grid too large");
+    const unsigned grid = (unsigned)(chunks * n);
+    const size_t smem = (size_t)3 * c * sizeof(float);
+    const TorgbGeo g{fh / 2, fw / 2, win->oy, win->ox, win->sh, win->sw, win->sy, win->sx, win->nchw ? 1 : 0,
+                     win->nchw ? win->cy : 0, win->nchw ? win->cx : 0};
+    hipStream_t st = (hipStream_t)stream;
+    switch (ppt) {
+        case 4: launch_torgb<4>(grid, smem, x, c, h, w, xcs, wt, kpad, s, s_ns, bias, skip, skcs, y, ycs, (int)chunks, g, st); break;
+        case 2: launch_torgb<2>(grid, smem, x, c, h, w, xcs, wt, kpad, s, s_ns, bias, skip, skcs, y, ycs, (int)chunks, g, st); break;
+        default: launch_torgb<1>(grid, smem, x, c, h, w, xcs, wt, kpad, s, s_ns, bias, skip, skcs, y, ycs, (int)chunks, g, st); break;
+    }
+    return check_launch("torgb_up2");
+}
+
 extern "C" int s2v_torgb_up2(const float *x, int n, int h, int w, int c, int xcs, const float *wt, int kpad,
                              const float *s, int s_ns, const float *bias, const float *skip, int skcs, float *y,
                              int ycs, s2v_stream_t stream) {
-    S2V_REQUIRE(x && wt && s && skip && y && n > 0 && h > 1 && w > 1 && c > 0, "torgb_up2: bad args");
     S2V_REQUIRE(h % 2 == 0 && w % 2 == 0, "torgb_up2: output %dx%d must be twice the skip size", h, w);
-    S2V_REQUIRE(c % 32 == 0 && xcs % 4 == 0 && xcs >= c && kpad >= c && s_ns >= c && skcs % 4 == 0 && skcs >= 4 &&
-                    ycs % 4 == 0 && ycs >= 4,
-                "torgb_up2: C %% 32 == 0, 4-channel skip / output, float4 pitches required");
-    S2V_REQUIRE(((uintptr_t)x % 16) == 0 && ((uintptr_t)skip % 16) == 0 && ((uintptr_t)y % 16) == 0,
-                "torgb_up2: 16-byte aligned x / skip / y");
-    const long long hw = (long long)h * w, total = (long long)n * hw;
-    int ppt = 16 / (c / 32);
-    if (ppt < 1) ppt = 1;
-    if (ppt > 4) ppt = 4;
-    while (ppt > 1 && hw % (32LL * ppt) != 0) ppt >>= 1;
-    S2V_REQUIRE(hw % (32LL * ppt) == 0, "torgb_up2: h * w must be a multiple of 32 (blocks stay in one sample)");
-    const unsigned grid = (unsigned)(total / (32LL * ppt));
-    const size_t smem = (size_t)3 * c * sizeof(float);
-    hipStream_t st = (hipStream_t)stream;
-    switch (ppt) {
-        case 4: launch_torgb<4>(grid, smem, x, c, h, w, xcs, wt, kpad, s, s_ns, bias, skip, skcs, y, ycs, st); break;
-        case 2: launch_torgb<2>(grid, smem, x, c, h, w, xcs, wt, kpad, s, s_ns, bias, skip, skcs, y, ycs, st); break;
-        default: launch_torgb<1>(grid, smem, x, c, h, w, xcs, wt, kpad, s, s_ns, bias, skip, skcs, y, ycs, st); break;
-    }
-    return check_launch("torgb_up2");
+    const s2v_torgb_win win{h, w, 0, 0, h / 2, w / 2, 0, 0, 0, 0, 0};
+    return s2v_torgb_up2_win(x, n, h, w, c, xcs, wt, kpad, s, s_ns, bias, skip, skcs, y, ycs, &win, stream);
 }
diff --git a/speech-to-video-mpp_amd/engine/enet.py b/speech-to-video-mpp_amd/engine/enet.py
--- a/speech-to-video-mpp_amd/engine/enet.py
+++ b/speech-to-video-mpp_amd/engine/enet.py
@@ -21,6 +21,27 @@
 PREMOD = os.environ.get("S2V_ENET_PREMOD", "1") == "1"
 STACK_STRIPS = os.environ.get("S2V_ENET_STACK_STRIPS", "1") == "1"
 RESUME_GRID = os.environ.get("S2V_ENET_RESUME_GRID", "")
+CROP_TAIL = os.environ.get("S2V_ENET_CROP_TAIL", "1") == "1"
+OUT_CROP = 8
+
+
+def crop_tail_cone(size: int, crop: int):
+    f1, f2 = 2 * size, 4 * size
+    lo, hi = crop, f2 - 1 - crop
+    if crop < 3 or lo > hi:
+        return None
+    need = {"rgb1": (lo, hi), "conv4": (lo, hi), "conv3": (lo - 1, hi + 1)}
+    p0, p1 = (lo - 1) // 2, (hi + 1) // 2
+    need["conv2"] = (p0 - 1, p1 + 1)
+    need["conv1"] = (p0 - 2, p1 + 2)
+    need["rgb0"] = ((2 * lo - 1) // 4, (2 * hi - 1) // 4 + 1)
+    win = {"conv1": (1, f1 - 2), "conv2": (2, f1 - 4), "rgb0": (2, f1 - 4), "conv3": (6, f2 - 12),
+           "conv4": (7, f2 - 14), "rgb1": (7, f2 - 14)}
+    for k, (a, b) in need.items():
+        o, n = win[k]
+        if n <= 0 or a < o or b > o + n - 1:
+            return None
+    return {"need": need, "win": win, "crop": crop - 7, "out": f2 - 2 * crop}
 
 
 def style_grid(device) -> int:
@@ -130,7 +151,7 @@
         ops.modconv_demod_rows(ctx, s2, t, dall, eps=1e-8, post=math.sqrt(2.0))
         return t, dall
 
-    def _premodulate(self, ctx, s2, dtab, dall, b) -> dict:
+    def _premodulate(self, ctx, s2, dtab, dall, b, strips=True) -> dict:
         wb = {}
         for st in range(2):
             for li in range(2):
@@ -142,8 +163,9 @@
                     continue
                 if POLY_UP and L.conv4 is not None:
                     d4 = dall[:, r0: r0 + wd]
-                    wb[idx] = {"conv4": ops.modulate_weights(ctx, L.conv4, sv, d4, b),
-                               "conv": ops.modulate_weights(ctx, L.conv, sv, d4[:, : L.cout], b)}
+                    wb[idx] = {"conv4": ops.modulate_weights(ctx, L.conv4, sv, d4, b)}
+                    if strips:
+                        wb[idx]["conv"] = ops.modulate_weights(ctx, L.conv, sv, d4[:, : L.cout], b)
                 elif L.rp is None:
                     wb[idx] = {"conv": ops.modulate_weights(ctx, L.conv, sv, dall[:, r0: r0 + L.cout], b)}
         return wb
@@ -192,6 +214,72 @@
             ysel(y.t).copy_(ssel(ys.t))
         return y
 
+    def _crop_cone(self, size, out):
+        L = self.layers
+        if not (CROP_TAIL and POLY_UP and FUSED_TORGB) or L[0].conv4 is not None or L[0].rp is not None or \
+                L[3].conv4 is None or L[1].conv4 is not None or L[4].conv4 is not None or L[2].cin % 32 or L[5].cin % 32:
+            return None
+        cone = crop_tail_cone(size, OUT_CROP)
+        if cone is not None and tuple(out.shape[1:]) != (3, cone["out"], cone["out"]):
+            return None
+        return cone
+
+    def _noise_window(self, ctx, L, idx, b, frame, origin, n, noises, ctr):
+        if not L.noise_w:
+            return None
+        if noises is not None and noises[idx] is not None:
+            plane = noises[idx].reshape(b, frame, frame)
+        else:
+            plane = torch.empty((b, frame, frame), device=self.device)
+            ops.gaussian_noise(ctx, plane, self.noise_seed, idx << 36, ctr=ctr, shift=40)
+            self.last_noises[idx] = plane
+        return plane[:, origin: origin + n, origin: origin + n].contiguous()
+
+    def _cropped_tail(self, ctx, cur: NHWC, s2, dtab, dall, wbs, noises, ctr, out, cone):
+        dev, b, win = self.device, cur.n, cone["win"]
+        f1, f2 = 2 * cur.h, 4 * cur.h
+        L = self.layers
+        kw = dict(act=ops.ACT_LRELU, alpha=LRELU, padding=(0, 0))
+
+        def mod(j):
+            sv = s2[:, self.mod_offs[j]: self.mod_offs[j] + L[j].cin]
+            if L[j].is_rgb:
+                return sv, None, {}
+            idx = j - j // 3
+            return sv, dtab.r0[idx], wbs.get(idx, {})
+
+        x = NHWC.empty(b, f1, f1, cur.c, dev)
+        ops.resize_nhwc(ctx, cur, x, scale_factor=2)
+        for j, name in ((0, "conv1"), (1, "conv2")):
+            o, n = win[name]
+            s, r0, wb = mod(j)
+            y = NHWC.empty(b, n, n, L[j].cout, dev)
+            ops.modulated_conv2d(ctx, x, L[j].conv, y, s, dall[:, r0: r0 + L[j].cout], pix_w=L[j].noise_w or 0.0,
+                                 pix_add=self._noise_window(ctx, L[j], j, b, f1, o, n, noises, ctr),
+                                 premod=wb.get("conv"), **kw)
+            x = y
+        o, n = win["rgb0"]
+        rgb0 = NHWC.empty(b, n, n, 4, dev)
+        ops.torgb_up2(ctx, x, L[2].conv, mod(2)[0], cur, rgb0, frame=(f1, f1), origin=(o, o))
+        o3, n3 = win["conv3"]
+        s, r0, wb = mod(3)
+        y = NHWC.empty(b, n3, n3, L[3].cout, dev)
+        ops.modulated_conv2d(ctx, x, L[3].conv4, y, s, dall[:, r0: r0 + dtab.width[2]], d2s=True,
+                             pix_w=L[3].noise_w or 0.0,
+                             pix_add=self._noise_window(ctx, L[3], 2, b, f2, o3, n3, noises, ctr),
+                             premod=wb.get("conv4"), **kw)
+        o4, n4 = win["conv4"]
+        s, r0, wb = mod(4)
+        z = NHWC.empty(b, n4, n4, L[4].cout, dev)
+        ops.modulated_conv2d(ctx, y, L[4].conv, z, s, dall[:, r0: r0 + L[4].cout], pix_w=L[4].noise_w or 0.0,
+                             pix_add=self._noise_window(ctx, L[4], 3, b, f2, o4, n4, noises, ctr),
+                             premod=wb.get("conv"), **kw)
+        dst = out if out.is_contiguous() else torch.empty(out.shape, device=dev)
+        ops.torgb_up2(ctx, z, L[5].conv, mod(5)[0], rgb0, dst, frame=(f2, f2), origin=(o4, o4), skip_origin=(o, o),
+                      crop=(cone["crop"], cone["crop"]))
+        if dst is not out:
+            out.copy_(dst)
+
     def style_code(self, ctx, ref: torch.Tensor):
         st = self.style_begin(ctx, ref)
         self.style_down(ctx, st, len(self.down))
@@ -233,6 +321,7 @@
         b = audio.shape[0]
         svec = NHWC.empty(b, 1, 1, self.mod.cout, dev)
         side = self._side(ctx) if OVERLAP else None
+        cone = self._crop_cone(96 + 4, out)
         enc = {}
 
         def finish(sctx):
@@ -240,7 +329,8 @@
             ops.conv2d(sctx, enc["style"], self.mod, svec)
             enc["d"] = self._demods(sctx, svec.t.view(b, -1))
             if PREMOD:
-                enc["wb"] = self._premodulate(sctx, svec.t.view(b, -1), enc["d"][0], enc["d"][1], b)
+                enc["wb"] = self._premodulate(sctx, svec.t.view(b, -1), enc["d"][0], enc["d"][1], b,
+                                              strips=cone is None)
 
         def fork():
             sst, sctx = side
@@ -294,6 +384,9 @@
         self.last_noises = [None] * 4
         if noises is None and any(L.noise_w for L in self.layers):
             ctr = ctx.noise(id(self)).bump(ctx)
+        if cone is not None:
+            self._cropped_tail(ctx, cur, s2, dtab, dall, enc.get("wb", {}), noises, ctr, out, cone)
+            return out, low
         for st in range(2):
             for li in range(2):
                 L = self.layers[3 * st + li]
diff --git a/speech-to-video-mpp_amd/ops.py b/speech-to-video-mpp_amd/ops.py
--- a/speech-to-video-mpp_amd/ops.py
+++ b/speech-to-video-mpp_amd/ops.py
@@ -673,8 +673,12 @@
 
 def modulated_conv2d(ctx: Ctx, x: NHWC, cw: ConvW, y: NHWC, s: torch.Tensor, d: torch.Tensor | None = None, *,
                      act=ACT_NONE, alpha=0.0, res: NHWC | None = None, res_after=False, pix_add=None, pix_w=0.0,
-                     shift=None, force_splits=0, d2s=False, premod=None):
+                     shift=None, force_splits=0, d2s=False, premod=None, padding=None, force_tile=0):
+    ph, pw = (cw.ph, cw.pw) if padding is None else padding
     oh, ow = cw.out_hw(x.h, x.w)
+    if padding is not None:
+        assert cw.in_mode == IN_DIRECT, "modulated_conv2d: a padding override on direct inputs only"
+        oh, ow = x.h + 2 * ph - (cw.kh - 1), x.w + 2 * pw - (cw.kw - 1)
     assert cw.in_mode != IN_TRANSPOSED and cw.poly is None and (cw.sh, cw.sw, cw.dh, cw.dw) == (1, 1, 1, 1), \
         "modulated_conv2d: direct stride-1 convs only"
     if d2s:
@@ -695,14 +699,15 @@
                             f"conv runs in {PRECISION!r} (code {prec})")
     sh = cw.shift if shift is None else shift
     xscale, flag = _range(ctx, cw, x, prec)
-    key, force_tile = None, 0
-    if (PERFDB or TUNE is not None) and prec != PREC_F32 and not (force_splits or x_split):
+    key = None
+    if (PERFDB or TUNE is not None) and prec != PREC_F32 and not (force_splits or x_split or force_tile) and \
+            padding is None:
         key = conv_key(x, cw, yv, 1, False, layout_code(prec)) + f"|mod{int(d is not None)}{int(d2s)}"
         if TUNE is None and perfdb_applies(x.t.device):
             force_tile, force_splits = PERFDB.get(key, (0, 0))
 
     def launch(ws, dry=False, st=_NOSTAMP, ft=None, fs=None):
-        return S2V.modulated_conv2d_(x.v, yv, cw.wt, s, d, wbuf, cw.cout, [cw.kh, cw.kw], [cw.ph, cw.pw], cw.in_mode,
+        return S2V.modulated_conv2d_(x.v, yv, cw.wt, s, d, wbuf, cw.cout, [cw.kh, cw.kw], [ph, pw], cw.in_mode,
                                      prec,
                                      x_split != 0, cw.scale, sh, pix_add, pix_w, resv, res_after, act, alpha, ws,
                                      force_splits if fs is None else fs, st[0], st[1], st[2], xscale, flag, dry, int(d2s),
@@ -903,10 +908,21 @@
     return out
 
 
-def torgb_up2(ctx: Ctx, x: NHWC, cw: "ConvW", s: torch.Tensor, skip: NHWC, y: NHWC):
+def torgb_up2(ctx: Ctx, x: NHWC, cw: "ConvW", s: torch.Tensor, skip: NHWC, y, *, frame=None, origin=(0, 0),
+              skip_origin=(0, 0), crop=None):
     assert cw.kh == cw.kw == 1 and cw.cout == 3 and x.c == cw.cin, "torgb_up2: a 1x1 conv to 3 channels"
-    assert (y.n, y.h, y.w, y.c) == (x.n, x.h, x.w, 4) and (skip.n, 2 * skip.h, 2 * skip.w, skip.c) == (x.n, x.h, x.w, 4)
-    S2V.torgb_up2_(x.v, cw.wt, s, cw.shift, skip.v, y.v)
+    assert skip.n == x.n and skip.c == 4
+    if frame is None:
+        assert origin == (0, 0) and skip_origin == (0, 0) and (2 * skip.h, 2 * skip.w) == (x.h, x.w)
+        window = []
+    else:
+        window = [int(frame[0]), int(frame[1]), int(origin[0]), int(origin[1]), int(skip_origin[0]), int(skip_origin[1])]
+    if crop is None:
+        assert (y.n, y.h, y.w, y.c) == (x.n, x.h, x.w, 4)
+        S2V.torgb_up2_(x.v, cw.wt, s, cw.shift, skip.v, y.v, window, [])
+    else:
+        assert tuple(y.shape) == (x.n, 3, x.h - 2 * crop[0], x.w - 2 * crop[1])
+        S2V.torgb_up2_(x.v, cw.wt, s, cw.shift, skip.v, y, window, [int(crop[0]), int(crop[1])])
     return y
 
 
```
